# rubund/gnuais

Hardware: AMD Instinct MI355X
Metric: Msamples/s demodulated (N-channel batch, full chain) (higher is better)
Workload: dtype f32 FIR on int16 samples; u32 PLL/HDLC/CRC; 1 GPU; C3: 16384 ch x 48000 samples @48 kHz per GPU, full chain incl. HDLC/CRC-16; channels_per_gpu=16384, samples_per_channel=48000, parallelism=channels sharded over 1 GPU(s), one process per GPU, no collectives

## Files before the change

### gnuais_amd/csrc/batch.h

```cpp
#pragma once
#include <hip/hip_runtime.h>

#include <algorithm>
#include <cmath>
#include <cstdio>
#include <cstdlib>
#include <cstring>
#include <string>
#include <utility>
#include <vector>

#include "../../include/gnuais_hip.h"
#include "kernels.h"

using namespace gnuais;

namespace gnuais {
int fail(int code, const char *what, hipError_t e = hipSuccess);
}

#define HIP_TRY(expr)                                                          \
    do {                                                                       \
        hipError_t e_ = (expr);                                                \
        if (e_ != hipSuccess) return fail(GNUAIS_E_HIP, #expr, e_);            \
    } while (0)

namespace gnuais {

template <class T, bool PINNED = false>
struct Buf {
    T *p = nullptr;
    size_t bytes = 0;
    Buf() = default;
    Buf(Buf &&o) noexcept : p(std::exchange(o.p, nullptr)), bytes(std::exchange(o.bytes, 0)) {}
    Buf &operator=(Buf &&o) noexcept { std::swap(p, o.p); std::swap(bytes, o.bytes); return *this; }
    ~Buf() { (void) release(); }
    operator T *() const { return p; }
    hipError_t release()
    {
        const hipError_t e = !p ? hipSuccess : PINNED ? hipHostFree(p) : hipFree(p);
        p = nullptr;
        bytes = 0;
        return e;
    }
    hipError_t alloc(size_t n, bool zeroed = false)
    {
        hipError_t e = release();
        if (e == hipSuccess) e = PINNED ? hipHostMalloc((void **) &p, n, hipHostMallocDefault) : hipMalloc((void **) &p, n);
        if (e != hipSuccess) return p = nullptr, e;
        bytes = n;
        if (zeroed) e = PINNED ? (memset(p, 0, n), hipSuccess) : hipMemset(p, 0, n);
        if (e != hipSuccess) (void) release();
        return e;
    }
    hipError_t ensure(size_t n, bool zeroed = false) { return p ? hipSuccess : alloc(n, zeroed); }
    hipError_t grow(size_t need, size_t slack = 0) { return bytes >= need ? hipSuccess : alloc(need + slack); }
};
template <class T> using Pinned = Buf<T, true>;

struct Event {
    hipEvent_t e = nullptr;
    Event() = default;
    Event(Event &&o) noexcept : e(std::exchange(o.e, nullptr)) {}
    Event &operator=(Event &&o) noexcept { std::swap(e, o.e); return *this; }
    ~Event() { if (e) (void) hipEventDestroy(e); }
    operator hipEvent_t() const { return e; }
    hipError_t ensure(unsigned flags = hipEventDefault) { return e ? hipSuccess : hipEventCreateWithFlags(&e, flags); }
};

struct Stream {
    hipStream_t s = nullptr;
    Stream() = default;
    Stream(Stream &&o) noexcept : s(std::exchange(o.s, nullptr)) {}
    Stream &operator=(Stream &&o) noexcept { std::swap(s, o.s); return *this; }
    ~Stream() { if (s) (void) hipStreamDestroy(s); }
    operator hipStream_t() const { return s; }
    hipError_t ensure(int priority = 0) { return s ? hipSuccess : hipStreamCreateWithPriority(&s, hipStreamNonBlocking, priority); }
};

}

namespace gnuais {
struct WideStage {
    int K = 0, U = 1, D = 0, T = 0, H = 0, R = 0, NA = 0;
    int per[CHAN_MAX_K] = {}, off[CHAN_MAX_K] = {};
    Buf<uint32_t> mix, poly, hist[2];
    Buf<int32_t> groups;
    Buf<int16_t> taps;
    int cur = 0;
    unsigned long long n = 0;
};
}

enum Stage { CHAN, DISC, AFC, CHAIN, N_STAGES };

enum FormId { AUDIO, IQ, WIDE };

struct gnuais_batch {
    int device = 0;
    int N = 0, NT = 0, NE = 0, d = 0;
    uint32_t pllinc = 0;
    int max_len = 0, frame_cap = 0;
    int sgn_words = 0, bits_words = 0;
    std::vector<float> taps;
    float te[128] = {0};
    static constexpr int HB = 4;
    Buf<int16_t> hist[HB];
    int hist_cur = 0;
    static constexpr int NBUF = 8;
    int nbuf = 3;
    int sets_alloc = 0;
    Buf<uint32_t> sgn[NBUF];
    Buf<uint32_t> pll, lastbit, prev;
    int n_cu = 256;
    Buf<uint32_t> segbits[NBUF];
    Buf<uint32_t> segcnt[NBUF];
    int n_seg = 0, seg_words = 0;
    hipStream_t s_k[4] = {nullptr, nullptr, nullptr, nullptr};
    hipStream_t s_k_default[4] = {nullptr, nullptr, nullptr, nullptr};
    static constexpr int POOL = 12;
    Stream pool[POOL];
    Event e_done[5][NBUF];
    unsigned long long calls = 0, hdlc_calls = 0;
    bool pipeline = true;
    Buf<uint32_t> ctl, cand;
    Buf<uint32_t> cand_first[NBUF], cand_count[NBUF];
    int cand_K = 64;
    Buf<int32_t> counters;
    Buf<int> maxval[HB];
    int max_cur = 0, max_last = 0;
    Buf<float> d_taps;
    Buf<MfmaTaps> d_mfma;
    Buf<uint8_t> d_seq[2];
    Buf<char> d_text;
    Buf<void> nmea_scratch;
    Buf<char> d_msg;
    Buf<uint32_t> d_word;
    Buf<void> vt;
    Buf<uint32_t> vt_fslot;
    uint32_t vt_slots = 0;
    int vt_capacity = 0;
    static constexpr int NRING = 8;
    Buf<gnuais_frame> ring[NRING];
    Buf<uint32_t> ring_count[NRING];
    Buf<uint2> ring_chunks[NRING];
    int ring_runs[NRING] = {};
    int n_chunks = 0;
    bool frame_times = false;
    unsigned long long rows = 0;
    bool clock_fresh = true;
    Buf<int64_t> times;
    bool frame_signal = false, fs_iq_call = false;
    int fs_RB = 0, fs_nbuf = 0;
    unsigned long long fs_v0 = 0, fs_end = 0;
    Buf<int64_t> fs_ring;
    Buf<uint32_t> fs_carry;
    Buf<gnuais_frame_signal> signal;
    int occ_E = 0, occ_margin = 0, occ_CB = 0, occ_nbuf = 0, occ_W = 0;
    bool occ_cover_clean = false;
    unsigned long long occ_v0 = 0, occ_seq = 0, occ_drained = 0;
    long long occ_next = 0, occ_lost = 0;
    long long occ_first[64] = {};
    Buf<uint16_t> occ_codes;
    Buf<uint8_t> occ_cover, occ_carry;
    Buf<gnuais_occupancy> occ_out;
    bool repair = false;
    Buf<int32_t> repaired;
    bool long_frames = false;
    int long_cap = 0;
    Buf<uint32_t> long_ctl, long_open, long_count;
    Buf<int32_t> long_counters;
    Buf<gnuais_long_frame> long_ring;
    bool long_repair = false;
    int long_cand_cap = 0;
    int long_parity = 0;
    Buf<uint32_t> long_clean, long_cand, long_cand_count;
    int uq_window = 0, uq_hash_bits = 64, uq_cur = 0, uq_n_tail = 0;
    long long uq_late = 0;
    Buf<uint32_t> uq_tail[2];
    Buf<void> uq_scratch;
    Buf<void> uq_heard;
    int ring_cur = 0;
    bool streaming = false;
    hipStream_t s_post = nullptr, s_copy = nullptr;
    Stream s_copy_own;
    Event e_fill[NRING], e_fmt[NRING], e_txt[NRING];
    Buf<char> sd_text[NRING];
    Pinned<char> sh_text[NRING];
    Pinned<uint32_t> sh_info;
    int s_stage[NRING] = {};
    size_t sh_text_want = 0;
    Buf<uint32_t> sd_info;
    bool copy_on_k3 = false;
    int copy_wgs = 24;
    Buf<uint8_t> sd_seq[2];
    int sd_seq_cur = 0;
    unsigned long long stream_calls = 0;
    Buf<int16_t> stage_x;
    Buf<float> stage_f;
    Pinned<int16_t> pin[2];
    Buf<int16_t> dev_in[2];
    size_t pin_bytes = 0;
    Stream s_io;
    Event e_in[2];
    hipEvent_t e_in_hook = nullptr;
    unsigned long long host_calls = 0;
    FirOptions fir;
    SignBounds sign;
    int stage_mask = 0x1f;
    int k0 = 0;
    int pll_variant = 0;
    int hdlc_lpw = 0;
    int hdlc_variant = 1;
    bool timing = false;
    int timing_stride = 1;
    static constexpr int TIMING_RING = 64;
    Event evr[TIMING_RING][10];
    unsigned long long timed_calls = 0;
    int last_k = 0;
    bool timed_last = false;
    struct { hipStream_t s = nullptr; bool used = false; } last[N_STAGES];
    int last_len = 0;
    int pll_form = 0;
    int k3_same = 1;
    Buf<int16_t> iq_prev;
    Buf<int16_t> iq_audio;
    WideStage wide;
    Buf<int16_t> wide_iq;
    int afc_W = 0, afc_nb = 0, afc_est_row = -1;
    unsigned long long afc_n = 0;
    Buf<int64_t> afc_blk;
    Buf<int16_t> afc_delay, afc_est, afc_audio;
};

struct Form {
    int bytes, cols, rows;
    unsigned stages;
    int up = 1;
    size_t bytes_of(int in_rows) const { return (size_t) bytes * (size_t) cols * (size_t) in_rows; }
};

namespace gnuais {
int set_device(const gnuais_batch *b);
int drain(gnuais_batch *b, unsigned stages, hipStream_t s);
hipStream_t k3_stream(const gnuais_batch *b);
hipStream_t behind_k3(const gnuais_batch *b);
double now_ms();
int chan_zero_state(gnuais_batch *b);
int afc_zero_state(gnuais_batch *b);
int occ_zero_state(gnuais_batch *b);
int occ_tail(gnuais_batch *b, const HdlcLaunch &h, int len, hipStream_t s);
}
```

### gnuais_amd/csrc/capi_delivery.hip

```cpp
#include "batch.h"

extern "C" {

static int ensure_post_buffers(gnuais_batch *b, uint32_t have)
{
    const size_t need_text = (size_t) have * 164, need_scratch = nmea_scratch_bytes((int) have);
    HIP_TRY(b->d_text.grow(need_text));
    HIP_TRY(b->nmea_scratch.grow(need_scratch));
    return GNUAIS_OK;
}

struct Pending {
    uint32_t have;
    bool overflow, watchdog;
};

static int read_pending(gnuais_batch *b, Pending &p)
{
    if (int rc = gnuais_batch_sync(b)) return rc;
    uint32_t cnt[4] = {0, 0, 0, 0};
    HIP_TRY(hipMemcpy(cnt, b->ring_count[0], sizeof cnt, hipMemcpyDeviceToHost));
    p.have = std::min<uint32_t>(cnt[0], (uint32_t) b->frame_cap);
    p.overflow = cnt[1] || cnt[0] > (uint32_t) b->frame_cap;
    p.watchdog = cnt[3] != 0;
    return GNUAIS_OK;
}

static int late_error(const char *who, bool watchdog, bool overflow, const char *watchdog_tail = "")
{
    char msg[200];
    if (watchdog) {
        snprintf(msg, sizeof msg, "%s: the PLL stage's watchdog fired (device hung or badly oversubscribed)%s", who, watchdog_tail);
        return fail(GNUAIS_E_HIP, msg);
    }
    if (!overflow) return GNUAIS_OK;
    snprintf(msg, sizeof msg, "%s: frame ring overflowed, frames were dropped", who);
    return fail(GNUAIS_E_OVERFLOW, msg);
}

static int finish_drain(gnuais_batch *b, const Pending &p, const char *who, const char *watchdog_tail = "")
{
    HIP_TRY(hipMemset(b->ring_count[0], 0, sizeof(uint32_t) * 4));
    b->hdlc_calls = 0;
    return late_error(who, p.watchdog, p.overflow, watchdog_tail);
}

static int upload_seq(gnuais_batch *b, const uint8_t *seqnr)
{
    const size_t N = (size_t) b->N;
    for (auto &p : b->d_seq) HIP_TRY(p.ensure(N));
    HIP_TRY(hipMemcpy(b->d_seq[0], seqnr, N, hipMemcpyHostToDevice));
    HIP_TRY(hipMemcpy(b->d_seq[1], b->d_seq[0], N, hipMemcpyDeviceToDevice));
    return GNUAIS_OK;
}

static int drain_impl(gnuais_batch *b, gnuais_frame *h_frames, int max_frames, int *n_frames,
                      uint8_t *seqnr, char *out, size_t out_cap, size_t *out_len, int *n_sentences,
                      int64_t *h_times = nullptr, gnuais_frame_signal *h_signal = nullptr)
{
    if (b->streaming) return fail(GNUAIS_E_STATE, "drain: the batch is streaming (gnuais_batch_stream_nmea); "
                                                  "set_option(\"streaming\", 0) leaves that mode");
    Pending pend;
    if (int rc = read_pending(b, pend)) return rc;
    const uint32_t have = pend.have;
    if (h_frames && (uint32_t) max_frames < have) return fail(GNUAIS_E_ARG, "drain: frame buffer too small");
    if (have) {
        const size_t N = (size_t) b->N;
        if (int rc = ensure_post_buffers(b, have)) return rc;
        if (seqnr) {
            if (int rc = upload_seq(b, seqnr)) return rc;
            uint32_t info[3] = {0, 0, 0};
            HIP_TRY(nmea_format(b->ring[0], (int) have, b->N, b->d_seq[0], b->d_seq[1], b->d_text, b->d_text.bytes,
                                b->nmea_scratch, b->nmea_scratch.bytes, info, nullptr));
            if (info[2]) return fail(GNUAIS_E_HIP, "drain: a frame record names a channel outside the batch");
            if ((size_t) info[0] > out_cap) {
                *out_len = info[0];
                return fail(GNUAIS_E_ARG, "drain: text buffer too small");
            }
            if (info[0]) HIP_TRY(hipMemcpy(out, b->d_text, info[0], hipMemcpyDeviceToHost));
            HIP_TRY(hipMemcpy(seqnr, b->d_seq[1], N, hipMemcpyDeviceToHost));
            *out_len = info[0];
            if (n_sentences) *n_sentences = (int) info[1];
        }
        if (h_frames) {
            static_assert(sizeof(gnuais_frame_signal) == sizeof(int64_t), "the signal records leave through the times' gather");
            gnuais_frame *sorted = reinterpret_cast<gnuais_frame *>(b->d_text.p);
            int64_t *sorted_t = reinterpret_cast<int64_t *>(sorted + have), *sorted_s = sorted_t + have;
            HIP_TRY(frames_sort_timed(b->ring[0], h_times ? b->times.p : nullptr, (int) have, sorted, sorted_t,
                                      b->nmea_scratch, b->nmea_scratch.bytes, nullptr,
                                      h_signal ? reinterpret_cast<const int64_t *>(b->signal.p) : nullptr, sorted_s));
            HIP_TRY(hipMemcpy(h_frames, sorted, sizeof(gnuais_frame) * have, hipMemcpyDeviceToHost));
            if (h_times) HIP_TRY(hipMemcpy(h_times, sorted_t, sizeof(int64_t) * have, hipMemcpyDeviceToHost));
            if (h_signal) HIP_TRY(hipMemcpy(h_signal, sorted_s, sizeof(gnuais_frame_signal) * have, hipMemcpyDeviceToHost));
        }
        if (n_frames) *n_frames = (int) have;
    }
    return finish_drain(b, pend, "drain", "; results are incomplete");
}

int gnuais_batch_drain_messages(gnuais_batch *b, uint8_t *seqnr, const char *chanid, char *nmea, size_t nmea_cap,
                                size_t *nmea_len, int *n_sentences, char *text, size_t text_cap, size_t *text_len,
                                int *n_lines, int *n_frames)
{
    if (!b || !seqnr || !nmea_len || !text_len || (nmea_cap && !nmea) || (text_cap && !text))
        return fail(GNUAIS_E_ARG, "drain_messages: argument");
    if (b->streaming) return fail(GNUAIS_E_ARG, "drain_messages: the batch is streaming (gnuais_batch_stream_nmea)");
    *nmea_len = *text_len = 0;
    if (n_sentences) *n_sentences = 0;
    if (n_lines) *n_lines = 0;
    if (n_frames) *n_frames = 0;
    Pending pend;
    if (int rc = read_pending(b, pend)) return rc;
    const uint32_t have = pend.have;
    if (have) {
        const size_t N = (size_t) b->N, line = messages_line_bytes();
        if (nmea_cap < (size_t) have * 164 || text_cap < (size_t) have * line)
            return fail(GNUAIS_E_ARG, "drain_messages: buffers too small (164 / 512 bytes per pending frame always suffice)");
        if (int rc = ensure_post_buffers(b, have)) return rc;
        const size_t need = (size_t) have * line * 2 + (size_t) have * 8 + 256 + N + 256;
        HIP_TRY(b->d_msg.grow(need, need / 4));
        char *lines = b->d_msg, *packed = lines + (size_t) have * line;
        uint32_t *len = reinterpret_cast<uint32_t *>(packed + (size_t) have * line), *off = len + have;
        uint32_t *info2 = off + have;
        char *d_chanid = reinterpret_cast<char *>(info2 + 64);
        if (chanid) HIP_TRY(hipMemcpy(d_chanid, chanid, N, hipMemcpyHostToDevice));
        if (int rc = upload_seq(b, seqnr)) return rc;
        uint32_t raw[4] = {0, 0, 0, 0}, inf[2] = {0, 0};
        HIP_TRY(nmea_format_enqueue(b->ring[0], (int) have, (int) have, b->N, b->d_seq[0], b->d_seq[1], b->d_text,
                                    b->d_text.bytes, b->nmea_scratch, b->nmea_scratch.bytes, raw, nullptr, 0, 0,
                                    nullptr, nullptr));
        HIP_TRY(messages_format_enqueue(b->ring[0], (int) have, b->N, b->d_seq[0], chanid ? d_chanid : nullptr,
                                        b->nmea_scratch, b->nmea_scratch.bytes, lines, len, off, packed,
                                        (size_t) have * line, info2, nullptr));
        HIP_TRY(hipDeviceSynchronize());
        HIP_TRY(hipMemcpy(inf, info2, 8, hipMemcpyDeviceToHost));
        if (raw[3]) return fail(GNUAIS_E_HIP, "drain_messages: a frame record names a channel outside the batch");
        const size_t nl = (size_t) raw[0] + raw[1];
        if (nl) HIP_TRY(hipMemcpy(nmea, b->d_text, nl, hipMemcpyDeviceToHost));
        if (inf[0]) HIP_TRY(hipMemcpy(text, packed, inf[0], hipMemcpyDeviceToHost));
        HIP_TRY(hipMemcpy(seqnr, b->d_seq[1], N, hipMemcpyDeviceToHost));
        *nmea_len = nl;
        *text_len = inf[0];
        if (n_sentences) *n_sentences = (int) raw[2];
        if (n_lines) *n_lines = (int) inf[1];
        if (n_frames) *n_frames = (int) have;
    }
    return finish_drain(b, pend, "drain_messages");
}

int gnuais_batch_fold_vessels(gnuais_batch *b, gnuais_vessel *vessels, int cap, int *n_vessels)
{
    if (!b || !n_vessels || cap < 0 || (cap > 0 && !vessels)) return fail(GNUAIS_E_ARG, "fold_vessels: argument");
    if (b->streaming) return fail(GNUAIS_E_ARG, "fold_vessels: the batch is streaming (gnuais_batch_stream_nmea)");
    *n_vessels = 0;
    Pending pend;
    if (int rc = read_pending(b, pend)) return rc;
    const uint32_t have = pend.have;
    if (!have) return GNUAIS_OK;
    if (int rc = ensure_post_buffers(b, have)) return rc;
    gnuais_vessel *d_tab = reinterpret_cast<gnuais_vessel *>(b->d_text.p);
    const int d_cap = (int) std::min<size_t>(b->d_text.bytes / sizeof(gnuais_vessel), (size_t) have);
    HIP_TRY(b->d_word.ensure(16));
    HIP_TRY(vessels_fold_enqueue(b->ring[0], (int) have, b->nmea_scratch, b->nmea_scratch.bytes, d_tab, d_cap,
                                 b->d_word, nullptr));
    HIP_TRY(hipDeviceSynchronize());
    uint32_t nv = 0;
    HIP_TRY(hipMemcpy(&nv, b->d_word, 4, hipMemcpyDeviceToHost));
    *n_vessels = (int) nv;
    if ((int) nv > cap) return fail(GNUAIS_E_OVERFLOW, "fold_vessels: table too small (*n_vessels entries needed)");
    if (nv) HIP_TRY(hipMemcpy(vessels, d_tab, sizeof(gnuais_vessel) * nv, hipMemcpyDeviceToHost));
    return GNUAIS_OK;
}

int gnuais_batch_vessel_table_enable(gnuais_batch *b, int capacity)
{
    if (!b || capacity < 1 || capacity > (1 << 24)) return fail(GNUAIS_E_ARG, "vessel_table_enable: capacity 1 .. 2^24");
    if (int rc = gnuais_batch_sync(b)) return rc;
    if (b->s_post) HIP_TRY(hipStreamSynchronize(b->s_post));
    uint32_t slots = 1024;
    while (slots < 2u * (uint32_t) capacity) slots <<= 1;
    b->vt_slots = 0;
    HIP_TRY(b->vt.alloc(vessel_table_bytes(slots), true));
    HIP_TRY(b->vt_fslot.ensure(sizeof(uint32_t) * (size_t) b->frame_cap));
    b->vt_slots = slots;
    b->vt_capacity = capacity;
    return GNUAIS_OK;
}

int gnuais_batch_vessel_table_clear(gnuais_batch *b)
{
    if (!b || !b->vt) return fail(GNUAIS_E_STATE, "vessel_table_clear: no table (gnuais_batch_vessel_table_enable)");
    if (int rc = gnuais_batch_sync(b)) return rc;
    if (b->s_post) HIP_TRY(hipStreamSynchronize(b->s_post));
    HIP_TRY(hipMemset(b->vt, 0, vessel_table_bytes(b->vt_slots)));
    return GNUAIS_OK;
}

int gnuais_batch_vessel_table_update(gnuais_batch *b)
{
    if (!b || !b->vt) return fail(GNUAIS_E_STATE, "vessel_table_update: no table (gnuais_batch_vessel_table_enable)");
    if (b->streaming) return fail(GNUAIS_E_STATE, "vessel_table_update: a streaming batch updates its table by itself");
    if (int rc = gnuais_batch_sync(b)) return rc;
    HIP_TRY(vessel_table_update_enqueue(b->ring[0], b->ring_count[0], b->frame_cap, b->vt, b->vt_slots, b->vt_fslot, behind_k3(b)));
    return GNUAIS_OK;
}

int gnuais_batch_vessel_table(gnuais_batch *b, gnuais_vessel *vessels, int cap, int *n_vessels)
{
    if (!b || !n_vessels || cap < 0 || (cap > 0 && !vessels)) return fail(GNUAIS_E_ARG, "vessel_table: argument");
    *n_vessels = 0;
    if (!b->vt) return fail(GNUAIS_E_STATE, "vessel_table: no table (gnuais_batch_vessel_table_enable)");
    if (int rc = set_device(b)) return rc;
    hipStream_t s = b->streaming ? b->s_post : behind_k3(b);
    uint32_t info[4] = {0, 0, 0, 0};
    int n = 0;
    HIP_TRY(vessel_table_fetch(b->vt, b->vt_slots, vessels, cap, &n, info, s));
    *n_vessels = n;
    if (info[1] || (int) info[0] > b->vt_capacity) {
        char msg[160];
        snprintf(msg, sizeof msg, "vessel_table: more vessels than the table was enabled for (%u seen%s, capacity %d)",
                 info[0], info[1] ? ", some dropped" : "", b->vt_capacity);
        return fail(GNUAIS_E_OVERFLOW, msg);
    }
    if (n > cap) return fail(GNUAIS_E_OVERFLOW, "vessel_table: output too small (*n_vessels entries needed)");
    std::sort(vessels, vessels + n, [](const gnuais_vessel &x, const gnuais_vessel &y) { return x.mmsi < y.mmsi; });
    return GNUAIS_OK;
}

int gnuais_batch_drain_frames(gnuais_batch *b, gnuais_frame *h_out, int max, int *n_out)
{
    if (!b || !n_out || (max > 0 && !h_out)) return fail(GNUAIS_E_ARG, "drain_frames: argument");
    *n_out = 0;
    static gnuais_frame none;
    return drain_impl(b, h_out ? h_out : &none, max, n_out, nullptr, nullptr, 0, nullptr, nullptr);
}

int gnuais_batch_drain_frames_timed(gnuais_batch *b, gnuais_frame *h_out, int64_t *h_times, int max, int *n_out)
{
    if (!b || !n_out || (max > 0 && (!h_out || !h_times))) return fail(GNUAIS_E_ARG, "drain_frames_timed: argument");
    *n_out = 0;
    if (!b->frame_times) return fail(GNUAIS_E_STATE, "drain_frames_timed: the batch does not time its frames (gnuais_batch_frame_times)");
    static gnuais_frame none;
    static int64_t none_t;
    return drain_impl(b, h_out ? h_out : &none, max, n_out, nullptr, nullptr, 0, nullptr, nullptr, h_times ? h_times : &none_t);
}

int gnuais_batch_drain_frames_signal(gnuais_batch *b, gnuais_frame *h_out, int64_t *h_times, gnuais_frame_signal *h_signal,
                                     int max, int *n_out)
{
    if (!b || !n_out || (max > 0 && (!h_out || !h_times || !h_signal))) return fail(GNUAIS_E_ARG, "drain_frames_signal: argument");
    *n_out = 0;
    if (!b->frame_signal) return fail(GNUAIS_E_STATE, "drain_frames_signal: the batch does not measure its frames (gnuais_batch_frame_signal)");
    static gnuais_frame none;
    static int64_t none_t;
    static gnuais_frame_signal none_s;
    return drain_impl(b, h_out ? h_out : &none, max, n_out, nullptr, nullptr, 0, nullptr, nullptr, h_times ? h_times : &none_t,
                      h_signal ? h_signal : &none_s);
}

static int drain_unique_impl(gnuais_batch *b, gnuais_frame *h_out, int64_t *h_times, int32_t *h_copies, int max, int *n_out,
                             int32_t *h_first, gnuais_hearer *h_members, int *n_members)
{
    *n_out = 0;
    if (!b->uq_window) return fail(GNUAIS_E_STATE, "drain_frames_unique: the batch does not merge duplicates (gnuais_batch_unique)");
    if (b->streaming) return fail(GNUAIS_E_STATE, "drain_frames_unique: the batch is streaming (gnuais_batch_stream_nmea)");
    Pending pend;
    if (int rc = read_pending(b, pend)) return rc;
    const uint32_t have = pend.have;
    if ((uint32_t) max < have) return fail(GNUAIS_E_ARG, "drain_frames_unique: buffers too small (one entry per pending frame always suffices)");
    const size_t m = (size_t) b->uq_n_tail + have;
    if (m) {
        if (have)
            if (int rc = ensure_post_buffers(b, have)) return rc;
        const size_t need = unique_scratch_bytes((int) m);
        HIP_TRY(b->uq_scratch.grow(need, need / 4));
        Buf<uint32_t> &next = b->uq_tail[b->uq_cur ^ 1];
        HIP_TRY(next.grow(64 * m, 16 * m));
        auto bits_of = [](unsigned long long v) { int n = 1; while (v >> n) ++n; return n; };
        UniqueLaunch a;
        a.frames = b->ring[0];
        a.times = b->times;
        a.have = (int) have;
        a.tail = b->uq_tail[b->uq_cur];
        a.n_tail = b->uq_n_tail;
        a.tail_out = next;
        a.window = b->uq_window;
        a.rows = (long long) b->rows;
        a.hash_bits = b->uq_hash_bits;
        a.ch_bits = bits_of((unsigned long long) (b->N - 1));
        a.time_bits = bits_of(b->rows);
        a.scratch = b->uq_scratch;
        a.scratch_bytes = b->uq_scratch.bytes;
        a.out_frames = reinterpret_cast<gnuais_frame *>(b->d_text.p);
        a.out_times = reinterpret_cast<int64_t *>(a.out_frames + have);
        a.out_copies = reinterpret_cast<int32_t *>(a.out_times + have);
        if (h_first) {
            static_assert(sizeof(gnuais_hearer) == 24 && sizeof(gnuais_frame_signal) == 8, "a member is three 64-bit words");
            const size_t need_h = unique_heard_scratch_bytes((int) have);
            HIP_TRY(b->uq_heard.grow(need_h, need_h / 4));
            a.signal = b->frame_signal ? b->signal.p : nullptr;
            a.heard_scratch = b->uq_heard;
            a.heard_scratch_bytes = b->uq_heard.bytes;
            a.out_first = a.out_copies + have;
            const uintptr_t at = reinterpret_cast<uintptr_t>(a.out_first + have + 1);
            a.out_members = reinterpret_cast<gnuais_hearer *>((at + 15) & ~(uintptr_t) 15);
        }
        uint32_t info[UNIQUE_INFO_WORDS] = {0};
        for (int exact = 0; exact < 2; ++exact) {
            HIP_TRY(unique_cluster_enqueue(a, exact != 0, nullptr));
            HIP_TRY(hipMemcpy(info, unique_info(a.scratch), sizeof info, hipMemcpyDeviceToHost));
            if (!info[UNIQUE_INFO_COLLISION]) break;
        }
        const uint32_t np = info[UNIQUE_INFO_PRIMARIES];
        if (np > have || info[UNIQUE_INFO_TAIL] > m) return fail(GNUAIS_E_HIP, "drain_frames_unique: the stage's counts are out of range");
        if (np) {
            HIP_TRY(unique_deliver_enqueue(a, (int) np, nullptr));
            HIP_TRY(hipMemcpy(h_out, a.out_frames, sizeof(gnuais_frame) * np, hipMemcpyDeviceToHost));
            HIP_TRY(hipMemcpy(h_times, a.out_times, sizeof(int64_t) * np, hipMemcpyDeviceToHost));
            HIP_TRY(hipMemcpy(h_copies, a.out_copies, sizeof(int32_t) * np, hipMemcpyDeviceToHost));
            if (h_first) {
                HIP_TRY(hipMemcpy(h_first, a.out_first, sizeof(int32_t) * ((size_t) np + 1), hipMemcpyDeviceToHost));
                const int32_t nm = h_first[np];
                if (nm < 0 || (uint32_t) nm > have) return fail(GNUAIS_E_HIP, "drain_frames_heard: the stage's counts are out of range");
                HIP_TRY(hipMemcpy(h_members, a.out_members, sizeof(gnuais_hearer) * (size_t) nm, hipMemcpyDeviceToHost));
                *n_members = (int) nm;
            }
        }
        unsigned long long late = 0;
        memcpy(&late, info + UNIQUE_INFO_LATE, sizeof late);
        b->uq_cur ^= 1;
        b->uq_n_tail = (int) info[UNIQUE_INFO_TAIL];
        b->uq_late += (long long) late;
        *n_out = (int) np;
    }
    return finish_drain(b, pend, h_first ? "drain_frames_heard" : "drain_frames_unique", "; results are incomplete");
}

int gnuais_batch_drain_frames_unique(gnuais_batch *b, gnuais_frame *h_out, int64_t *h_times, int32_t *h_copies, int max,
                                     int *n_out)
{
    if (!b || !n_out || max < 0 || (max > 0 && (!h_out || !h_times || !h_copies)))
        return fail(GNUAIS_E_ARG, "drain_frames_unique: argument");
    return drain_unique_impl(b, h_out, h_times, h_copies, max, n_out, nullptr, nullptr, nullptr);
}

int gnuais_batch_drain_frames_heard(gnuais_batch *b, gnuais_frame *h_out, int64_t *h_times, int32_t *h_copies, int max,
                                    int *n_out, int32_t *h_first, gnuais_hearer *h_members, int *n_members)
{
    if (!b || !n_out || !n_members || !h_first || max < 0 || (max > 0 && (!h_out || !h_times || !h_copies || !h_members)))
        return fail(GNUAIS_E_ARG, "drain_frames_heard: argument");
    *n_members = 0;
    h_first[0] = 0;
    return drain_unique_impl(b, h_out, h_times, h_copies, max, n_out, h_first, h_members, n_members);
}

int gnuais_batch_drain_nmea(gnuais_batch *b, uint8_t *seqnr, char *out, size_t out_cap, size_t *out_len,
                            int *n_sentences, int *n_frames)
{
    if (!b || !seqnr || !out_len || (out_cap > 0 && !out)) return fail(GNUAIS_E_ARG, "drain_nmea: argument");
    *out_len = 0;
    if (n_sentences) *n_sentences = 0;
    if (n_frames) *n_frames = 0;
    return drain_impl(b, nullptr, 0, n_frames, seqnr, out, out_cap, out_len, n_sentences);
}

int gnuais_batch_drain_frames_nmea(gnuais_batch *b, gnuais_frame *h_frames, int max, int *n_frames,
                                   uint8_t *seqnr, char *out, size_t out_cap, size_t *out_len, int *n_sentences)
{
    if (!b || !h_frames || !n_frames || !seqnr || !out_len || (out_cap > 0 && !out))
        return fail(GNUAIS_E_ARG, "drain_frames_nmea: argument");
    *n_frames = 0;
    *out_len = 0;
    if (n_sentences) *n_sentences = 0;
    return drain_impl(b, h_frames, max, n_frames, seqnr, out, out_cap, out_len, n_sentences);
}

static int stream_setup(gnuais_batch *b)
{
    constexpr int NR = gnuais_batch::NRING;
    const size_t N = (size_t) b->N;
    const size_t text_cap = (size_t) b->frame_cap * 164;
    if (b->frame_times) return fail(GNUAIS_E_STATE, "stream_nmea: the batch times its frames (gnuais_batch_frame_times); "
                                                    "the streamed delivery carries no times");
    if (b->repair) return fail(GNUAIS_E_STATE, "stream_nmea: the batch repairs frames (gnuais_batch_repair); the streamed "
                                               "delivery's order table describes the CRC stage's records only");
    if (b->frame_signal) return fail(GNUAIS_E_STATE, "stream_nmea: the batch measures its frames (gnuais_batch_frame_signal); "
                                                     "the streamed delivery carries no records of them");
    if (b->uq_window) return fail(GNUAIS_E_STATE, "stream_nmea: the batch merges duplicates (gnuais_batch_unique); the "
                                                  "streamed delivery has no such stage");
    if (b->long_frames) return fail(GNUAIS_E_STATE, "stream_nmea: the batch decodes long frames (gnuais_batch_long_frames); "
                                                    "the streamed delivery carries no records of them");
    if (int rc = gnuais_batch_sync(b)) return rc;
    for (int q = 1; q < NR; ++q) {
        HIP_TRY(b->ring[q].ensure(sizeof(gnuais_frame) * (size_t) b->frame_cap));
        HIP_TRY(b->ring_count[q].ensure(sizeof(uint32_t) * 4, true));
    }
    b->n_chunks = k3_blocks(b->N) * k3_passes(b->cand_K);
    b->sh_text_want = std::max(b->sh_text_want, ((size_t) b->frame_cap * 32 + 65536) & ~(size_t) 15);
    for (int q = 0; q < NR; ++q) {
        HIP_TRY(b->ring_chunks[q].ensure(sizeof(uint2) * (size_t) b->n_chunks));
        b->ring_runs[q] = 2;
        HIP_TRY(b->sd_text[q].ensure(text_cap));
        for (Event *e : {&b->e_fill[q], &b->e_fmt[q], &b->e_txt[q]}) HIP_TRY(e->ensure(hipEventDisableTiming));
        HIP_TRY(b->sh_text[q].ensure(b->sh_text_want));
    }
    HIP_TRY(b->sd_info.ensure(sizeof(uint32_t) * 8 * NR, true));
    if (const char *v = getenv("GNUAIS_COPY_WGS")) b->copy_wgs = std::max(1, atoi(v));
    if (const char *v = getenv("GNUAIS_COPY_ON_K3")) b->copy_on_k3 = atoi(v) != 0;
    HIP_TRY(b->nmea_scratch.grow(nmea_scratch_bytes(b->frame_cap, b->n_chunks)));
    if (!b->s_copy_own) {
        int lo = 0, hi = 0;
        HIP_TRY(hipDeviceGetStreamPriorityRange(&lo, &hi));
        HIP_TRY(b->s_copy_own.ensure(hi));
        b->s_copy = b->s_copy_own;
    }
    HIP_TRY(b->sh_info.ensure(sizeof(uint32_t) * 8 * NR, true));
    for (auto &p : b->sd_seq) HIP_TRY(p.ensure(N, true));
    HIP_TRY(hipDeviceSynchronize());
    b->streaming = true;
    return GNUAIS_OK;
}

int gnuais_batch_stream_nmea(gnuais_batch *b, const char **text, size_t *len, int *n_sentences, int *n_frames)
{
    if (!b || !text || !len) return fail(GNUAIS_E_ARG, "stream_nmea: argument");
    if (int rc = set_device(b)) return rc;
    *text = nullptr;
    *len = 0;
    if (n_sentences) *n_sentences = 0;
    if (n_frames) *n_frames = -1;
    constexpr int NR = gnuais_batch::NRING;
    const size_t N = (size_t) b->N;
    if (!b->streaming)
        if (int rc = stream_setup(b)) return rc;
    hipStream_t sD = behind_k3(b);
    const int c = b->ring_cur;
    HIP_TRY(hipEventRecord(b->e_fill[c], sD));
    const int runs = b->ring_runs[c];
    const int nx = (c + 1) % NR;
    if (b->s_stage[nx]) HIP_TRY(hipStreamWaitEvent(sD, b->e_fmt[nx], 0));
    b->ring_cur = nx;
    b->ring_runs[nx] = 0;
    int rc_late = GNUAIS_OK;
    if (b->s_stage[nx]) {
        HIP_TRY(hipEventSynchronize(b->e_txt[nx]));
        const uint32_t *info = b->sh_info + 8 * nx;
        const uint32_t have = std::min<uint32_t>(info[4], (uint32_t) b->frame_cap);
        const size_t n_text = (size_t) info[0] + info[1];
        if (n_text > b->sh_text[nx].bytes) {
            const size_t want = std::max(b->sh_text_want, (n_text + n_text / 2 + 65536) & ~(size_t) 15);
            b->sh_text_want = want;
            HIP_TRY(b->sh_text[nx].grow(b->sh_text_want));
            HIP_TRY(hipMemcpyAsync(b->sh_text[nx], b->sd_text[nx], n_text, hipMemcpyDeviceToHost, b->s_copy));
            HIP_TRY(hipStreamSynchronize(b->s_copy));
        }
        *text = b->sh_text[nx];
        *len = n_text;
        if (n_sentences) *n_sentences = (int) info[2];
        if (n_frames) *n_frames = (int) have;
        b->s_stage[nx] = 0;
        if (info[3]) rc_late = fail(GNUAIS_E_HIP, "stream_nmea: a frame record names a channel outside the batch");
        else rc_late = late_error("stream_nmea", info[7] != 0, info[5] || info[4] > (uint32_t) b->frame_cap);
    }
    b->s_post = sD;
    uint32_t *totals = nullptr;
    HIP_TRY(b->sh_text[c].grow(b->sh_text_want));
    if (runs >= 1) {
        int n_host = -1;
        if (runs > 1) {
            uint32_t cnt[4];
            HIP_TRY(hipStreamSynchronize(b->s_post));
            HIP_TRY(hipMemcpy(cnt, b->ring_count[c], 16, hipMemcpyDeviceToHost));
            n_host = (int) std::min<uint32_t>(cnt[0], (uint32_t) b->frame_cap);
        }
        if (n_host != 0) {
            uint8_t *sin = b->sd_seq[b->sd_seq_cur], *sout = b->sd_seq[b->sd_seq_cur ^ 1];
            HIP_TRY(hipMemcpyAsync(sout, sin, N, hipMemcpyDeviceToDevice, b->s_post));
            HIP_TRY(nmea_format_enqueue(b->ring[c], n_host, b->frame_cap, b->N, sin, sout, b->sd_text[c],
                                        b->sd_text[c].bytes, b->nmea_scratch, b->nmea_scratch.bytes, nullptr,
                                        b->ring_chunks[c], b->n_chunks, k3_passes(b->cand_K), &totals, b->s_post));
            b->sd_seq_cur ^= 1;
        }
    }
    if (b->vt && runs >= 1)
        HIP_TRY(vessel_table_update_enqueue(b->ring[c], b->ring_count[c], b->frame_cap, b->vt, b->vt_slots, b->vt_fslot,
                                            b->s_post));
    HIP_TRY(nmea_slot_info_enqueue(totals, b->ring_count[c], b->sd_info + 8 * c, b->s_post));
    HIP_TRY(hipMemsetAsync(b->ring_count[c], 0, 16, b->s_post));
    HIP_TRY(hipEventRecord(b->e_fmt[c], b->s_post));
    hipStream_t sc = b->copy_on_k3 ? b->s_post : b->s_copy;
    if (!b->copy_on_k3) HIP_TRY(hipStreamWaitEvent(sc, b->e_fmt[c], 0));
    HIP_TRY(nmea_text_copy_enqueue(b->sd_text[c], b->sd_info + 8 * c, b->sh_text[c], b->sh_text[c].bytes,
                                   b->sh_info + 8 * c, b->copy_wgs, sc));
    HIP_TRY(hipEventRecord(b->e_txt[c], sc));
    b->s_stage[c] = 1;
    b->hdlc_calls = 0;
    b->stream_calls++;
    return rc_late;
}

int gnuais_batch_pending_frames(gnuais_batch *b, int *n_out)
{
    if (!b || !n_out) return fail(GNUAIS_E_ARG, "pending_frames: argument");
    if (b->streaming) return fail(GNUAIS_E_STATE, "pending_frames: the batch is streaming (gnuais_batch_stream_nmea)");
    Pending pend;
    if (int rc = read_pending(b, pend)) return rc;
    *n_out = (int) pend.have;
    return GNUAIS_OK;
}

int gnuais_batch_discard_frames(gnuais_batch *b, void *stream)
{
    if (!b) return fail(GNUAIS_E_ARG, "discard_frames: NULL batch");
    if (b->streaming) return fail(GNUAIS_E_STATE, "discard_frames: the batch is streaming (gnuais_batch_stream_nmea)");
    if (int rc = set_device(b)) return rc;
    hipStream_t s = b->pipeline ? k3_stream(b) : (hipStream_t) stream;
    HIP_TRY(hipMemsetAsync(b->ring_count[0], 0, sizeof(uint32_t) * 3, s));
    b->hdlc_calls = 0;
    return GNUAIS_OK;
}

int gnuais_batch_autotune_delivery(gnuais_batch *b, const int16_t *d_samples, int len, void *stream, float *ms_per_call)
{
    if (!b || !d_samples) return fail(GNUAIS_E_ARG, "autotune_delivery: NULL argument");
    if (int rc = gnuais_batch_sync(b)) return rc;
    const char *text = nullptr;
    size_t tl = 0;
    if (int rc = gnuais_batch_stream_nmea(b, &text, &tl, nullptr, nullptr)) return rc;
    if (!b->pipeline) {
        if (ms_per_call) *ms_per_call = 0.0f;
        return gnuais_batch_reset(b);
    }
    const bool timing = b->timing;
    b->timing = false;
    auto quiesce = [&]() -> int {
        if (int rc = gnuais_batch_sync(b)) return rc;
        HIP_TRY(hipDeviceSynchronize());
        return GNUAIS_OK;
    };
    auto measure = [&](double &ms, int meas) -> int {
        const int warm = gnuais_batch::NRING + 2;
        for (int i = 0; i < warm + meas; ++i) {
            if (i == warm) {
                if (int rc = quiesce()) return rc;
                ms = -now_ms();
            }
            if (int rc = gnuais_batch_run(b, d_samples, len, stream)) return rc;
            const int rc = gnuais_batch_stream_nmea(b, &text, &tl, nullptr, nullptr);
            if (rc != GNUAIS_OK && rc != GNUAIS_E_OVERFLOW) return rc;
        }
        if (int rc = quiesce()) return rc;
        ms = (ms + now_ms()) / meas;
        return GNUAIS_OK;
    };
    hipStream_t own = b->s_copy_own;
    hipStream_t top[2] = {own, own};
    double top_ms[2] = {1e30, 1e30};
    for (int cand = -1; cand < gnuais_batch::POOL; ++cand) {
        hipStream_t st = cand < 0 ? own : b->pool[cand];
        bool used = false;
        for (int q = 0; q < 4; ++q) used |= b->s_k[q] == st;
        if (used || !st) continue;
        b->s_copy = st;
        double ms = 0;
        if (int rc = measure(ms, 12)) return rc;
        if (ms < top_ms[0]) { top_ms[1] = top_ms[0]; top[1] = top[0]; top_ms[0] = ms; top[0] = st; }
        else if (ms < top_ms[1]) { top_ms[1] = ms; top[1] = st; }
    }
    hipStream_t best_s = top[0];
    double best = 1e30;
    for (int k = 0; k < 2; ++k) {
        if (k == 1 && top[1] == top[0]) break;
        b->s_copy = top[k];
        double ms = 0;
        if (int rc = measure(ms, 30)) return rc;
        if (ms < best) { best = ms; best_s = top[k]; }
    }
    b->s_copy = best_s;
    b->timing = timing;
    if (ms_per_call) *ms_per_call = (float) best;
    return gnuais_batch_reset(b);
}

}
```

### gnuais_amd/csrc/gnuais_capi.hip

```cpp
#include <chrono>

#include "batch.h"

namespace gnuais {
namespace scalar { hipError_t launch_fir_slice(const FirLaunch &a, hipStream_t stream); }
}

static thread_local std::string g_err;

int gnuais::fail(int code, const char *what, hipError_t e)
{
    char buf[512];
    if (e != hipSuccess)
        snprintf(buf, sizeof buf, "%s: %s", what, hipGetErrorString(e));
    else
        snprintf(buf, sizeof buf, "%s", what);
    g_err = buf;
    return code;
}

static const double k_tap_half[18] = {
    2.5959e-55, 2.9479e-49, 1.4741e-43, 3.2462e-38, 3.1480e-33, 1.3443e-28,
    2.5280e-24, 2.0934e-20, 7.6339e-17, 1.2259e-13, 8.6690e-11, 2.6996e-08,
    3.7020e-06, 2.2355e-04, 5.9448e-03, 6.9616e-02, 3.5899e-01, 8.1522e-01};

int gnuais::drain(gnuais_batch *b, unsigned stages, hipStream_t s)
{
    for (int q = 0; q < N_STAGES; ++q) {
        auto &l = b->last[q];
        if (!(stages >> q & 1u) || !l.used || l.s == s) continue;
        HIP_TRY(hipStreamSynchronize(l.s));
        l.s = s;
    }
    return GNUAIS_OK;
}

int gnuais::set_device(const gnuais_batch *b)
{
    HIP_TRY(hipSetDevice(b->device));
    return GNUAIS_OK;
}

double gnuais::now_ms()
{
    return std::chrono::duration<double, std::milli>(std::chrono::steady_clock::now().time_since_epoch()).count();
}

hipStream_t gnuais::k3_stream(const gnuais_batch *b)
{
    return (b->k3_same && !b->streaming) ? b->s_k[2] : b->s_k[3];
}

hipStream_t gnuais::behind_k3(const gnuais_batch *b) { return b->pipeline ? k3_stream(b) : b->last[CHAIN].s; }

template <class T>
static int read_out(gnuais_batch *b, const void *d, size_t n, std::vector<T> &v)
{
    if (int rc = gnuais_batch_sync(b)) return rc;
    v.resize(n);
    HIP_TRY(hipMemcpy(v.data(), d, n * sizeof(T), hipMemcpyDeviceToHost));
    return GNUAIS_OK;
}

extern "C" {

const char *gnuais_last_error(void) { return g_err.c_str(); }
const char *gnuais_version(void) { return "gnuais-hip 0.1 (gfx950)"; }

int gnuais_default_taps(float *out36)
{
    if (!out36) return fail(GNUAIS_E_ARG, "gnuais_default_taps: NULL");
    for (int k = 0; k < 18; ++k) {
        out36[k] = (float) k_tap_half[k];
        out36[35 - k] = (float) k_tap_half[k];
    }
    return 36;
}

static hipError_t alloc_sets(gnuais_batch *b, int n)
{
    const size_t N = (size_t) b->N;
    for (int k = b->sets_alloc; k < n && k < gnuais_batch::NBUF; ++k) {
        struct { Buf<uint32_t> &buf; size_t bytes; } want[] = {
            {b->sgn[k], sizeof(uint32_t) * sgn_words_alloc(b->sgn_words, b->N)},
            {b->segbits[k], sizeof(uint32_t) * N * (size_t) b->n_seg * PACK_STRIDE},
            {b->segcnt[k], sizeof(uint32_t) * N * (size_t) b->n_seg},
            {b->cand_first[k], sizeof(uint32_t) * N},
            {b->cand_count[k], sizeof(uint32_t) * N}};
        for (auto &w : want)
            if (hipError_t e = w.buf.ensure(w.bytes, true)) return e;
        b->sets_alloc = k + 1;
    }
    return hipSuccess;
}

void gnuais_batch_destroy(gnuais_batch *b)
{
    if (!b) return;
    (void) hipSetDevice(b->device);
    delete b;
}

int gnuais_batch_create(gnuais_batch **out, int device, int n_channels, const float *taps,
                        int n_taps, unsigned pllinc, int max_len, int frame_capacity)
{
    if (!out) return fail(GNUAIS_E_ARG, "create: out is NULL");
    *out = nullptr;
    if (n_channels <= 0 || max_len <= 0) return fail(GNUAIS_E_ARG, "create: n_channels/max_len");
    if (taps && (n_taps <= 0 || n_taps > GNUAIS_MAX_TAPS)) return fail(GNUAIS_E_ARG, "create: n_taps");
    if (pllinc > 0xffffu) return fail(GNUAIS_E_ARG, "create: pllinc must be < 0x10000");
    int ndev = 0;
    HIP_TRY(hipGetDeviceCount(&ndev));
    if (ndev <= 0) return fail(GNUAIS_E_HIP, "create: no HIP device");
    if (device < 0 || device >= ndev) return fail(GNUAIS_E_ARG, "create: device index");
    HIP_TRY(hipSetDevice(device));
    {
        int lds = 0;
        if (hipDeviceGetAttribute(&lds, hipDeviceAttributeMaxSharedMemoryPerBlock, device) == hipSuccess &&
            lds < pll_need_lds())
            return fail(GNUAIS_E_HIP, "create: the device offers too little LDS per workgroup (gfx950 / MI355X with "
                                      "160 KB is what this library is built for)");
    }
    HIP_TRY(pll_prepare_device());

    gnuais_batch *b = new gnuais_batch;
    b->device = device;
    if (hipDeviceGetAttribute(&b->n_cu, hipDeviceAttributeMultiprocessorCount, device) != hipSuccess || b->n_cu <= 0)
        b->n_cu = 256;
    b->N = n_channels;
    if (taps) {
        b->taps.assign(taps, taps + n_taps);
    } else {
        b->taps.resize(36);
        gnuais_default_taps(b->taps.data());
    }
    b->NT = (int) b->taps.size();
    b->pllinc = pllinc ? pllinc : (0x10000u / 5u);
    b->max_len = max_len;
    b->frame_cap = frame_capacity > 0 ? frame_capacity : std::max(4096, n_channels * 48);

    int k0 = 0, k1 = b->NT - 1;
    while (k0 < b->NT - 1 && b->taps[k0] == 0.0f) ++k0;
    while (k1 > k0 && b->taps[k1] == 0.0f) --k1;
    b->NE = k1 - k0 + 1;
    b->d = b->NT - k0;
    b->k0 = k0;
    if (b->NE <= FIR_MAX_NE)
        for (int j = 0; j < b->NE; ++j) b->te[j] = b->taps[k0 + j];

    b->sign = sign_bounds(b->te, b->NE);
    b->sgn_words = (max_len + 31) / 32;
    const uint64_t step = (uint64_t) b->pllinc + b->pllinc / 16;
    b->bits_words = (int) (((uint64_t) max_len * step / 65536 + 2 + 31) / 32) + 1;

    const size_t N = (size_t) b->N;
    hipError_t e = hipSuccess;
    b->n_seg = (b->sgn_words + SEG_WORDS - 1) / SEG_WORDS;
    b->seg_words = (int) (((uint64_t) SEG_WORDS * 32 * step / 65536 + 2 + 31) / 32) + 1;
    const uint64_t launch_bits = std::max((uint64_t) b->bits_words * 32, (uint64_t) b->seg_words * 32 * (uint64_t) b->n_seg);
    b->cand_K = (int) std::max<uint64_t>(64, launch_bits / 30 + 2);
    if (const char *v = getenv("GNUAIS_NBUF")) b->nbuf = std::min((int) gnuais_batch::NBUF, std::max(2, atoi(v)));
    {
        const size_t per_set = sizeof(uint32_t) * (sgn_words_alloc(b->sgn_words, b->N) + N * (size_t) b->n_seg * (PACK_STRIDE + 1) + 2 * N);
        const size_t need = gnuais_batch::HB * (sizeof(int16_t) * N * b->NT + sizeof(int) * N) + (size_t) b->nbuf * per_set +
                            sizeof(uint32_t) * N * ((size_t) b->cand_K * CAND_WORDS + HDLC_CTL_WORDS + 6) +
                            sizeof(gnuais_frame) * (size_t) b->frame_cap;
        size_t free_b = 0, total_b = 0;
        if (hipMemGetInfo(&free_b, &total_b) == hipSuccess && need > free_b) {
            char msg[256];
            snprintf(msg, sizeof msg, "create: %d channels x %d samples need %.2f GB of device memory, device %d has %.2f GB free of %.2f",
                     b->N, b->max_len, need / 1e9, device, free_b / 1e9, total_b / 1e9);
            delete b;
            return fail(GNUAIS_E_HIP, msg);
        }
    }
    auto alloc = [&](auto &buf, size_t bytes) {
        if (e == hipSuccess) e = buf.alloc(bytes, true);
    };
    for (int q = 0; q < gnuais_batch::HB; ++q) alloc(b->hist[q], sizeof(int16_t) * N * b->NT);
    if (b->seg_words > 16) {
        gnuais_batch_destroy(b);
        return fail(GNUAIS_E_ARG, "create: pllinc too large (more than one slice per ~4.6 samples)");
    }
    if (e == hipSuccess) e = alloc_sets(b, b->nbuf);
    alloc(b->pll, sizeof(uint32_t) * N);
    alloc(b->lastbit, sizeof(uint32_t) * N);
    alloc(b->prev, sizeof(uint32_t) * N);
    alloc(b->ctl, sizeof(uint32_t) * N * HDLC_CTL_WORDS);
    alloc(b->cand, sizeof(uint32_t) * N * (size_t) b->cand_K * CAND_WORDS);
    alloc(b->ring_count[0], sizeof(uint32_t) * 4);
    alloc(b->counters, sizeof(int32_t) * N * 3);
    for (int q = 0; q < gnuais_batch::HB; ++q) alloc(b->maxval[q], sizeof(int) * N);
    alloc(b->ring[0], sizeof(gnuais_frame) * (size_t) b->frame_cap);
    alloc(b->d_taps, sizeof(float) * b->NT);
    alloc(b->iq_prev, sizeof(int16_t) * 2 * N);
    if (b->sign.mfma_ok) {
        MfmaTaps host;
        fir_sign_mfma_pack(b->sign.tq, b->sign.tq_sum, &host);
        alloc(b->d_mfma, sizeof(MfmaTaps));
        if (e == hipSuccess) e = hipMemcpy(b->d_mfma, &host, sizeof(MfmaTaps), hipMemcpyHostToDevice);
    }
    if (e == hipSuccess)
        e = hipMemcpy(b->d_taps, b->taps.data(), sizeof(float) * b->NT, hipMemcpyHostToDevice);
    for (auto &set : b->evr)
        for (auto &ev : set)
            if (e == hipSuccess) e = ev.ensure();
    for (auto &pair : b->e_done)
        for (auto &ev : pair)
            if (e == hipSuccess) e = ev.ensure(hipEventDisableTiming);
    {
        int lo = 0, hi = 0;
        if (e == hipSuccess) e = hipDeviceGetStreamPriorityRange(&lo, &hi);
        const char *order = getenv("GNUAIS_STREAM_ORDER");
        if (!order || strlen(order) != 4) order = "0123";
        int made = 0;
        for (int q = 0; q < 4; ++q) {
            const int idx = (order[q] - '0') & 3;
            if (e == hipSuccess && !b->s_k[idx]) {
                e = b->pool[made].ensure(hi);
                b->s_k[idx] = b->pool[made++];
            }
        }
        for (auto &st : b->s_k)
            if (e == hipSuccess && !st) {
                e = b->pool[made].ensure(hi);
                st = b->pool[made++];
            }
        for (int q = 0; q < 4; ++q) b->s_k_default[q] = b->s_k[q];
        for (; made < gnuais_batch::POOL; ++made)
            if (e == hipSuccess) e = b->pool[made].ensure(made < 8 ? hi : 0);
    }
    if (const char *v = getenv("GNUAIS_K3_SAME")) b->k3_same = atoi(v) != 0;
    if (const char *v = getenv("GNUAIS_PLL_VARIANT")) {
        const int pv = atoi(v);
        if (pv == 0 || pv == 7 || pv == 8) b->pll_variant = pv;
    }
    if (const char *v = getenv("GNUAIS_PIPELINE")) b->pipeline = atoi(v) != 0;
    if (const char *v = getenv("GNUAIS_HDLC_VARIANT")) b->hdlc_variant = atoi(v) != 0;
    if (const char *v = getenv("GNUAIS_HDLC_LPW")) b->hdlc_lpw = std::min(64, std::max(1, atoi(v)));
    if (e != hipSuccess) {
        gnuais_batch_destroy(b);
        return fail(GNUAIS_E_HIP, "create: device allocation", e);
    }
    if (const char *v = getenv("GNUAIS_FIR_VARIANT")) {
        const int fv = atoi(v);
        if (fv == 0 || fv == 3) b->fir.fir_variant = fv;
    }
    if (const char *v = getenv("GNUAIS_FIR_FLAG2")) b->fir.fir_flag2 = atoi(v) != 0;
    if (const char *v = getenv("GNUAIS_FIR_T")) b->fir.fir_T = std::max(64, atoi(v) / 32 * 32);
    *out = b;
    int rc = gnuais_batch_reset(b);
    if (rc != GNUAIS_OK) {
        gnuais_batch_destroy(b);
        *out = nullptr;
    }
    return rc;
}


static int rings_reset(gnuais_batch *b)
{
    for (int q = 0; q < gnuais_batch::NRING; ++q) {
        if (b->ring_count[q]) HIP_TRY(hipMemset(b->ring_count[q], 0, sizeof(uint32_t) * 4));
        b->s_stage[q] = 0;
        b->ring_runs[q] = 0;
    }
    b->ring_cur = 0;
    b->stream_calls = 0;
    return GNUAIS_OK;
}

static int long_zero_state(gnuais_batch *b, bool everything)
{
    if (!b->long_ctl) return GNUAIS_OK;
    HIP_TRY(launch_hdlc_long_reset(b->long_ctl, everything ? b->long_counters.p : nullptr, b->N, nullptr));
    if (everything) HIP_TRY(hipMemset(b->long_count, 0, sizeof(uint32_t) * 2));
    if (everything && b->long_cand_count) {
        HIP_TRY(hipMemset(b->long_cand_count, 0, sizeof(uint32_t) * 2));
        b->long_parity = 0;
    }
    return GNUAIS_OK;
}

static int latch_rows(gnuais_batch *b, unsigned long long rows)
{
    b->rows = rows;
    b->fs_v0 = b->fs_end = rows;
    return occ_zero_state(b);
}

int gnuais_batch_reset(gnuais_batch *b)
{
    if (!b) return fail(GNUAIS_E_ARG, "reset: NULL batch");
    if (int rc = set_device(b)) return rc;
    const size_t N = (size_t) b->N;
    HIP_TRY(hipDeviceSynchronize());
    for (int q = 0; q < gnuais_batch::HB; ++q)
        HIP_TRY(hipMemset(b->hist[q], 0, sizeof(int16_t) * N * b->NT));
    b->hist_cur = 0;
    HIP_TRY(hipMemset(b->pll, 0, sizeof(uint32_t) * N));
    HIP_TRY(hipMemset(b->lastbit, 0, sizeof(uint32_t) * N));
    HIP_TRY(hipMemset(b->prev, 0, sizeof(uint32_t) * N));
    for (int k = 0; k < b->sets_alloc; ++k)
        HIP_TRY(hipMemset(b->segcnt[k], 0, sizeof(uint32_t) * N * (size_t) b->n_seg));
    b->calls = 0;
    if (int rc = latch_rows(b, 0)) return rc;
    b->last[CHAIN].used = false;
    b->hdlc_calls = 0;
    HIP_TRY(hipMemset(b->counters, 0, sizeof(int32_t) * N * 3));
    if (b->repaired) HIP_TRY(hipMemset(b->repaired, 0, sizeof(int32_t) * N));
    b->uq_n_tail = 0;
    b->uq_late = 0;
    for (int q = 0; q < gnuais_batch::HB; ++q) HIP_TRY(hipMemset(b->maxval[q], 0, sizeof(int) * N));
    b->max_cur = 0;
    b->max_last = 0;
    if (int rc = rings_reset(b)) return rc;
    for (auto &p : b->sd_seq)
        if (p) HIP_TRY(hipMemset(p, 0, N));
    HIP_TRY(launch_hdlc_reset(b->ctl, b->N, nullptr));
    if (int rc = long_zero_state(b, true)) return rc;
    HIP_TRY(hipMemset(b->iq_prev, 0, sizeof(int16_t) * 2 * N));
    b->last[DISC].used = false;
    if (int rc = chan_zero_state(b)) return rc;
    if (int rc = afc_zero_state(b)) return rc;
    HIP_TRY(hipDeviceSynchronize());
    b->last_len = 0;
    b->pll_form = 0;
    b->clock_fresh = true;
    return GNUAIS_OK;
}

int gnuais_batch_set_clock(gnuais_batch *b, long long rows, const uint64_t *h_bits)
{
    if (!b) return fail(GNUAIS_E_ARG, "set_clock: NULL batch");
    if (rows < 0) return fail(GNUAIS_E_ARG, "set_clock: rows < 0");
    if (!b->clock_fresh) return fail(GNUAIS_E_STATE, "set_clock: a run or decode call has been made since create / reset");
    if (b->wide.K || b->afc_W)
        return fail(GNUAIS_E_STATE, "set_clock: not with a wide stage or the AFC configured (their sample counts start at 0)");
    if (int rc = set_device(b)) return rc;
    const size_t N = (size_t) b->N;
    std::vector<uint32_t> lo(N), hi(N);
    for (size_t c = 0; c < N; ++c) {
        const uint64_t v = h_bits ? h_bits[c] : 0;
        lo[c] = (uint32_t) v;
        hi[c] = (uint32_t) (v >> 32);
    }
    HIP_TRY(hipDeviceSynchronize());
    HIP_TRY(hipMemcpy(b->ctl + 2 * N, lo.data(), sizeof(uint32_t) * N, hipMemcpyHostToDevice));
    HIP_TRY(hipMemcpy(b->ctl + 5 * N, hi.data(), sizeof(uint32_t) * N, hipMemcpyHostToDevice));
    return latch_rows(b, (unsigned long long) rows);
}

int gnuais_batch_set_option(gnuais_batch *b, const char *name, int value)
{
    if (!b || !name) return fail(GNUAIS_E_ARG, "set_option: NULL");
    if (!strcmp(name, "stage_mask")) {
        b->stage_mask = value & 0x1f;
        return GNUAIS_OK;
    }
    if (!strcmp(name, "fir_T")) {
        if (value < 64 || value % 32) return fail(GNUAIS_E_ARG, "fir_T must be a multiple of 32, >= 64");
        b->fir.fir_T = value;
    } else if (!strcmp(name, "nbuf")) {
        if (value < 2 || value > gnuais_batch::NBUF) return fail(GNUAIS_E_ARG, "nbuf must be 2..8");
        if (b->frame_signal && value > b->fs_nbuf)
            return fail(GNUAIS_E_STATE, "nbuf: the block ring of gnuais_batch_frame_signal is sized for the depth it was switched on "
                                        "at; switch it off first");
        if (b->occ_E && value > b->occ_nbuf)
            return fail(GNUAIS_E_STATE, "nbuf: the rings of gnuais_batch_occupancy are sized for the depth it was switched on at; "
                                        "switch it off first");
        if (int rc = gnuais_batch_sync(b)) return rc;
        HIP_TRY(hipDeviceSynchronize());
        HIP_TRY(alloc_sets(b, value));
        b->nbuf = value;
    } else if (!strcmp(name, "streaming")) {
        if (value != 0 && b->frame_times)
            return fail(GNUAIS_E_STATE, "streaming: the batch times its frames (gnuais_batch_frame_times); the streamed delivery carries no times");
        if (value != 0 && b->repair)
            return fail(GNUAIS_E_STATE, "streaming: the batch repairs frames (gnuais_batch_repair); the streamed delivery's order table describes the CRC stage's records only");
        if (value != 0 && b->frame_signal)
            return fail(GNUAIS_E_STATE, "streaming: the batch measures its frames (gnuais_batch_frame_signal); the streamed delivery carries no records of them");
        if (value != 0 && b->uq_window)
            return fail(GNUAIS_E_STATE, "streaming: the batch merges duplicates (gnuais_batch_unique); the streamed delivery has no such stage");
        if (value != 0 && b->long_repair)
            return fail(GNUAIS_E_STATE, "streaming: the batch repairs long frames (gnuais_batch_long_repair); the streamed delivery carries no records of them");
        if (value != 0 && b->long_frames)
            return fail(GNUAIS_E_STATE, "streaming: the batch decodes long frames (gnuais_batch_long_frames); the streamed delivery carries no records of them");
        if (value != 0) return fail(GNUAIS_E_ARG, "streaming can only be switched off here (stream_nmea switches it on)");
        if (b->streaming) {
            if (int rc = gnuais_batch_sync(b)) return rc;
            HIP_TRY(hipDeviceSynchronize());
            if (int rc = rings_reset(b)) return rc;
            b->hdlc_calls = 0;
            b->streaming = false;
        }
    } else if (!strcmp(name, "fir_flag2")) {
        if (value != 0 && value != 1) return fail(GNUAIS_E_ARG, "fir_flag2: 0 or 1");
        b->fir.fir_flag2 = value;
    } else if (!strcmp(name, "fir_pk_taps")) {
        if (value != 0 && value != 48) return fail(GNUAIS_E_ARG, "fir_pk_taps: 0 or 48");
        b->fir.fir_pk_taps = value;
    } else if (!strcmp(name, "fir_mfma")) {
        if (value != 0 && value != 1) return fail(GNUAIS_E_ARG, "fir_mfma: 0 or 1");
        b->fir.fir_mfma = value;
    } else if (!strcmp(name, "fir_variant")) {
        if (value != 0 && value != 3) return fail(GNUAIS_E_ARG, "fir_variant must be 0 (the exact sum for every sample) or 3 (the sign-exact slicer)");
        b->fir.fir_variant = value;
    } else if (!strcmp(name, "timing_stride")) {
        if (value < 1) return fail(GNUAIS_E_ARG, "timing_stride must be >= 1");
        b->timing_stride = value;
    } else if (!strcmp(name, "pipeline")) {
        b->pipeline = value != 0;
    } else if (!strcmp(name, "pll_variant")) {
        if (value != 0 && value != 7 && value != 8)
            return fail(GNUAIS_E_ARG, "pll_variant must be 0 (by channel count), 7 (time-parallel, pll_tp.hip) or 8 (pll_h3.hip)");
        b->pll_variant = value;
    } else if (!strcmp(name, "hdlc_variant")) {
        b->hdlc_variant = value != 0;
    } else if (!strcmp(name, "unique_hash_bits")) {
        if (value < 1 || value > 64) return fail(GNUAIS_E_ARG, "unique_hash_bits must be 1..64");
        b->uq_hash_bits = value;
    } else if (!strcmp(name, "hdlc_lpw")) {
        if (value < 1 || value > 64) return fail(GNUAIS_E_ARG, "hdlc_lpw must be 1..64");
        b->hdlc_lpw = value;
    } else {
        return fail(GNUAIS_E_ARG, "set_option: unknown option");
    }
    return GNUAIS_OK;
}

static void fill_fir(const gnuais_batch *b, FirLaunch &f, const int16_t *x, int len, float *dump,
                     int k)
{
    memset(&f, 0, sizeof f);
    f.x = x;
    f.hist = b->hist[b->hist_cur];
    f.sgn = b->sgn[k];
    f.dump = dump;
    f.maxval = b->maxval[b->max_cur];
    f.hist_out = b->hist[(b->hist_cur + 1) % gnuais_batch::HB];
    f.maxval_next = b->maxval[(b->max_cur + 2) % gnuais_batch::HB];
    f.d_taps = b->d_taps;
    memcpy(f.te, b->te, sizeof f.te);
    f.N = b->N;
    f.L = len;
    f.NT = b->NT;
    f.NE = b->NE;
    f.d = b->d;
    f.te_mem = b->d_taps + b->k0;
    f.map = 1;
}

static void fill_hdlc(const gnuais_batch *b, HdlcLaunch &h, int k)
{
    h.segbits = b->segbits[k]; h.segcnt = b->segcnt[k]; h.ctl = b->ctl; h.cand = b->cand;
    h.cand_first = b->cand_first[k]; h.cand_count = b->cand_count[k];
    h.counters = b->counters;
    h.frames = b->ring[b->ring_cur];
    h.frame_count = b->ring_count[b->ring_cur];
    h.frame_cap = (uint32_t) b->frame_cap; h.N = b->N; h.n_seg = b->n_seg;
    h.seg_words = b->seg_words; h.K = b->cand_K; h.K_call = b->cand_K;
    int small_lpw = 1;
    while (small_lpw < 16 && (b->N + small_lpw - 1) / small_lpw > 512) small_lpw *= 2;
    if (b->N > PLL_TP_MAX_CHANNELS) small_lpw = 16;
    const int ev_lpw = 2 * ((b->N + 63) / 64) > (b->n_cu > 0 ? b->n_cu : 256) ? 64 : small_lpw;
    h.lanes_per_wave = b->hdlc_lpw ? b->hdlc_lpw : (b->hdlc_variant ? ev_lpw : 64);
    h.chunks = (b->streaming && b->ring_runs[b->ring_cur] == 0) ? b->ring_chunks[b->ring_cur] : nullptr;
}

static FrameTimeLaunch fill_frame_times(const gnuais_batch *b, const HdlcLaunch &h, int len)
{
    FrameTimeLaunch t;
    t.frames = h.frames; t.frame_count = h.frame_count; t.frame_cap = h.frame_cap;
    t.ctl = h.ctl; t.segcnt = h.segcnt; t.times = b->times;
    t.N = h.N; t.n_seg = h.n_seg; t.seg_words = h.seg_words;
    t.len = len; t.n0 = (int64_t) b->rows;
    return t;
}

static FrameSignalLaunch fill_frame_signal(const gnuais_batch *b, const HdlcLaunch &h, int len)
{
    FrameSignalLaunch a;
    a.frames = h.frames; a.frame_count = h.frame_count; a.frame_cap = h.frame_cap;
    a.times = b->times; a.ring = b->fs_ring; a.signal = b->signal.p;
    a.RB = b->fs_RB; a.N = h.N;
    a.len = len; a.n0 = (int64_t) b->rows;
    a.pllinc = b->pllinc; a.n_taps = b->NT; a.afc_window = b->afc_W;
    a.v0 = (int64_t) (b->fs_iq_call ? b->fs_v0 : b->rows + (unsigned long long) std::max(len, 0));
    return a;
}

static RepairLaunch fill_repair(const gnuais_batch *b, const HdlcLaunch &h)
{
    RepairLaunch r;
    r.cand = h.cand; r.cand_first = h.cand_first; r.cand_count = h.cand_count;
    r.repaired = b->repaired;
    r.frames = h.frames; r.frame_count = h.frame_count; r.frame_cap = h.frame_cap;
    r.N = h.N; r.K = h.K;
    return r;
}

static LongLaunch fill_long(const gnuais_batch *b, const HdlcLaunch &h, int len)
{
    LongLaunch a;
    a.segbits = h.segbits; a.segcnt = h.segcnt; a.ctl = h.ctl;
    a.lctl = b->long_ctl; a.open = b->long_open; a.counters = b->long_counters;
    a.frames = b->long_ring.p; a.frame_count = b->long_count; a.frame_cap = (uint32_t) b->long_cap;
    a.N = h.N; a.n_seg = h.n_seg; a.seg_words = h.seg_words;
    a.len = len; a.n0 = (int64_t) b->rows;
    if (b->long_repair) {
        a.clean = b->long_clean; a.cand = b->long_cand; a.cand_count = b->long_cand_count;
        a.cand_cap = (uint32_t) b->long_cand_cap; a.parity = b->long_parity;
    }
    return a;
}

static int run_long(gnuais_batch *b, const HdlcLaunch &h, int len, hipStream_t s)
{
    HIP_TRY(launch_hdlc_long(fill_long(b, h, len), s));
    if (b->long_repair) {
        LongRepairLaunch r;
        r.cand = b->long_cand; r.cand_count = b->long_cand_count.p + b->long_parity; r.cand_cap = (uint32_t) b->long_cand_cap;
        r.repaired = b->long_counters.p + 2 * (size_t) b->N;
        r.frames = b->long_ring.p; r.frame_count = b->long_count; r.frame_cap = (uint32_t) b->long_cap;
        r.N = b->N;
        r.blocks = 16 * std::max(b->n_cu, 1);
        HIP_TRY(launch_hdlc_long_repair(r, s));
        b->long_parity ^= 1;
    }
    return GNUAIS_OK;
}

static int run_fir(gnuais_batch *b, const int16_t *x, int len, float *dump, hipStream_t s, int k)
{
    const FirPlan p = plan_fir(b->sign, b->fir, FirShape{b->N, b->NT, b->NE, b->d}, len, dump != nullptr);
    FirLaunch f;
    fill_fir(b, f, x, len, dump, k);
    static_cast<FirThresholds &>(f) = p.th;
    if (b->sign.ok)
        for (int j = 0; j < f.NC; ++j) f.ctaps[j] = b->te[(b->NE - f.NC) / 2 + j];
    switch (p.kernel) {
    case FirKernel::GENERIC:
        HIP_TRY(hipMemsetAsync(f.maxval_next, 0, sizeof(int) * (size_t) b->N, s));
        HIP_TRY(launch_fir_generic(f, s));
        HIP_TRY(launch_fir_history(x, f.hist, f.hist_out, b->N, len, b->NT, s));
        break;
    case FirKernel::SCALAR32:
        HIP_TRY(scalar::launch_fir_slice(f, s));
        break;
    case FirKernel::SIGN:
        HIP_TRY(launch_fir_sign(f, s));
        break;
    case FirKernel::SIGN_PACKED:
        HIP_TRY(launch_fir_sign_pk(f, s));
        break;
    case FirKernel::SIGN_PACKED_MFMA: {
        FirLaunch m = f;
        f.T = p.head;
        f.max_segments = 1;
        m.NC = FIR_MFMA_NC;
        m.mfma = b->d_mfma;
        m.eps_seen = p.mfma_seen_u;
        m.eps_ahead = p.mfma_abs_u;
        HIP_TRY(launch_fir_sign_pk(f, s));
        HIP_TRY(launch_fir_sign_mfma(m, p.head, s));
        break;
    }
    }
    b->hist_cur = (b->hist_cur + 1) % gnuais_batch::HB;
    b->max_last = b->max_cur;
    b->max_cur = (b->max_cur + 1) % gnuais_batch::HB;
    return GNUAIS_OK;
}

static void fill_pll(const gnuais_batch *b, PllLaunch &p, int k, int len)
{
    p.sgn = b->sgn[k]; p.pll = b->pll; p.prev = b->prev;
    p.watchdog = b->ring_count[b->ring_cur] + 3; p.lastbit = b->lastbit;
    p.segbits = b->segbits[k]; p.segcnt = b->segcnt[k];
    p.N = b->N; p.L = len; p.n_seg = b->n_seg; p.seg_words = b->seg_words; p.pllinc = b->pllinc; p.variant = b->pll_variant;
    p.n_cu = b->n_cu;
}


static int run_tail(gnuais_batch *b, int k, int len, bool tm, const Event *ev,
                    hipStream_t s0, hipEvent_t after)
{
    const bool pl = b->pipeline;
    hipStream_t sC = pl ? b->s_k[2] : s0, sD = pl ? k3_stream(b) : s0;
    HdlcLaunch h;
    fill_hdlc(b, h, k);
    if (pl && after) HIP_TRY(hipStreamWaitEvent(sC, after, 0));
    if (pl && b->calls >= 1 && sD != sC)
        HIP_TRY(hipStreamWaitEvent(sC, b->e_done[4][(k + b->nbuf - 1) % b->nbuf], 0));
    if (tm) HIP_TRY(hipEventRecord(ev[5], sC));
    if (b->stage_mask & 8) HIP_TRY(b->hdlc_variant ? launch_hdlc_events(h, sC) : launch_hdlc_deframe(h, sC));
    if (tm) HIP_TRY(hipEventRecord(ev[7], sC));
    if (pl) HIP_TRY(hipEventRecord(b->e_done[3][k], sC));
    if (pl && sD != sC) HIP_TRY(hipStreamWaitEvent(sD, b->e_done[3][k], 0));
    if (tm) HIP_TRY(hipEventRecord(ev[9], sD));
    if (b->stage_mask & 16) HIP_TRY(launch_hdlc_crc(h, sD));
    if (b->repair && (b->stage_mask & 16)) HIP_TRY(launch_hdlc_repair(fill_repair(b, h), sD));
    if (b->frame_times && (b->stage_mask & 16)) HIP_TRY(launch_frame_times(fill_frame_times(b, h, len), sD));
    if (b->frame_signal && (b->stage_mask & 16)) HIP_TRY(launch_frame_signal(fill_frame_signal(b, h, len), sD));
    if (b->occ_E && b->fs_iq_call && (b->stage_mask & 16))
        if (int rc = occ_tail(b, h, len, sD)) return rc;
    if (b->long_frames && (b->stage_mask & 8))
        if (int rc = run_long(b, h, len, sD)) return rc;
    if (b->streaming) b->ring_runs[b->ring_cur]++;
    b->hdlc_calls++;
    if (tm) HIP_TRY(hipEventRecord(ev[4], sD));
    if (pl) HIP_TRY(hipEventRecord(b->e_done[4][k], sD));
    return GNUAIS_OK;
}

int gnuais_batch_run(gnuais_batch *b, const int16_t *d_samples, int len, void *stream)
{
    if (!b || !d_samples) return fail(GNUAIS_E_ARG, "run: NULL argument");
    if (len <= 0 || len > b->max_len) return fail(GNUAIS_E_ARG, "run: len out of range (max_len)");
    if (int rc = set_device(b)) return rc;
    b->clock_fresh = false;
    hipStream_t s0 = (hipStream_t) stream;
    const bool pl = b->pipeline;
    const int k = (int) (b->calls % (unsigned) b->nbuf);
    const bool reuse = pl && b->calls >= (unsigned) b->nbuf;
    const bool tm = b->timing && (b->calls % (unsigned) b->timing_stride) == 0;
    const Event *ev = b->evr[b->timed_calls % gnuais_batch::TIMING_RING];

    {
        hipStream_t sA = pl ? b->s_k[0] : s0;
        if (reuse) HIP_TRY(hipEventSynchronize(b->e_done[4][k]));
        if (int rc = drain(b, 1u << CHAIN, s0)) return rc;
        hipStream_t sF = s0;
        if (tm) HIP_TRY(hipEventRecord(ev[0], sF));
        if (b->stage_mask & 1)
            if (int rc = run_fir(b, d_samples, len, nullptr, sF, k)) return rc;
        if (tm) HIP_TRY(hipEventRecord(ev[1], sF));
        if (b->e_in_hook) {
            HIP_TRY(hipEventRecord(b->e_in_hook, sF));
            b->e_in_hook = nullptr;
        }
        if (pl) HIP_TRY(hipEventRecord(b->e_done[0][k], sF));
        PllLaunch p;
        fill_pll(b, p, k, len);
        if (pl) HIP_TRY(hipStreamWaitEvent(sA, b->e_done[0][k], 0));
        if (tm) HIP_TRY(hipEventRecord(ev[2], sA));
        if (b->stage_mask & 2) {
            b->pll_form = pll_form_of(p);
            HIP_TRY(launch_pll(p, sA));
        }
        if (tm) HIP_TRY(hipEventRecord(ev[6], sA));
        if (pl) HIP_TRY(hipEventRecord(b->e_done[1][k], sA));
        if (int rc = run_tail(b, k, len, tm, ev, s0, pl ? b->e_done[1][k] : nullptr)) return rc;
    }

    b->timed_last = tm;
    if (tm) b->timed_calls++;
    b->last[CHAIN] = {s0, true};
    b->last_len = len;
    b->last_k = k;
    b->calls++;
    b->rows += (unsigned long long) len;
    return GNUAIS_OK;
}

int gnuais_batch_autotune(gnuais_batch *b, const int16_t *d_samples, int len, void *stream, float *ms_per_call)
{
    if (!b || !d_samples) return fail(GNUAIS_E_ARG, "autotune: NULL argument");
    if (!b->pipeline) {
        if (ms_per_call) *ms_per_call = 0.0f;
        return GNUAIS_OK;
    }
    if (int rc = gnuais_batch_sync(b)) return rc;
    const bool timing = b->timing;
    b->timing = false;
    struct K3Own { gnuais_batch *b; int was; ~K3Own() { b->k3_same = was; } } k3_own{b, b->k3_same};
    b->k3_same = 0;
    auto measure = [&](double &ms, int meas = 10) -> int {
        const int warm = 4;
        for (int i = 0; i < warm + meas; ++i) {
            if (i == warm) {
                if (int rc = gnuais_batch_sync(b)) return rc;
                ms = -now_ms();
            }
            if (int rc = gnuais_batch_run(b, d_samples, len, stream)) return rc;
            if (int rc = gnuais_batch_discard_frames(b, stream)) return rc;
        }
        if (int rc = gnuais_batch_sync(b)) return rc;
        ms = (ms + now_ms()) / meas;
        return GNUAIS_OK;
    };
    const int order[4] = {0, 3, 2, 1};
    double best_all = 0;
    auto search = [&](int chosen[4]) -> int {
        for (int q = 0; q < 4; ++q) chosen[q] = -1;
        for (int r = 0; r < 4; ++r) {
            const int role = order[r];
            double best = 1e30;
            int best_s = -1;
            for (int cand = 0; cand < gnuais_batch::POOL; ++cand) {
                bool used = false;
                for (int q = 0; q < r; ++q) used |= chosen[order[q]] == cand;
                if (used) continue;
                int trial[4];
                for (int q = 0; q < 4; ++q) trial[q] = chosen[q];
                trial[role] = cand;
                for (int q = r + 1; q < 4; ++q) {
                    for (int f = 0; f < gnuais_batch::POOL; ++f) {
                        bool taken = false;
                        for (int t = 0; t < 4; ++t) taken |= trial[t] == f;
                        if (!taken) { trial[order[q]] = f; break; }
                    }
                }
                for (int q = 0; q < 4; ++q) b->s_k[q] = b->pool[trial[q]];
                double ms = 0;
                if (int rc = measure(ms)) return rc;
                if (ms < best) { best = ms; best_s = cand; }
            }
            chosen[role] = best_s;
        }
        return GNUAIS_OK;
    };
    hipStream_t cand_set[3][4];
    int n_sets = 0;
    for (int q = 0; q < 4; ++q) cand_set[0][q] = b->s_k_default[q];
    n_sets = 1;
    for (int rep = 0; rep < 2; ++rep) {
        int chosen[4];
        if (int rc = search(chosen)) return rc;
        for (int q = 0; q < 4; ++q) cand_set[n_sets][q] = b->pool[chosen[q]];
        ++n_sets;
    }
    int best_set = 0;
    best_all = 1e30;
    double ms_set[3] = {0, 0, 0};
    for (int k = 0; k < n_sets; ++k) {
        for (int q = 0; q < 4; ++q) b->s_k[q] = cand_set[k][q];
        if (int rc = measure(ms_set[k], 40)) return rc;
    }
    best_all = ms_set[0];
    for (int k = 1; k < n_sets; ++k)
        if (ms_set[k] < 0.97 * ms_set[0] && ms_set[k] < best_all) { best_all = ms_set[k]; best_set = k; }
    for (int q = 0; q < 4; ++q) b->s_k[q] = cand_set[best_set][q];
    b->timing = timing;
    if (ms_per_call) *ms_per_call = (float) best_all;
    return gnuais_batch_reset(b);
}

int gnuais_batch_sync(gnuais_batch *b)
{
    if (!b) return fail(GNUAIS_E_ARG, "sync: NULL batch");
    if (int rc = set_device(b)) return rc;
    HIP_TRY(hipStreamSynchronize(b->last[CHAIN].s));
    for (auto &st : b->s_k) HIP_TRY(hipStreamSynchronize(st));
    return GNUAIS_OK;
}


int gnuais_batch_filter(gnuais_batch *b, const int16_t *d_samples, int len, float *d_out,
                        void *stream)
{
    if (!b || !d_samples || !d_out) return fail(GNUAIS_E_ARG, "filter: NULL argument");
    if (len <= 0 || len > b->max_len) return fail(GNUAIS_E_ARG, "filter: len out of range");
    if (int rc = set_device(b)) return rc;
    hipStream_t s = (hipStream_t) stream;
    if (int rc = gnuais_batch_sync(b)) return rc;
    if (int rc = run_fir(b, d_samples, len, d_out, s, (int) (b->calls % (unsigned) b->nbuf))) return rc;
    b->last[CHAIN].s = s;
    b->timed_last = false;
    return GNUAIS_OK;
}

int gnuais_batch_filter_host(gnuais_batch *b, const int16_t *h_samples, int len, float *h_out)
{
    if (!b || !h_samples || !h_out) return fail(GNUAIS_E_ARG, "filter_host: NULL argument");
    if (len <= 0 || len > b->max_len) return fail(GNUAIS_E_ARG, "filter_host: len out of range");
    if (int rc = set_device(b)) return rc;
    const size_t n = (size_t) len * (size_t) b->N;
    HIP_TRY(b->stage_x.grow(n * sizeof(int16_t)));
    HIP_TRY(b->stage_f.grow(n * sizeof(float)));
    HIP_TRY(hipMemcpy(b->stage_x, h_samples, n * sizeof(int16_t), hipMemcpyHostToDevice));
    if (int rc = gnuais_batch_filter(b, b->stage_x, len, b->stage_f, nullptr)) return rc;
    if (int rc = gnuais_batch_sync(b)) return rc;
    HIP_TRY(hipMemcpy(h_out, b->stage_f, n * sizeof(float), hipMemcpyDeviceToHost));
    return GNUAIS_OK;
}

int gnuais_batch_decode_bits(gnuais_batch *b, const uint8_t *h_bits, int stride,
                             const int32_t *h_count)
{
    if (!b || !h_bits || !h_count || stride <= 0) return fail(GNUAIS_E_ARG, "decode_bits: argument");
    if (int rc = gnuais_batch_sync(b)) return rc;
    b->clock_fresh = false;
    const int N = b->N, segcap = b->seg_words * 32, chunk = segcap * b->n_seg;
    int maxc = 0;
    for (int c = 0; c < N; ++c) {
        if (h_count[c] < 0 || h_count[c] > stride) return fail(GNUAIS_E_ARG, "decode_bits: count");
        maxc = std::max(maxc, h_count[c]);
    }
    const size_t rowlen = (size_t) b->n_seg * PACK_STRIDE;
    std::vector<uint32_t> words(rowlen * N), cnt((size_t) b->n_seg * N);
    for (int pos = 0; pos < maxc; pos += chunk) {
        std::fill(words.begin(), words.end(), 0u);
        std::fill(cnt.begin(), cnt.end(), 0u);
        for (int c = 0; c < N; ++c) {
            const int n = std::max(0, std::min(chunk, h_count[c] - pos));
            const uint8_t *src = h_bits + (size_t) c * stride + pos;
            for (int k = 0; k < n; ++k) {
                const int seg = k / segcap, kk = k % segcap;
                if (src[k] & 1)
                    words[(size_t) c * rowlen + (size_t) seg * PACK_STRIDE + (kk >> 5)] |= 1u << (kk & 31);
            }
            for (int seg = 0; seg * segcap < n; ++seg)
                cnt[(size_t) c * b->n_seg + seg] = (uint32_t) std::min(segcap, n - seg * segcap);
        }
        HIP_TRY(hipMemcpy(b->segbits[0], words.data(), words.size() * 4, hipMemcpyHostToDevice));
        HIP_TRY(hipMemcpy(b->segcnt[0], cnt.data(), cnt.size() * 4, hipMemcpyHostToDevice));
        HdlcLaunch h;
        fill_hdlc(b, h, 0);
        HIP_TRY(b->hdlc_variant ? launch_hdlc_events(h, nullptr) : launch_hdlc_deframe(h, nullptr));
        HIP_TRY(launch_hdlc_crc(h, nullptr));
        if (b->repair) HIP_TRY(launch_hdlc_repair(fill_repair(b, h), nullptr));
        if (b->frame_times) HIP_TRY(launch_frame_times(fill_frame_times(b, h, 0), nullptr));
        if (b->frame_signal) HIP_TRY(launch_frame_signal(fill_frame_signal(b, h, 0), nullptr));
        if (b->long_frames)
            if (int rc = run_long(b, h, 0, nullptr)) return rc;
        if (b->streaming) b->ring_runs[b->ring_cur]++;
        b->hdlc_calls++;
        HIP_TRY(hipDeviceSynchronize());
    }
    b->last[CHAIN].s = nullptr;
    return GNUAIS_OK;
}

int gnuais_batch_last_bits(gnuais_batch *b, uint8_t *h_bits, int stride, int32_t *h_count)
{
    if (!b || !h_bits || !h_count || stride <= 0) return fail(GNUAIS_E_ARG, "last_bits: argument");
    if (int rc = gnuais_batch_sync(b)) return rc;
    const int N = b->N;
    const size_t rowlen = (size_t) b->n_seg * PACK_STRIDE;
    std::vector<uint32_t> words(rowlen * N), cnt((size_t) b->n_seg * N);
    HIP_TRY(hipMemcpy(words.data(), b->segbits[b->last_k], words.size() * 4, hipMemcpyDeviceToHost));
    HIP_TRY(hipMemcpy(cnt.data(), b->segcnt[b->last_k], cnt.size() * 4, hipMemcpyDeviceToHost));
    const int nseg_used = ((b->last_len + 31) / 32 + SEG_WORDS - 1) / SEG_WORDS;
    for (int c = 0; c < N; ++c) {
        int n = 0;
        uint8_t *dst = h_bits + (size_t) c * stride;
        for (int seg = 0; seg < nseg_used; ++seg) {
            const int m = (int) std::min<uint32_t>(cnt[(size_t) c * b->n_seg + seg],
                                                   (uint32_t) b->seg_words * 32);
            if (n + m > stride) return fail(GNUAIS_E_ARG, "last_bits: stride too small");
            const uint32_t *w = &words[(size_t) c * rowlen + (size_t) seg * PACK_STRIDE];
            for (int k = 0; k < m; ++k) dst[n + k] = (w[k >> 5] >> (k & 31)) & 1u;
            n += m;
        }
        h_count[c] = n;
    }
    return GNUAIS_OK;
}


int gnuais_batch_counters(gnuais_batch *b, gnuais_counters *h_out)
{
    if (!b || !h_out) return fail(GNUAIS_E_ARG, "counters: argument");
    const int N = b->N;
    std::vector<int32_t> v;
    if (int rc = read_out(b, b->counters, (size_t) N * 3, v)) return rc;
    for (int c = 0; c < N; ++c) {
        h_out[c].receivedframes = v[c];
        h_out[c].lostframes = v[(size_t) N + c];
        h_out[c].lostframes2 = v[(size_t) 2 * N + c];
    }
    return GNUAIS_OK;
}

int gnuais_batch_total_received(gnuais_batch *b, long long *total)
{
    if (!b || !total) return fail(GNUAIS_E_ARG, "total_received: argument");
    std::vector<int32_t> v;
    if (int rc = read_out(b, b->counters, (size_t) b->N, v)) return rc;
    long long t = 0;
    for (int32_t x : v) t += x;
    *total = t;
    return GNUAIS_OK;
}

int gnuais_batch_maxval(gnuais_batch *b, int16_t *h_out)
{
    if (!b || !h_out) return fail(GNUAIS_E_ARG, "maxval: argument");
    std::vector<int> v;
    if (int rc = read_out(b, b->maxval[b->max_last], (size_t) b->N, v)) return rc;
    for (int c = 0; c < b->N; ++c) h_out[c] = (int16_t) v[c];
    return GNUAIS_OK;
}

int gnuais_batch_pll_state(gnuais_batch *b, gnuais_pll_state *h_out)
{
    if (!b || !h_out) return fail(GNUAIS_E_ARG, "pll_state: argument");
    std::vector<uint32_t> v, lb, pv;
    if (int rc = read_out(b, b->pll, (size_t) b->N, v)) return rc;
    if (int rc = read_out(b, b->lastbit, (size_t) b->N, lb)) return rc;
    if (int rc = read_out(b, b->prev, (size_t) b->N, pv)) return rc;
    for (int c = 0; c < b->N; ++c) {
        h_out[c].pll = v[c] & 0xffffu;
        h_out[c].prev = pv[c] & 1;
        h_out[c].lastbit = lb[c] & 1;
    }
    return GNUAIS_OK;
}

int gnuais_batch_fsm_state(gnuais_batch *b, gnuais_fsm_state *h_out)
{
    if (!b || !h_out) return fail(GNUAIS_E_ARG, "fsm_state: argument");
    std::vector<uint32_t> v;
    if (int rc = read_out(b, b->ctl, (size_t) b->N, v)) return rc;
    for (int c = 0; c < b->N; ++c) {
        const uint32_t w = v[c];
        h_out[c].state = w & 7;
        h_out[c].nstartsign = (w >> 3) & 15;
        h_out[c].antallpreamble = (w >> 7) & 15;
        h_out[c].antallenner = (w >> 11) & 7;
        h_out[c].bitstuff = (w >> 14) & 1;
        h_out[c].last = (w >> 15) & 1;
        h_out[c].bufferpos = (w >> 16) & 511;
    }
    return GNUAIS_OK;
}

int gnuais_batch_protodec_reset(gnuais_batch *b)
{
    if (!b) return fail(GNUAIS_E_ARG, "protodec_reset: NULL batch");
    if (int rc = gnuais_batch_sync(b)) return rc;
    HIP_TRY(launch_hdlc_fsm_reset(b->ctl, b->N, nullptr));
    if (int rc = long_zero_state(b, false)) return rc;
    HIP_TRY(hipStreamSynchronize(nullptr));
    return GNUAIS_OK;
}

int gnuais_batch_frame_bits(gnuais_batch *b, int channel, uint8_t *h_bits, int cap, int *n_bits)
{
    if (!b || !h_bits || !n_bits || channel < 0 || channel >= b->N || cap < 0)
        return fail(GNUAIS_E_ARG, "frame_bits: argument");
    if (int rc = gnuais_batch_sync(b)) return rc;
    uint32_t w[HDLC_CTL_WORDS];
    for (int q = 0; q < HDLC_CTL_WORDS; ++q)
        HIP_TRY(hipMemcpy(&w[q], b->ctl + (size_t) q * (size_t) b->N + channel, 4, hipMemcpyDeviceToHost));
    *n_bits = -1;
    const uint32_t state = w[0] & 7, nstart = w[3];
    if (nstart == 0) return GNUAIS_OK;
    uint32_t rec[CAND_WORDS];
    HIP_TRY(hipMemcpy(rec, b->cand + ((size_t) channel * b->cand_K + (nstart - 1) % (uint32_t) b->cand_K) * CAND_WORDS,
                      sizeof rec, hipMemcpyDeviceToHost));
    int rawlen;
    const bool open = state == 4 || state == 5;
    if (open) {
        rawlen = (int) w[4];
        if ((rawlen >> 5) < CAND_WORDS - CAND_HDR) rec[CAND_HDR + (rawlen >> 5)] = w[1];
    } else if (rec[0] >> 17) {
        rawlen = (int) ((rec[0] >> 17) & 0x3ffu);
    } else {
        return GNUAIS_OK;
    }
    if (rawlen < 0 || rawlen > 32 * (CAND_WORDS - CAND_HDR)) return fail(GNUAIS_E_STATE, "frame_bits: record length");
    int n = 0, ones = 0;
    for (int i = 0; i < rawlen; ++i) {
        const uint8_t x = (rec[CAND_HDR + (i >> 5)] >> (i & 31)) & 1u;
        if (ones == 5) { ones = 0; continue; }
        if (n < cap) h_bits[n] = x;
        ++n;
        ones = x ? ones + 1 : 0;
    }
    *n_bits = n;
    return GNUAIS_OK;
}

int gnuais_batch_history(gnuais_batch *b, int16_t *h_out)
{
    if (!b || !h_out) return fail(GNUAIS_E_ARG, "history: argument");
    const int N = b->N, NT = b->NT;
    std::vector<int16_t> v;
    if (int rc = read_out(b, b->hist[b->hist_cur], (size_t) N * NT, v)) return rc;
    for (int c = 0; c < N; ++c)
        for (int k = 0; k < NT; ++k) h_out[(size_t) c * NT + k] = v[(size_t) k * N + c];
    return GNUAIS_OK;
}

int gnuais_batch_last_signs(gnuais_batch *b, uint8_t *h_out, int stride)
{
    if (!b || !h_out || stride < b->last_len) return fail(GNUAIS_E_ARG, "last_signs: argument");
    if (int rc = gnuais_batch_sync(b)) return rc;
    const int N = b->N, W = (b->last_len + 31) / 32;
    std::vector<uint32_t> w(sgn_words_alloc(W, N));
    if (W) HIP_TRY(hipMemcpy(w.data(), b->sgn[b->last_k], w.size() * 4, hipMemcpyDeviceToHost));
    for (int c = 0; c < N; ++c)
        for (int n = 0; n < b->last_len; ++n)
            h_out[(size_t) c * stride + n] = (w[sgn_index(n >> 5, N, c)] >> (31 - (n & 31))) & 1u;
    return GNUAIS_OK;
}

static int long_ring_capacity(const gnuais_batch *b)
{
    const uint64_t launch_bits = std::max((uint64_t) b->bits_words * 32, (uint64_t) b->seg_words * 32 * (uint64_t) b->n_seg);
    return (int) std::max<uint64_t>(256, (uint64_t) b->N * (launch_bits / 470 + 2));
}

int gnuais_batch_info(const gnuais_batch *b, const char *name, double *value)
{
    if (!b || !name || !value) return fail(GNUAIS_E_ARG, "info: argument");
    const SignChoice c = sign_choice(b->sign, b->fir, b->N);
    if (!strcmp(name, "sign_exact")) *value = c.exact;
    else if (!strcmp(name, "sign_eps")) *value = c.eps;
    else if (!strcmp(name, "sign_flag_scale")) *value = c.th.fscale;
    else if (!strcmp(name, "sign_eps_seen")) *value = c.th.eps_seen;
    else if (!strcmp(name, "sign_eps_ahead")) *value = c.th.eps_ahead;
    else if (!strcmp(name, "sign_matrix_pipe")) *value = c.matrix_pipe;
    else if (!strcmp(name, "sign_central_taps")) *value = c.th.NC;
    else if (!strcmp(name, "first_effective_tap")) *value = b->k0;
    else if (!strcmp(name, "n_effective_taps")) *value = b->NE;
    else if (!strcmp(name, "compute_units")) *value = b->n_cu;
    else if (!strcmp(name, "device")) *value = b->device;
    else if (!strcmp(name, "afc_window")) *value = b->afc_W;
    else if (!strcmp(name, "segments")) *value = b->n_seg;
    else if (!strcmp(name, "pack_bits")) *value = b->seg_words * 32;
    else if (!strcmp(name, "frame_times")) *value = b->frame_times;
    else if (!strcmp(name, "frame_signal")) *value = b->frame_signal;
    else if (!strcmp(name, "occupancy")) *value = b->occ_E;
    else if (!strcmp(name, "rows")) *value = (double) b->rows;
    else if (!strcmp(name, "pll_form")) *value = b->pll_form;
    else if (!strcmp(name, "repair")) *value = b->repair;
    else if (!strcmp(name, "long_frames")) *value = b->long_frames;
    else if (!strcmp(name, "long_frame_cap")) *value = b->long_cap ? b->long_cap : long_ring_capacity(b);
    else if (!strcmp(name, "long_repair")) *value = b->long_repair;
    else if (!strcmp(name, "long_cand_cap")) *value = b->long_cand_cap ? b->long_cand_cap : long_ring_capacity(b);
    else if (!strcmp(name, "unique")) *value = b->uq_window;
    else if (!strcmp(name, "unique_late")) *value = (double) b->uq_late;
    else if (!strncmp(name, "stream_of_stage_", 16) && name[16] >= '0' && name[16] <= '3' && !name[17]) {
        *value = -1;
        for (int q = 0; q < gnuais_batch::POOL; ++q)
            if (b->pool[q] == b->s_k[name[16] - '0']) *value = q;
    }
    else if (!strcmp(name, "stream_depth")) *value = gnuais_batch::NRING - 1;
    else return fail(GNUAIS_E_ARG, "info: unknown name");
    return GNUAIS_OK;
}

int gnuais_batch_frame_times(gnuais_batch *b, int on)
{
    if (!b) return fail(GNUAIS_E_ARG, "frame_times: NULL batch");
    if (b->streaming) return fail(GNUAIS_E_STATE, "frame_times: the batch is streaming (gnuais_batch_stream_nmea); "
                                                  "set_option(\"streaming\", 0) leaves that mode");
    if (!on && b->uq_window)
        return fail(GNUAIS_E_STATE, "frame_times: the batch merges duplicates by their times (gnuais_batch_unique); "
                                    "gnuais_batch_unique(b, 0) first");
    if (!on && b->frame_signal)
        return fail(GNUAIS_E_STATE, "frame_times: the batch finds its frames' spans by their times (gnuais_batch_frame_signal); "
                                    "gnuais_batch_frame_signal(b, 0) first");
    if (int rc = gnuais_batch_sync(b)) return rc;
    if (on && !b->frame_times) {
        HIP_TRY(b->times.ensure(sizeof(int64_t) * (size_t) b->frame_cap));
        HIP_TRY(hipMemset(b->times, 0xff, sizeof(int64_t) * (size_t) b->frame_cap));
    }
    b->frame_times = on != 0;
    return GNUAIS_OK;
}

int gnuais_batch_long_frames(gnuais_batch *b, int on)
{
    if (!b) return fail(GNUAIS_E_ARG, "long_frames: NULL batch");
    if (b->streaming) return fail(GNUAIS_E_STATE, "long_frames: the batch is streaming (gnuais_batch_stream_nmea); "
                                                  "set_option(\"streaming\", 0) leaves that mode");
    if (int rc = gnuais_batch_sync(b)) return rc;
    HIP_TRY(hipDeviceSynchronize());
    if (on && !b->long_ctl) {
        const size_t N = (size_t) b->N;
        b->long_cap = long_ring_capacity(b);
        HIP_TRY(b->long_open.ensure(sizeof(uint32_t) * N * LONG_REC_WORDS, true));
        HIP_TRY(b->long_counters.ensure(sizeof(int32_t) * N * 3, true));
        HIP_TRY(b->long_count.ensure(sizeof(uint32_t) * 2, true));
        HIP_TRY(b->long_ring.ensure(sizeof(gnuais_long_frame) * (size_t) b->long_cap));
        HIP_TRY(b->long_ctl.ensure(sizeof(uint32_t) * N * LONG_CTL_WORDS, true));
    }
    if (int rc = long_zero_state(b, true)) return rc;
    HIP_TRY(hipStreamSynchronize(nullptr));
    b->long_frames = on != 0;
    if (!on) b->long_repair = false;
    return GNUAIS_OK;
}

int gnuais_batch_long_repair(gnuais_batch *b, int on)
{
    if (!b) return fail(GNUAIS_E_ARG, "long_repair: NULL batch");
    if (b->streaming) return fail(GNUAIS_E_STATE, "long_repair: the batch is streaming (gnuais_batch_stream_nmea); "
                                                  "set_option(\"streaming\", 0) leaves that mode");
    if (!b->long_frames)
        return fail(GNUAIS_E_STATE, "long_repair: the batch does not decode long frames (gnuais_batch_long_frames): "
                                    "the repair works on what that decoder counts as failed");
    if (int rc = gnuais_batch_sync(b)) return rc;
    HIP_TRY(hipDeviceSynchronize());
    if (on && !b->long_cand) {
        const size_t N = (size_t) b->N;
        b->long_cand_cap = b->long_cap;
        HIP_TRY(b->long_clean.ensure(sizeof(uint32_t) * N * LONG_REC_WORDS, true));
        HIP_TRY(b->long_cand_count.ensure(sizeof(uint32_t) * 2, true));
        HIP_TRY(b->long_cand.ensure(sizeof(uint32_t) * (size_t) b->long_cand_cap * LONG_CAND_WORDS));
    }
    if (on) {
        HIP_TRY(hipMemset(b->long_cand_count, 0, sizeof(uint32_t) * 2));
        b->long_parity = 0;
    }
    b->long_repair = on != 0;
    return GNUAIS_OK;
}

int gnuais_batch_long_repaired(gnuais_batch *b, int32_t *h_out)
{
    if (!b || !h_out) return fail(GNUAIS_E_ARG, "long_repaired: argument");
    if (!b->long_ctl) return fail(GNUAIS_E_STATE, "long_repaired: the batch has never decoded long frames (gnuais_batch_long_frames)");
    std::vector<int32_t> v;
    if (int rc = read_out(b, b->long_counters, (size_t) b->N * 3, v)) return rc;
    memcpy(h_out, v.data() + 2 * (size_t) b->N, sizeof(int32_t) * (size_t) b->N);
    return GNUAIS_OK;
}

static_assert(sizeof(gnuais_long_frame) == 152 && sizeof(gnuais_long_frame) == 4 * LONG_FRAME_WORDS, "gnuais_long_frame layout");

static int long_pending(gnuais_batch *b, const char *who, uint32_t &have, bool &overflow)
{
    if (!b->long_ctl) {
        char msg[160];
        snprintf(msg, sizeof msg, "%s: the batch has never decoded long frames (gnuais_batch_long_frames)", who);
        return fail(GNUAIS_E_STATE, msg);
    }
    if (int rc = gnuais_batch_sync(b)) return rc;
    uint32_t cnt[2] = {0, 0};
    HIP_TRY(hipMemcpy(cnt, b->long_count, sizeof cnt, hipMemcpyDeviceToHost));
    have = std::min<uint32_t>(cnt[0], (uint32_t) b->long_cap);
    overflow = cnt[1] || cnt[0] > (uint32_t) b->long_cap;
    return GNUAIS_OK;
}

int gnuais_batch_pending_long_frames(gnuais_batch *b, int *n_out)
{
    if (!b || !n_out) return fail(GNUAIS_E_ARG, "pending_long_frames: argument");
    uint32_t have = 0;
    bool overflow = false;
    if (int rc = long_pending(b, "pending_long_frames", have, overflow)) return rc;
    *n_out = (int) have;
    return GNUAIS_OK;
}

int gnuais_batch_drain_long_frames(gnuais_batch *b, gnuais_long_frame *h_out, int max, int *n_out)
{
    if (!b || !n_out || max < 0 || (max && !h_out)) return fail(GNUAIS_E_ARG, "drain_long_frames: argument");
    *n_out = 0;
    uint32_t have = 0;
    bool overflow = false;
    if (int rc = long_pending(b, "drain_long_frames", have, overflow)) return rc;
    if ((uint32_t) max < have) return fail(GNUAIS_E_ARG, "drain_long_frames: frame buffer too small");
    if (have) {
        std::vector<gnuais_long_frame> v(have);
        HIP_TRY(hipMemcpy(v.data(), b->long_ring, sizeof(gnuais_long_frame) * have, hipMemcpyDeviceToHost));
        const auto stamp = [](const gnuais_long_frame &f) { return (uint64_t) f.end_bit | ((uint64_t) ((f.flags >> 1) & 31) << 32); };
        std::stable_sort(v.begin(), v.end(), [&](const gnuais_long_frame &x, const gnuais_long_frame &y) {
            return x.channel != y.channel ? x.channel < y.channel : stamp(x) < stamp(y);
        });
        memcpy(h_out, v.data(), sizeof(gnuais_long_frame) * have);
    }
    *n_out = (int) have;
    HIP_TRY(hipMemset(b->long_count, 0, sizeof(uint32_t) * 2));
    if (overflow) return fail(GNUAIS_E_OVERFLOW, "drain_long_frames: long-frame ring overflowed, frames were dropped");
    return GNUAIS_OK;
}

int gnuais_batch_long_counters(gnuais_batch *b, int32_t *h_delivered, int32_t *h_failed)
{
    if (!b || !h_delivered || !h_failed) return fail(GNUAIS_E_ARG, "long_counters: argument");
    if (!b->long_ctl) return fail(GNUAIS_E_STATE, "long_counters: the batch has never decoded long frames (gnuais_batch_long_frames)");
    std::vector<int32_t> v;
    if (int rc = read_out(b, b->long_counters, (size_t) b->N * 2, v)) return rc;
    memcpy(h_delivered, v.data(), sizeof(int32_t) * (size_t) b->N);
    memcpy(h_failed, v.data() + b->N, sizeof(int32_t) * (size_t) b->N);
    return GNUAIS_OK;
}

int gnuais_batch_long_fsm_state(gnuais_batch *b, gnuais_fsm_state *h_out)
{
    if (!b || !h_out) return fail(GNUAIS_E_ARG, "long_fsm_state: argument");
    if (!b->long_ctl) return fail(GNUAIS_E_STATE, "long_fsm_state: the batch has never decoded long frames (gnuais_batch_long_frames)");
    std::vector<uint32_t> v;
    if (int rc = read_out(b, b->long_ctl, (size_t) b->N, v)) return rc;
    for (int c = 0; c < b->N; ++c) {
        const uint32_t w = v[c];
        h_out[c].state = w & 7;
        h_out[c].nstartsign = (w >> 3) & 15;
        h_out[c].antallpreamble = (w >> 7) & 15;
        h_out[c].antallenner = (w >> 11) & 7;
        h_out[c].bitstuff = (w >> 14) & 1;
        h_out[c].last = (w >> 15) & 1;
        h_out[c].bufferpos = (w >> 16) & 2047;
    }
    return GNUAIS_OK;
}

int gnuais_batch_repair(gnuais_batch *b, int on)
{
    if (!b) return fail(GNUAIS_E_ARG, "repair: NULL batch");
    if (b->streaming) return fail(GNUAIS_E_STATE, "repair: the batch is streaming (gnuais_batch_stream_nmea); "
                                                  "set_option(\"streaming\", 0) leaves that mode");
    if (int rc = gnuais_batch_sync(b)) return rc;
    if (on) HIP_TRY(b->repaired.ensure(sizeof(int32_t) * (size_t) b->N, true));
    b->repair = on != 0;
    return GNUAIS_OK;
}

int gnuais_batch_unique(gnuais_batch *b, int window_rows)
{
    if (!b || window_rows < 0) return fail(GNUAIS_E_ARG, "unique: NULL batch or a negative window");
    if (b->streaming) return fail(GNUAIS_E_STATE, "unique: the batch is streaming (gnuais_batch_stream_nmea); "
                                                  "set_option(\"streaming\", 0) leaves that mode");
    if (window_rows && !b->frame_times)
        return fail(GNUAIS_E_STATE, "unique: the batch does not time its frames (gnuais_batch_frame_times): copies are "
                                    "merged by their receive times");
    if (int rc = gnuais_batch_sync(b)) return rc;
    b->uq_window = window_rows;
    b->uq_n_tail = 0;
    b->uq_late = 0;
    return GNUAIS_OK;
}

int gnuais_batch_unique_late(gnuais_batch *b, long long *late)
{
    if (!b || !late) return fail(GNUAIS_E_ARG, "unique_late: argument");
    *late = b->uq_late;
    return GNUAIS_OK;
}

int gnuais_batch_repaired(gnuais_batch *b, int32_t *h_out)
{
    if (!b || !h_out) return fail(GNUAIS_E_ARG, "repaired: argument");
    if (!b->repaired) {
        if (int rc = gnuais_batch_sync(b)) return rc;
        std::fill(h_out, h_out + b->N, 0);
        return GNUAIS_OK;
    }
    std::vector<int32_t> v;
    if (int rc = read_out(b, b->repaired, (size_t) b->N, v)) return rc;
    std::copy(v.begin(), v.end(), h_out);
    return GNUAIS_OK;
}

int gnuais_batch_time_map(const gnuais_batch *b, int kind, long long *mul, long long *off)
{
    if (!b || !mul || !off) return fail(GNUAIS_E_ARG, "time_map: argument");
    const long long d_f = (b->NT + 1) / 2, half_w = b->afc_W / 2;
    switch (kind) {
    case GNUAIS_INPUT_AUDIO:
        *mul = 1;
        *off = -d_f;
        return GNUAIS_OK;
    case GNUAIS_INPUT_IQ:
        *mul = 1;
        *off = -d_f - half_w;
        return GNUAIS_OK;
    case GNUAIS_INPUT_WIDEBAND: {
        if (!b->wide.K) return fail(GNUAIS_E_STATE, "time_map: no channeliser configured (gnuais_batch_channeliser)");
        if (b->wide.U > 1)
            return fail(GNUAIS_E_STATE, "time_map: the wide stage resamples by a ratio up / down with up > 1: use "
                                        "gnuais_batch_time_map_ratio");
        const long long D = b->wide.D, T = b->wide.T;
        *mul = D;
        *off = (-d_f - half_w) * D + D - 1 - (T - 1) / 2;
        return GNUAIS_OK;
    }
    default:
        return fail(GNUAIS_E_ARG, "time_map: kind must be GNUAIS_INPUT_AUDIO, _IQ or _WIDEBAND");
    }
}

int gnuais_batch_time_map_ratio(const gnuais_batch *b, int kind, long long *num, long long *den, long long *off)
{
    if (!b || !num || !den || !off) return fail(GNUAIS_E_ARG, "time_map_ratio: argument");
    if (kind != GNUAIS_INPUT_WIDEBAND || !b->wide.K || b->wide.U == 1) {
        *den = 1;
        return gnuais_batch_time_map(b, kind, num, off);
    }
    const long long d_f = (b->NT + 1) / 2, half_w = b->afc_W / 2, D = b->wide.D, T = b->wide.T;
    *num = D;
    *den = b->wide.U;
    *off = (-d_f - half_w) * D + D - 1 - (T - 1) / 2;
    return GNUAIS_OK;
}

int gnuais_batch_n_channels(const gnuais_batch *b) { return b ? b->N : 0; }
int gnuais_batch_n_taps(const gnuais_batch *b) { return b ? b->NT : 0; }

int gnuais_batch_set_timing(gnuais_batch *b, int on)
{
    if (!b) return fail(GNUAIS_E_ARG, "set_timing: NULL batch");
    b->timing = on != 0;
    if (on) b->timed_calls = 0;
    return GNUAIS_OK;
}

static int timing_of(gnuais_batch *b, unsigned long long call, float *ms)
{
    const Event *ev = b->evr[call % gnuais_batch::TIMING_RING];
    HIP_TRY(hipEventElapsedTime(&ms[0], ev[0], ev[1]));
    HIP_TRY(hipEventElapsedTime(&ms[1], ev[2], ev[6]));
    HIP_TRY(hipEventElapsedTime(&ms[2], ev[5], ev[7]));
    HIP_TRY(hipEventElapsedTime(&ms[3], ev[9], ev[4]));
    HIP_TRY(hipEventElapsedTime(&ms[4], ev[0], ev[4]));
    return GNUAIS_OK;
}

int gnuais_batch_last_timing(gnuais_batch *b, float *ms5)
{
    if (!b || !ms5) return fail(GNUAIS_E_ARG, "last_timing: argument");
    if (!b->timed_calls) return fail(GNUAIS_E_STATE, "last_timing: no timed run");
    if (int rc = gnuais_batch_sync(b)) return rc;
    return timing_of(b, b->timed_calls - 1, ms5);
}

int gnuais_batch_mean_timing(gnuais_batch *b, float *ms5, int *n_calls)
{
    if (!b || !ms5 || !n_calls) return fail(GNUAIS_E_ARG, "mean_timing: argument");
    if (!b->timed_calls) return fail(GNUAIS_E_STATE, "mean_timing: no timed run");
    if (int rc = gnuais_batch_sync(b)) return rc;
    const unsigned long long n = std::min<unsigned long long>(b->timed_calls, gnuais_batch::TIMING_RING);
    double acc[5] = {0, 0, 0, 0, 0};
    for (unsigned long long i = 0; i < n; ++i) {
        float t[5];
        if (int rc = timing_of(b, b->timed_calls - 1 - i, t)) return rc;
        for (int q = 0; q < 5; ++q) acc[q] += t[q];
    }
    for (int q = 0; q < 5; ++q) ms5[q] = (float) (acc[q] / (double) n);
    *n_calls = (int) n;
    return GNUAIS_OK;
}

int gnuais_crc16_batch(int device, const uint8_t *h_data, int stride, const int32_t *h_len,
                       int n_msgs, uint16_t *h_crc)
{
    if (!h_data || !h_len || !h_crc || stride <= 0 || n_msgs <= 0)
        return fail(GNUAIS_E_ARG, "crc16_batch: argument");
    HIP_TRY(hipSetDevice(device));
    Buf<uint8_t> d_data;
    Buf<int32_t> d_len;
    Buf<uint16_t> d_crc;
    hipError_t e = d_data.alloc((size_t) stride * n_msgs);
    if (e == hipSuccess) e = d_len.alloc(sizeof(int32_t) * n_msgs);
    if (e == hipSuccess) e = d_crc.alloc(sizeof(uint16_t) * n_msgs);
    if (e == hipSuccess) e = hipMemcpy(d_data, h_data, (size_t) stride * n_msgs, hipMemcpyHostToDevice);
    if (e == hipSuccess) e = hipMemcpy(d_len, h_len, sizeof(int32_t) * n_msgs, hipMemcpyHostToDevice);
    if (e == hipSuccess) e = launch_crc16(d_data, stride, d_len, n_msgs, d_crc, nullptr);
    if (e == hipSuccess) e = hipMemcpy(h_crc, d_crc, sizeof(uint16_t) * n_msgs, hipMemcpyDeviceToHost);
    if (e != hipSuccess) return fail(GNUAIS_E_HIP, "crc16_batch", e);
    return GNUAIS_OK;
}

int gnuais_crc16_bits(int device, const uint8_t *h_bits, int n_bytes, uint16_t *h_crc, uint8_t *h_msb, int n_out)
{
    if (!h_bits || !h_crc || n_bytes <= 0 || n_bytes > 64 || n_out < 0 || n_out > 8 * n_bytes || (n_out > 0 && !h_msb))
        return fail(GNUAIS_E_ARG, "crc16_bits: argument (1..64 bytes, n_out <= 8 * n_bytes)");
    HIP_TRY(hipSetDevice(device));
    Buf<uint8_t> d;
    hipError_t e = d.alloc(512 + 512 + 16);
    if (e == hipSuccess) e = hipMemcpy(d, h_bits, (size_t) n_bytes * 8, hipMemcpyHostToDevice);
    if (e == hipSuccess)
        e = launch_crc16_bits(d, n_bytes, reinterpret_cast<uint16_t *>(d + 1024), n_out ? d + 512 : nullptr, n_out, nullptr);
    if (e == hipSuccess) e = hipMemcpy(h_crc, d + 1024, sizeof(uint16_t), hipMemcpyDeviceToHost);
    if (e == hipSuccess && n_out) e = hipMemcpy(h_msb, d + 512, (size_t) n_out, hipMemcpyDeviceToHost);
    if (e != hipSuccess) return fail(GNUAIS_E_HIP, "crc16_bits", e);
    return GNUAIS_OK;
}

int gnuais_tile_channels(const int16_t *d_base, int n_base, int len, int16_t *d_out,
                         int n_channels, void *stream)
{
    if (!d_base || !d_out || n_base <= 0 || len <= 0 || n_channels <= 0)
        return fail(GNUAIS_E_ARG, "tile_channels: argument");
    HIP_TRY(launch_tile_channels(d_base, n_base, len, d_out, n_channels, (hipStream_t) stream));
    return GNUAIS_OK;
}

}
```

### gnuais_amd/csrc/hdlc_crc.hip

```cpp
#include <hip/hip_runtime.h>
#include <stdint.h>

#include "kernels.h"

namespace gnuais {

enum { ST_SKURR = 1, ST_PREAMBLE = 2, ST_STARTSIGN = 3, ST_DATA = 4, ST_STOPSIGN = 5 };

constexpr uint32_t CAND_VALID = 0x10000u;
constexpr int PACK_MAX = PACK_STRIDE;

__global__ void hdlc_reset_kernel(uint32_t *__restrict__ ctl, int N)
{
    const int c = blockIdx.x * blockDim.x + threadIdx.x;
    if (c >= N) return;
    ctl[c] = ST_SKURR;
    ctl[(size_t) N + c] = 0;
    ctl[(size_t) 2 * N + c] = 0;
    ctl[(size_t) 3 * N + c] = 0;
    ctl[(size_t) 4 * N + c] = 0;
    ctl[(size_t) 5 * N + c] = 0;
}

__global__ void hdlc_fsm_reset_kernel(uint32_t *__restrict__ ctl, int N)
{
    const int c = blockIdx.x * blockDim.x + threadIdx.x;
    if (c >= N) return;
    ctl[c] = ST_SKURR;
    ctl[(size_t) N + c] = 0;
    ctl[(size_t) 4 * N + c] = 0;
}

__device__ __forceinline__ uint32_t lowmask(int k)
{
    return k >= 32 ? ~0u : ((1u << k) - 1u);
}
__device__ __forceinline__ int ctz32(uint32_t v)
{
    return v ? __ffs((int) v) - 1 : 32;
}
__device__ __forceinline__ int clz32(uint32_t v)
{
    return v ? __clz((int) v) : 32;
}

__global__ __launch_bounds__(64) __attribute__((amdgpu_waves_per_eu(7, 8))) void hdlc_deframe_kernel(
    const uint32_t *__restrict__ segbits, const uint32_t *__restrict__ segcnt,
    uint32_t *__restrict__ ctl, uint32_t *__restrict__ cand, uint32_t *__restrict__ cand_first,
    uint32_t *__restrict__ cand_count, int32_t *__restrict__ counters,
    uint32_t *__restrict__ flags, int N, int n_seg, int seg_words, int K)
{
    __builtin_amdgcn_s_setprio(3);
    const int cg = blockIdx.x * blockDim.x + threadIdx.x;
    const bool live = cg < N;
    const size_t c = (size_t) (live ? cg : N - 1), n_ = (size_t) N;

    const uint32_t c0 = ctl[c];
    int state = c0 & 7, nstartsign = (c0 >> 3) & 15, antallpreamble = (c0 >> 7) & 15;
    int antallenner = (c0 >> 11) & 7, bitstuff = (c0 >> 14) & 1;
    uint32_t last = (c0 >> 15) & 1;
    int bufferpos = (c0 >> 16) & 511;
    uint32_t cur = ctl[n_ + c];
    const uint32_t seen0 = ctl[2 * n_ + c], seenhi0 = ctl[5 * n_ + c];
    uint32_t nstart = ctl[3 * n_ + c];
    int rawpos = (int) ctl[4 * n_ + c];
    int lost2 = 0;

    const bool open0 = (state == ST_DATA || state == ST_STOPSIGN);
    const uint32_t first = nstart - (open0 ? 1u : 0u);
    uint32_t *rec = cand + ((size_t) c * K + (open0 ? (nstart - 1) % (uint32_t) K : 0u)) * CAND_WORDS;
    bool rec_ok = open0;

    uint32_t seenbase = seen0;

#define HDLC_RESET()                                                                    \
    do { state = ST_SKURR; nstartsign = 0; antallpreamble = 0; antallenner = 0;        \
         last = 0; bitstuff = 0; bufferpos = 0; } while (0)

    extern __shared__ uint32_t lds_pack[];
    const int tpb = (int) blockDim.x, tx = (int) threadIdx.x;
    const uint32_t *__restrict__ rows = segbits + c * (size_t) n_seg * (size_t) PACK_STRIDE;
    uint32_t pf[PACK_MAX];
    int pf_cnt = live ? (int) segcnt[c * (size_t) n_seg] : 0;
#pragma unroll
    for (int q = 0; q < PACK_MAX / 4; ++q) {
        const uint4 v = reinterpret_cast<const uint4 *>(rows)[q];
        pf[4 * q] = v.x; pf[4 * q + 1] = v.y; pf[4 * q + 2] = v.z; pf[4 * q + 3] = v.w;
    }

    for (int seg = 0; seg < n_seg; ++seg) {
        int tile_end = pf_cnt;
        if (tile_end > seg_words * 32) tile_end = seg_words * 32;
#pragma unroll
        for (int q = 0; q < PACK_MAX; ++q) lds_pack[q * tpb + tx] = pf[q];
        lds_pack[PACK_MAX * tpb + tx] = 0;
        if (seg + 1 < n_seg) {
            const uint32_t *__restrict__ nrow = rows + (size_t) (seg + 1) * (size_t) PACK_STRIDE;
            pf_cnt = live ? (int) segcnt[c * (size_t) n_seg + seg + 1] : 0;
#pragma unroll
            for (int q = 0; q < PACK_MAX / 4; ++q) {
                const uint4 v = reinterpret_cast<const uint4 *>(nrow)[q];
                pf[4 * q] = v.x; pf[4 * q + 1] = v.y; pf[4 * q + 2] = v.z; pf[4 * q + 3] = v.w;
            }
        }
        int pos = 0;
#define FETCH_WINDOW()                                                                          \
        const int lw = pos >> 5, sh = pos & 31;                                                 \
        const uint32_t lo = lds_pack[lw * tpb + tx], hi = lds_pack[(lw + 1) * tpb + tx];        \
        const uint32_t W = sh ? ((lo >> sh) | (hi << (32 - sh))) : lo;   \
        const int nv = (tile_end - pos < 32) ? tile_end - pos : 32

        while (__any(pos < tile_end)) {
            while (__any(pos < tile_end && state == ST_SKURR)) {
                if (pos < tile_end && state == ST_SKURR) {
                    FETCH_WINDOW();
                    const uint32_t vm = lowmask(nv);
                    const uint32_t A = W ^ ((W << 1) | last);
                    const uint32_t B2 = A & (A << 1), B4 = B2 & (B2 << 2), B8 = B4 & (B4 << 4);
                    const uint32_t B15 = B8 & (B8 << 7);
                    const int t = ctz32(~A);
                    const int need = 14 - antallpreamble;
                    const uint32_t C = lowmask(t) & ~lowmask(need > 0 ? need : 0);
                    const uint32_t TR = (B15 | C) & ~W & vm;
                    if (TR) {
                        pos += ctz32(TR) + 1;
                        state = ST_PREAMBLE;
                        antallpreamble = 0;
                        last = 0;
                    } else {
                        pos += nv;
                        last = (W >> (nv - 1)) & 1u;
                        const int ap = (t >= nv) ? antallpreamble + nv : clz32(~(A << (32 - nv)));
                        antallpreamble = ap > 15 ? 15 : ap;
                    }
                }
            }
            while (__any(pos < tile_end && state != ST_SKURR && state != ST_DATA)) {
                if (pos < tile_end && state != ST_SKURR && state != ST_DATA) {
                    FETCH_WINDOW();
                    int k = 0;
                    if (state == ST_STOPSIGN) {
                        const uint32_t x = W & 1u;
                        const int nb = bufferpos - 6 - 16;
                        if (x == 0 && nb > 0) {
                            if (rec_ok) {
                                rec[CAND_HDR + (rawpos >> 5)] = cur;
                                const uint32_t eb = seenbase + (uint32_t) pos;
                                const uint32_t ebhi = (seenhi0 + (eb < seen0 ? 1u : 0u)) & 31u;
                                rec[1] = eb;
                                rec[0] = (uint32_t) nb | CAND_VALID | ((uint32_t) rawpos << 17) | (ebhi << 27);
                            }
                        } else {
                            ++lost2;
                            if (rec_ok) {
                                rec[CAND_HDR + (rawpos >> 5)] = cur;
                                rec[0] = (uint32_t) rawpos << 17;
                            }
                        }
                        HDLC_RESET();
                        last = x;
                        k = 1;
                    } else if (state != ST_PREAMBLE && state != ST_STARTSIGN) {
                        HDLC_RESET();
                        last = W & 1u;
                        k = 1;
                    } else {
                        if (state == ST_PREAMBLE && nstartsign == 0) {
                            const uint32_t A = W ^ ((W << 1) | last);
                            int t = ctz32(~A);
                            if (t > nv) t = nv;
                            if (t > 0) {
                                antallpreamble = antallpreamble + t > 15 ? 15 : antallpreamble + t;
                                last = (W >> (t - 1)) & 1u;
                                k = t;
                            }
                            if (k < nv) {
                                const uint32_t x0 = (W >> k) & 1u;
                                nstartsign = x0 ? 3 : 1;
                                last = x0;
                                ++k;
                            }
                        }
                        if (k < nv && nstartsign != 0) {
                            const int R = 7 - nstartsign;
                            const int avail = nv - k;
                            int L = ctz32(~(W >> k));
                            if (L > avail) L = avail;
                            if (L >= R + 1) {
                                HDLC_RESET(); nstartsign = 1; last = 1; k += R + 1;
                            } else if (L < avail) {
                                if (L == R) {
                                    state = ST_DATA; nstartsign = 1; antallenner = 0; antallpreamble = 0;
                                    bufferpos = 0; cur = 0; rawpos = 0; bitstuff = 0; last = 0;
                                    rec_ok = (nstart - first) < (uint32_t) K;
                                    rec = cand + ((size_t) c * K + nstart % (uint32_t) K) * CAND_WORDS;
                                    if (rec_ok) rec[0] = 0; else flags[1] = 1;
                                    ++nstart;
                                } else if (L == R - 1) {
                                    HDLC_RESET(); nstartsign = 1; last = 0;
                                } else {
                                    HDLC_RESET(); last = 0;
                                }
                                k += L + 1;
                            } else {
                                nstartsign += L;
                                if (nstartsign >= 6) { state = ST_STARTSIGN; antallpreamble = 0; }
                                last = 1;
                                k += L;
                            }
                        }
                    }
                    pos += k;
                }
            }
            while (__any(pos < tile_end && state == ST_DATA)) {
                if (pos < tile_end && state == ST_DATA) {
                    FETCH_WINDOW();
                    if (bitstuff) {
                        const uint32_t x = W & 1u;
                        if (x) {
                            state = ST_STOPSIGN;
                        } else {
                            if ((rawpos & 31) == 31) {
                                if (rec_ok) rec[CAND_HDR + (rawpos >> 5)] = cur;
                                cur = 0;
                            }
                            ++rawpos;
                        }
                        bitstuff = 0;
                        last = x;
                        pos += 1;
                    } else {
                        const int m = last ? antallenner + 1 : 0;
                        const int room = 449 - bufferpos;
                        int nw = nv;
                        if (nw > 32 - m) nw = 32 - m;
                        if (nw > room) nw = room;
                        const int nvE = nw + m;
                        const uint32_t vmE = lowmask(nvE);
                        const uint32_t E = ((W << m) | lowmask(m)) & vmE;
                        const uint32_t X1 = E & (E >> 1), X2 = X1 & (X1 >> 2);
                        const uint32_t R5 = X2 & (E >> 4);
                        const uint32_t S5 = R5 & ~(E << 1);
                        const uint32_t P5 = S5 << 4;
                        const uint32_t nx = E >> 1, kn = vmE >> 1;
                        const uint32_t END5 = P5 & nx & kn;
                        const uint32_t STF5 = P5 & ~nx & kn;
                        const uint32_t PND5 = P5 & ~kn;
                        int nraw, stored;
                        if (END5) {
                            const int pe = ctz32(END5);
                            nraw = pe + 1 - m;
                            stored = nraw - __popc(STF5 & lowmask(pe));
                        } else {
                            nraw = nw;
                            stored = nw - __popc(STF5);
                        }
                        {
                            const uint32_t sb = W & lowmask(nraw);
                            const int bsh = rawpos & 31;
                            const uint64_t t64 = (uint64_t) sb << bsh;
                            cur |= (uint32_t) t64;
                            if (bsh + nraw >= 32) {
                                if (rec_ok) rec[CAND_HDR + (rawpos >> 5)] = cur;
                                cur = (uint32_t) (t64 >> 32);
                            }
                            rawpos += nraw;
                        }
                        bufferpos += stored;
                        if (END5) {
                            pos += nraw + 1;
                            state = ST_STOPSIGN;
                            antallenner = 0;
                            last = 1;
                        } else {
                            pos += nraw;
                            const uint32_t xl = (W >> (nraw - 1)) & 1u;
                            if (bufferpos >= 449) {
                                if (rec_ok) rec[0] = 0;
                                HDLC_RESET();
                                last = xl;
                            } else if (PND5) {
                                bitstuff = 1;
                                antallenner = 0;
                                last = 1;
                            } else {
                                const int r = clz32(~(E << (32 - nvE)));
                                last = xl;
                                antallenner = r > 0 ? r - 1 : 0;
                            }
                        }
                    }
                }
            }
        }
#undef FETCH_WINDOW
        seenbase += (uint32_t) tile_end;
    }
#undef HDLC_RESET

    if (live) {
        ctl[c] = (uint32_t) state | ((uint32_t) nstartsign << 3) | ((uint32_t) antallpreamble << 7) |
                 ((uint32_t) antallenner << 11) | ((uint32_t) bitstuff << 14) | (last << 15) |
                 ((uint32_t) bufferpos << 16);
        ctl[n_ + c] = cur;
        ctl[2 * n_ + c] = seenbase;
        ctl[5 * n_ + c] = seenhi0 + (seenbase < seen0 ? 1u : 0u);
        ctl[3 * n_ + c] = nstart;
        ctl[4 * n_ + c] = (uint32_t) rawpos;
        const bool open1 = (state == ST_DATA || state == ST_STOPSIGN);
        const uint32_t limit = nstart - (open1 ? 1u : 0u);
        cand_first[c] = first;
        uint32_t cnt = limit - first;
        cand_count[c] = cnt > (uint32_t) K ? (uint32_t) K : cnt;
        if (lost2) counters[2 * n_ + c] += lost2;
    }
}

__global__ __launch_bounds__(256) void hdlc_crc_kernel(
    const uint32_t *__restrict__ cand, const uint32_t *__restrict__ cand_first,
    const uint32_t *__restrict__ cand_count, int32_t *__restrict__ counters,
    uint32_t *__restrict__ frames, uint32_t *__restrict__ flags, uint32_t frame_cap, int N, int K,
    uint2 *__restrict__ chunks, int n_pass)
{
    __shared__ uint32_t tab[256];
    __shared__ uint32_t pre[K3_CH + 1];
    extern __shared__ uint32_t k3_dyn[];
    uint32_t (*const stage)[HDLC_BUF_WORDS + 1] = reinterpret_cast<uint32_t (*)[HDLC_BUF_WORDS + 1]>(k3_dyn);
    uint32_t (*const rawlds)[CAND_WORDS - CAND_HDR + 1] =
        reinterpret_cast<uint32_t (*)[CAND_WORDS - CAND_HDR + 1]>(k3_dyn + 256 * (HDLC_BUF_WORDS + 1));
    __shared__ uint32_t wave_cnt[4];
    __shared__ uint32_t pass_base;
    const int tid = threadIdx.x;
    const int c_own = blockIdx.x * K3_CH + tid;

    {
        uint32_t t = (uint32_t) tid;
#pragma unroll
        for (int k = 0; k < 8; ++k) t = (t >> 1) ^ ((t & 1u) ? 0x8408u : 0u);
        tab[tid] = t;
    }
    if (tid < K3_CH) pre[tid + 1] = (c_own < N) ? cand_count[c_own] : 0u;
    __syncthreads();
    if (tid == 0) {
        uint32_t run = 0;
        pre[0] = 0;
        for (int q = 1; q <= K3_CH; ++q) { run += pre[q]; pre[q] = run; }
    }
    __syncthreads();
    const uint32_t total = pre[K3_CH];
    const size_t n_ = (size_t) N;

    int pass = 0;
    for (uint32_t i0 = 0; i0 < total; i0 += 256, ++pass) {
        const uint32_t i = i0 + (uint32_t) tid;
        bool good = false;
        uint32_t out[16];
#pragma unroll
        for (int q = 0; q < 16; ++q) out[q] = 0;
        if (i < total) {
            int lo = 0, hi = K3_CH - 1;
            while (lo < hi) {
                const int mid = (lo + hi + 1) >> 1;
                if (pre[mid] <= i) lo = mid; else hi = mid - 1;
            }
            const int c = blockIdx.x * K3_CH + lo;
            const uint32_t j = i - pre[lo];
            const uint32_t slot = (cand_first[c] + j) % (uint32_t) K;
            const uint32_t *rec = cand + ((size_t) c * K + slot) * CAND_WORDS;
            const uint32_t hdr = rec[0];
            if (hdr & CAND_VALID) {
                const int n = (int) (hdr & 0xffffu);
                const int rawlen = (int) ((hdr >> 17) & 0x3ffu);
                const int nbytes = n >> 3, buflen = nbytes + 2;
                {
                    uint32_t raw[CAND_WORDS - CAND_HDR];
#pragma unroll
                    for (int q = 0; q < CAND_WORDS - CAND_HDR; ++q) raw[q] = rec[CAND_HDR + q];
#pragma unroll
                    for (int q = 0; q < CAND_WORDS - CAND_HDR; ++q) rawlds[tid][q] = raw[q];
                    unsigned long long acc = 0;
                    uint32_t prevw = 0;
                    int fill = 0, ow = 0;
                    const int nwords = (rawlen + 31) >> 5;
#pragma unroll 1
                    for (int q = 0; q < nwords; ++q) {
                        uint32_t rw = rawlds[tid][q];
                        const int nvq = rawlen - 32 * q < 32 ? rawlen - 32 * q : 32;
                        const unsigned long long cc = ((unsigned long long) rw << 32) | prevw;
                        const uint32_t five = (uint32_t) (cc >> 31) & (uint32_t) (cc >> 30) & (uint32_t) (cc >> 29) &
                                              (uint32_t) (cc >> 28) & (uint32_t) (cc >> 27);
                        uint32_t stf = five & ~rw & (nvq >= 32 ? ~0u : (1u << nvq) - 1u);
                        prevw = rw;
                        int nout = nvq;
                        while (stf) {
                            const int pz = 31 - __clz((int) stf);
                            stf &= ~(1u << pz);
                            rw = (rw & ((1u << pz) - 1u)) | ((pz >= 31 ? 0u : rw >> (pz + 1)) << pz);
                            --nout;
                        }
                        if (nout < 32) rw &= (1u << nout) - 1u;
                        acc |= (unsigned long long) rw << fill;
                        fill += nout;
                        if (fill >= 32) {
                            if (ow <= HDLC_BUF_WORDS) stage[tid][ow] = (uint32_t) acc;
                            ++ow;
                            acc >>= 32;
                            fill -= 32;
                        }
                    }
                    if (ow <= HDLC_BUF_WORDS) stage[tid][ow] = (uint32_t) acc;
                    for (int q = ow + 1; q <= HDLC_BUF_WORDS; ++q) stage[tid][q] = 0;
                }
                uint32_t w[HDLC_BUF_WORDS];
#pragma unroll
                for (int q = 0; q < HDLC_BUF_WORDS; ++q) w[q] = stage[tid][q];
                uint32_t crc = 0xffffu;
#pragma unroll
                for (int q = 0; q < HDLC_BUF_WORDS; ++q) {
#pragma unroll
                    for (int bq = 0; bq < 4; ++bq) {
                        if (q * 4 + bq < buflen) {
                            const uint32_t byte = (w[q] >> (8 * bq)) & 0xffu;
                            crc = (crc >> 8) ^ tab[(crc ^ byte) & 0xffu];
                        }
                    }
                }
                if (crc == 0xf0b8u) {
                    good = true;
                    atomicAdd(&counters[c], 1);
                    out[0] = (uint32_t) c;
                    out[1] = rec[1];
#pragma unroll
                    for (int q = 0; q < 14; ++q) {
                        uint32_t v = 0;
                        if (q * 4 < nbytes) {
                            v = w[q];
                            const int keep = nbytes - q * 4;
                            if (keep < 4) v &= (1u << (8 * keep)) - 1u;
                        }
                        if (q == 13) v = (v & 0xffu) | ((1u | ((hdr >> 27) << 1)) << 8) | ((uint32_t) n << 16);
                        out[2 + q] = v;
                    }
                } else {
                    atomicAdd(&counters[n_ + c], 1);
                }
            }
        }
        const unsigned long long m = __ballot(good);
        const int wave = tid >> 6, lane = tid & 63;
        const uint32_t below = (uint32_t) __popcll(m & ((1ull << lane) - 1ull));
        if (lane == 0) wave_cnt[wave] = (uint32_t) __popcll(m);
        __syncthreads();
        uint32_t woff = 0, npass = 0;
#pragma unroll
        for (int q = 0; q < 4; ++q) {
            if (q < wave) woff += wave_cnt[q];
            npass += wave_cnt[q];
        }
        if (tid == 0) {
            const uint32_t base = npass ? atomicAdd(&flags[0], npass) : 0u;
            pass_base = base;
            if (chunks && pass < n_pass)
                chunks[(size_t) blockIdx.x * n_pass + pass] =
                    make_uint2(base, base >= frame_cap ? 0u : (npass < frame_cap - base ? npass : frame_cap - base));
        }
        __syncthreads();
        if (good) {
            const uint32_t idx = pass_base + woff + below;
            if (idx < frame_cap) {
                uint4 *dst = reinterpret_cast<uint4 *>(frames + (size_t) idx * 16);
                dst[0] = make_uint4(out[0], out[1], out[2], out[3]);
                dst[1] = make_uint4(out[4], out[5], out[6], out[7]);
                dst[2] = make_uint4(out[8], out[9], out[10], out[11]);
                dst[3] = make_uint4(out[12], out[13], out[14], out[15]);
            } else {
                flags[1] = 1;
            }
        }
        __syncthreads();
    }
    if (chunks)
        for (int q = pass + tid; q < n_pass; q += 256) chunks[(size_t) blockIdx.x * n_pass + q] = make_uint2(0u, 0u);
}

hipError_t launch_hdlc_deframe(const HdlcLaunch &a, hipStream_t stream)
{
    const int lpw = a.lanes_per_wave > 0 ? a.lanes_per_wave : 64;
    if (a.seg_words > PACK_MAX) return hipErrorInvalidValue;
    hipLaunchKernelGGL(hdlc_deframe_kernel, dim3((a.N + lpw - 1) / lpw), dim3(lpw),
                       (PACK_MAX + 1) * lpw * sizeof(uint32_t), stream,
                       a.segbits, a.segcnt, a.ctl, a.cand, a.cand_first, a.cand_count, a.counters,
                       a.frame_count, a.N, a.n_seg, a.seg_words, a.K);
    return hipGetLastError();
}

hipError_t launch_hdlc_crc(const HdlcLaunch &a, hipStream_t stream)
{
    constexpr size_t K3_DYN_LDS = 256 * ((HDLC_BUF_WORDS + 1) + (CAND_WORDS - CAND_HDR + 1)) * sizeof(uint32_t);
    hipLaunchKernelGGL(hdlc_crc_kernel, dim3((unsigned) ((a.N + K3_CH - 1) / K3_CH)), dim3(256), K3_DYN_LDS,
                       stream, a.cand, a.cand_first, a.cand_count, a.counters,
                       (uint32_t *) a.frames, a.frame_count, a.frame_cap, a.N, a.K, a.chunks, k3_passes(a.K_call > 0 ? a.K_call : a.K));
    return hipGetLastError();
}

hipError_t launch_hdlc_fsm_reset(uint32_t *ctl, int N, hipStream_t stream)
{
    hipLaunchKernelGGL(hdlc_fsm_reset_kernel, dim3((N + 255) / 256), dim3(256), 0, stream, ctl, N);
    return hipGetLastError();
}

hipError_t launch_hdlc_reset(uint32_t *ctl, int N, hipStream_t stream)
{
    hipLaunchKernelGGL(hdlc_reset_kernel, dim3((N + 255) / 256), dim3(256), 0, stream, ctl, N);
    return hipGetLastError();
}

}
```

### gnuais_amd/csrc/hdlc_events.hip

```cpp
#include <hip/hip_runtime.h>
#include <stdint.h>

#include "kernels.h"

namespace gnuais {

namespace {

enum { ST_SKURR = 1, ST_PREAMBLE = 2, ST_STARTSIGN = 3, ST_DATA = 4, ST_STOPSIGN = 5 };
constexpr uint32_t CAND_VALID = 0x10000u;
constexpr int EW = PACK_STRIDE;
constexpr int NONE = 1 << 20;

__device__ __forceinline__ uint32_t lowmask(int k) { return k >= 32 ? ~0u : k <= 0 ? 0u : ((1u << k) - 1u); }
__device__ __forceinline__ int ctz32(uint32_t v) { return v ? __ffs((int) v) - 1 : 32; }
__device__ __forceinline__ int clz32(uint32_t v) { return v ? __clz((int) v) : 32; }
__device__ __forceinline__ int wave_max_i(int v, int lanes, int lane)
{
#pragma unroll
    for (int o = 32; o; o >>= 1) {
        const int u = __shfl_xor(v, o);
        v = ((lane ^ o) < lanes && u > v) ? u : v;
    }
    return v;
}

}

constexpr int EV_ROWS = (EW + 2) + 4 * EW + (EW + 1);

template <int TPB>
__global__ __launch_bounds__(64) void hdlc_events_kernel(
    const uint32_t *__restrict__ segbits, const uint32_t *__restrict__ segcnt,
    uint32_t *__restrict__ ctl, uint32_t *__restrict__ cand, uint32_t *__restrict__ cand_first,
    uint32_t *__restrict__ cand_count, int32_t *__restrict__ counters,
    uint32_t *__restrict__ flags, int N, int n_seg, int seg_words, int K)
{
    __builtin_amdgcn_s_setprio(3);
    extern __shared__ uint32_t lds[];
    const int tpb = TPB > 0 ? TPB : (int) blockDim.x, tx = (int) threadIdx.x;
    const int cg = blockIdx.x * blockDim.x + threadIdx.x;
    const bool live = cg < N;
    const size_t c = (size_t) (live ? cg : N - 1), n_ = (size_t) N;
    uint32_t *const Xa = lds + tx, *const NAa = Xa + (EW + 2) * tpb, *const CBa = NAa + EW * tpb,
                   *const E6a = CBa + EW * tpb, *const SFa = E6a + EW * tpb, *const PSa = SFa + EW * tpb;
#define XW(q) Xa[((q) + 1) * tpb]

    const uint32_t c0 = ctl[c];
    int state = c0 & 7, nstartsign = (c0 >> 3) & 15, antallpreamble = (c0 >> 7) & 15;
    int antallenner = (c0 >> 11) & 7, bitstuff = (c0 >> 14) & 1;
    uint32_t last = (c0 >> 15) & 1;
    int bufferpos = (c0 >> 16) & 511;
    uint32_t cur = ctl[n_ + c];
    const uint32_t seen0 = ctl[2 * n_ + c], seenhi0 = ctl[5 * n_ + c];
    uint32_t nstart = ctl[3 * n_ + c];
    int rawpos = (int) ctl[4 * n_ + c];
    int lost2 = 0;

    const bool open0 = (state == ST_DATA || state == ST_STOPSIGN);
    const uint32_t first = nstart - (open0 ? 1u : 0u);
    uint32_t *rec = cand + ((size_t) c * K + (open0 ? (nstart - 1) % (uint32_t) K : 0u)) * CAND_WORDS;
    bool rec_ok = open0;
    uint32_t seenbase = seen0;

#define HDLC_RESET()                                                                    \
    do { state = ST_SKURR; nstartsign = 0; antallpreamble = 0; antallenner = 0;        \
         last = 0; bitstuff = 0; bufferpos = 0; } while (0)
#define ENTER_DATA()                                                                    \
    do { state = ST_DATA; nstartsign = 1; antallenner = 0; antallpreamble = 0;         \
         bufferpos = 0; cur = 0; rawpos = 0; bitstuff = 0; last = 0;                    \
         rec_ok = (nstart - first) < (uint32_t) K;                                      \
         rec = cand + ((size_t) c * K + nstart % (uint32_t) K) * CAND_WORDS;            \
         if (rec_ok) rec[0] = 0; else flags[1] = 1;                                     \
         ++nstart; } while (0)
#define RAW_APPEND(v_, n_bits_)                                                         \
    do { const uint32_t sb_ = (v_); const int nb_ = (n_bits_), bsh_ = rawpos & 31;      \
         const uint64_t t64_ = (uint64_t) sb_ << bsh_;                                  \
         cur |= (uint32_t) t64_;                                                        \
         if (bsh_ + nb_ >= 32) {                                                        \
             if (rec_ok) rec[CAND_HDR + (rawpos >> 5)] = cur;                           \
             cur = (uint32_t) (t64_ >> 32);                                             \
         }                                                                              \
         rawpos += nb_; } while (0)
#define STOP_BIT(x_, at_)                                                               \
    do { const int nb_ = bufferpos - 6 - 16;                                            \
         if ((x_) == 0 && nb_ > 0) {                                                    \
             if (rec_ok) {                                                              \
                 const uint32_t eb_ = seenbase + (uint32_t) (at_);                      \
                 const uint32_t ebhi_ = (seenhi0 + (eb_ < seen0 ? 1u : 0u)) & 31u;      \
                 rec[CAND_HDR + (rawpos >> 5)] = cur;                                   \
                 rec[1] = eb_;                                                          \
                 rec[0] = (uint32_t) nb_ | CAND_VALID | ((uint32_t) rawpos << 17) | (ebhi_ << 27); \
             }                                                                          \
         } else {                                                                       \
             ++lost2;                                                                   \
             if (rec_ok) {       \
                 rec[CAND_HDR + (rawpos >> 5)] = cur;                                   \
                 rec[0] = (uint32_t) rawpos << 17;                                      \
             }                                                                          \
         }                                                                              \
         HDLC_RESET();                                                                  \
         last = (x_); } while (0)

    auto slow_bit = [&](uint32_t x, int at) {
        int ns_v = nstartsign, bp_v = bufferpos;
        {
        int nstartsign = ns_v, bufferpos = bp_v;
        switch (state) {
        case ST_DATA:
            if (bitstuff) {
                if (x == 1) {
                    state = ST_STOPSIGN;
                } else {
                    RAW_APPEND(0u, 1);
                }
                bitstuff = 0;
            } else {
                if (x == last && x == 1) {
                    if (++antallenner == 4) { bitstuff = 1; antallenner = 0; }
                } else {
                    antallenner = 0;
                }
                RAW_APPEND(x, 1);
                if (++bufferpos >= 449) {
                    if (rec_ok) rec[0] = 0;
                    HDLC_RESET();
                }
            }
            break;
        case ST_SKURR:
            antallpreamble = (x != last) ? (antallpreamble < 15 ? antallpreamble + 1 : 15) : 0;
            if (antallpreamble > 14 && x == 0) { state = ST_PREAMBLE; antallpreamble = 0; }
            break;
        case ST_PREAMBLE:
            if (x != last && nstartsign == 0) {
                antallpreamble = antallpreamble < 15 ? antallpreamble + 1 : 15;
            } else if (x == 1) {
                if (nstartsign == 0) nstartsign = 3;
                else if (nstartsign == 5) { nstartsign = 6; antallpreamble = 0; state = ST_STARTSIGN; }
                else ++nstartsign;
            } else {
                if (nstartsign == 0) nstartsign = 1; else HDLC_RESET();
            }
            break;
        case ST_STARTSIGN:
            if (nstartsign >= 7) {
                if (x == 0) { ENTER_DATA(); nstartsign = 0; } else HDLC_RESET();
            } else if (x == 0) {
                HDLC_RESET();
            }
            ++nstartsign;
            if (nstartsign > 15) nstartsign = 15;
            break;
        case ST_STOPSIGN:
            STOP_BIT(x, at);
            break;
        default:
            HDLC_RESET();
            break;
        }
        ns_v = nstartsign; bp_v = bufferpos;
        }
        nstartsign = ns_v; bufferpos = bp_v;
        last = x;
    };

    const uint32_t *__restrict__ rows = segbits + c * (size_t) n_seg * (size_t) PACK_STRIDE;
    uint32_t pf[EW];
    int pf_cnt = 0;
    bool pf_ready = false;
    auto fetch = [&](int seg) {
        const uint32_t *__restrict__ row = rows + (size_t) seg * (size_t) PACK_STRIDE;
        {
            pf_cnt = live ? (int) segcnt[c * (size_t) n_seg + seg] : 0;
#pragma unroll
            for (int q = 0; q < EW / 4; ++q) {
                const uint4 v = reinterpret_cast<const uint4 *>(row)[q];
                pf[4 * q] = v.x; pf[4 * q + 1] = v.y; pf[4 * q + 2] = v.z; pf[4 * q + 3] = v.w;
            }
        }
        pf_ready = true;
    };

    for (int seg = 0; seg < n_seg; ++seg) {
        if (!pf_ready) fetch(seg);
        int tile_end = pf_cnt;
        if (tile_end > seg_words * 32) tile_end = seg_words * 32;

        const int m_in = (state == ST_DATA) ? (bitstuff ? 5 : (last ? antallenner + 1 : 0)) : 0;
        uint32_t prevw = (state == ST_DATA) ? (m_in ? ~0u << (32 - m_in) : 0u) : (last << 31);
        uint32_t ps = 0, nzNA = 0, nzCB = 0, nzE6 = 0;
        XW(-1) = prevw;
#pragma unroll
        for (int q = 0; q < EW; ++q) XW(q) = pf[q];
        pf_ready = false;
        if (seg + 1 < n_seg) fetch(seg + 1);
        const int nwq = __builtin_amdgcn_readfirstlane((int) wave_max_i((tile_end + 31) >> 5, tpb, tx));
        auto shl_in = [](uint32_t v, uint32_t below, int n) -> uint32_t {
            return __builtin_amdgcn_alignbit(v, below, 32 - n);
        };
        uint32_t pA = 0, pa2 = 0, pa4 = 0, pa8 = 0;
        uint32_t pu2 = prevw & (prevw << 1);
        uint32_t pt = (pu2 & (pu2 << 2)) & (prevw << 4);
#pragma unroll
        for (int q = 0; q < EW; ++q) {
            if (q >= nwq) {
                XW(q) = 0; NAa[q * tpb] = 0; CBa[q * tpb] = 0; E6a[q * tpb] = 0; SFa[q * tpb] = 0; PSa[q * tpb] = ps;
                continue;
            }
            const uint32_t vm = lowmask(tile_end - 32 * q);
            const uint32_t xw = XW(q) & vm;
            const uint32_t A = (xw ^ shl_in(xw, prevw, 1)) & vm;
            const uint32_t a2 = A & shl_in(A, pA, 1), a4 = a2 & shl_in(a2, pa2, 2), a8 = a4 & shl_in(a4, pa4, 4);
            const uint32_t a15 = a8 & shl_in(a8, pa8, 7);
            const uint32_t u2 = xw & shl_in(xw, prevw, 1), u4 = u2 & shl_in(u2, pu2, 2);
            const uint32_t t5 = u4 & shl_in(xw, prevw, 4);
            const uint32_t na = ~A & vm, cb = a15 & ~xw & vm;
            const uint32_t e6 = u4 & shl_in(u2, pu2, 4) & vm;
            const uint32_t sf = shl_in(t5, pt, 1) & ~xw & vm;
            XW(q) = xw;
            NAa[q * tpb] = na;
            CBa[q * tpb] = cb;
            E6a[q * tpb] = e6;
            SFa[q * tpb] = sf;
            PSa[q * tpb] = ps;
            ps += (uint32_t) __popc(sf);
            nzNA |= (na < 1u ? na : 1u) << q;
            nzCB |= (cb < 1u ? cb : 1u) << q;
            nzE6 |= (e6 < 1u ? e6 : 1u) << q;
            pA = A; pa2 = a2; pa4 = a4; pa8 = a8; pu2 = u2; pt = t5;
            prevw = xw;
        }
        XW(EW) = 0;
        PSa[EW * tpb] = ps;

        auto first_set = [&](const uint32_t *arr, uint32_t nz, int p) -> int {
            if (p >= tile_end) return NONE;
            const int q = p >> 5;
            const uint32_t m = arr[q * tpb] & (~0u << (p & 31));
            if (m) return 32 * q + ctz32(m);
            const uint32_t rest = q >= 31 ? 0u : nz & (~0u << (q + 1));
            if (!rest) return NONE;
            const int q2 = ctz32(rest);
            return 32 * q2 + ctz32(arr[q2 * tpb]);
        };
        auto bit_at = [&](int p) -> uint32_t { return (XW(p >> 5) >> (p & 31)) & 1u; };
        auto window = [&](int p) -> uint32_t {
            const int q = p >> 5, sh = p & 31;
            const uint32_t lo = XW(q), hi = XW(q + 1 <= EW ? q + 1 : EW);
            return sh ? ((lo >> sh) | (hi << (32 - sh))) : lo;
        };
        auto stuffed = [&](int a, int b) -> int {
            if (b <= a) return 0;
            const int qa = a >> 5, qb = b >> 5;
            int n = (int) PSa[qb * tpb] - (int) PSa[qa * tpb];
            n -= __popc(SFa[qa * tpb] & lowmask(a & 31));
            if (qb < EW) n += __popc(SFa[qb * tpb] & lowmask(b & 31));
            return n;
        };

        int pos = 0;
        int rs = -1;
        bool hunt0 = true;
        bool slow = false;

        auto hunt = [&]() {
            int trig = NONE;
            if (rs < 0 && hunt0) {
                const int t0 = first_set(NAa, nzNA, 0);
                int k0 = 14 - antallpreamble;
                if (k0 < 0) k0 = 0;
                const int lim = t0 < tile_end ? t0 : tile_end;
                if (k0 < lim && bit_at(k0)) ++k0;
                if (k0 < lim) trig = k0;
                const int cb = first_set(CBa, nzCB, 0);
                if (cb < trig) trig = cb;
            } else {
                const int from = rs + 15 > pos ? rs + 15 : pos;
                trig = first_set(CBa, nzCB, from);
            }
            if (trig < tile_end) {
                state = ST_PREAMBLE;
                antallpreamble = 0;
                last = 0;
                pos = trig + 1;
            } else {
                int lastna = -1;
                for (uint32_t nz = nzNA; nz;) {
                    const int q = 31 - clz32(nz);
                    const uint32_t m = NAa[q * tpb];
                    lastna = 32 * q + 31 - clz32(m);
                    break;
                }
                int ap;
                if (rs < 0 && hunt0) ap = lastna < 0 ? antallpreamble + tile_end : tile_end - 1 - lastna;
                else {
                    const int since = tile_end - 1 - rs, run = tile_end - 1 - lastna;
                    ap = since < run ? since : run;
                }
                antallpreamble = ap > 15 ? 15 : ap;
                last = bit_at(tile_end - 1);
                pos = tile_end;
            }
        };

        while (__any(pos < tile_end)) {
            if (pos < tile_end) {
                if (state == ST_SKURR && !slow) hunt();
                if (state == ST_PREAMBLE && nstartsign == 0 && pos < tile_end && !slow) {
                    const int j = first_set(NAa, nzNA, pos);
                    if (j >= tile_end) {
                        const int ap = antallpreamble + (tile_end - pos);
                        antallpreamble = ap > 15 ? 15 : ap;
                        last = bit_at(tile_end - 1);
                        pos = tile_end;
                    } else {
                        const int ap = antallpreamble + (j - pos);
                        antallpreamble = ap > 15 ? 15 : ap;
                        const uint32_t xj = bit_at(j);
                        nstartsign = xj ? 3 : 1;
                        last = xj;
                        pos = j + 1;
                    }
                }
                if (((state == ST_PREAMBLE && nstartsign != 0) || state == ST_STARTSIGN) && pos < tile_end && !slow) {
                    const uint32_t W = window(pos);
                    const int avail = tile_end - pos < 32 ? tile_end - pos : 32;
                    const int R = 7 - nstartsign;
                    int Lr = ctz32(~W);
                    if (Lr > avail) Lr = avail;
                    if (R < 0) {
                        slow = true;
                    } else if (Lr >= R + 1) {
                        HDLC_RESET(); nstartsign = 1; last = 1;
                        rs = pos + R; hunt0 = false;
                        pos += R + 1;
                    } else if (Lr < avail) {
                        if (Lr == R) {
                            ENTER_DATA();
                            pos += Lr + 1;
                        } else if (Lr == R - 1) {
                            HDLC_RESET(); nstartsign = 1; last = 0;
                            rs = pos + Lr; hunt0 = false;
                            pos += Lr + 1;
                        } else {
                            HDLC_RESET(); last = 0;
                            rs = pos + Lr; hunt0 = false;
                            pos += Lr + 1;
                        }
                    } else {
                        nstartsign += Lr;
                        if (nstartsign >= 6) { state = ST_STARTSIGN; antallpreamble = 0; }
                        last = 1;
                        pos += Lr;
                    }
                }
                if (state == ST_DATA && pos < tile_end && !slow) {
                    const int e6 = first_set(E6a, nzE6, pos);
                    const int e = e6 < tile_end ? e6 : tile_end;
                    const int stored = (e - pos) - stuffed(pos, e);
                    if (bufferpos + stored >= 449) {
                        int need = 449 - bufferpos, p = pos, t = pos;
                        for (;;) {
                            const int q = p >> 5;
                            const int we = (32 * (q + 1) < e) ? 32 * (q + 1) : e;
                            uint32_t m = ~SFa[q * tpb] & (~0u << (p & 31)) & lowmask(we - 32 * q);
                            const int n = __popc(m);
                            if (n >= need) {
                                for (int k = 1; k < need; ++k) m &= m - 1;
                                t = 32 * q + ctz32(m);
                                break;
                            }
                            need -= n;
                            p = we;
                        }
                        if (rec_ok) rec[0] = 0;
                        const uint32_t xt = bit_at(t);
                        HDLC_RESET();
                        last = xt;
                        rs = t; hunt0 = false;
                        pos = t + 1;
                    } else {
                        for (int p = pos; p < e;) {
                            const int sh = p & 31;
                            const int take = (32 - sh < e - p) ? 32 - sh : e - p;
                            RAW_APPEND((XW(p >> 5) >> sh) & lowmask(take), take);
                            p += take;
                        }
                        bufferpos += stored;
                        if (e6 < tile_end) {
                            state = ST_STOPSIGN;
                            antallenner = 0;
                            bitstuff = 0;
                            last = 1;
                            pos = e6 + 1;
                        } else {
                            int r;
                            if (tile_end >= 8) {
                                r = clz32(~(window(tile_end - 8) << 24));
                            } else {
                                r = clz32(~((XW(0) << (32 - tile_end)) | (XW(-1) >> tile_end)));
                            }
                            last = bit_at(tile_end - 1);
                            if (r >= 5) { bitstuff = 1; antallenner = 0; }
                            else { bitstuff = 0; antallenner = r > 0 ? r - 1 : 0; }
                            pos = tile_end;
                        }
                    }
                }
                if (state == ST_STOPSIGN && pos < tile_end && !slow) {
                    const uint32_t x = bit_at(pos);
                    STOP_BIT(x, pos);
                    rs = pos; hunt0 = false;
                    pos += 1;
                }
                if (pos < tile_end && (slow || state < ST_SKURR || state > ST_STOPSIGN)) {
                    const int st0 = state;
                    const uint32_t x = bit_at(pos);
                    slow_bit(x, pos);
                    if (state == ST_SKURR && st0 != ST_SKURR) { rs = pos; hunt0 = false; }
                    if (state != st0) slow = false;
                    pos += 1;
                }
                if (state == ST_SKURR && !slow && pos < tile_end) hunt();
            }
        }
        seenbase += (uint32_t) tile_end;
    }
#undef XW
#undef HDLC_RESET
#undef ENTER_DATA
#undef RAW_APPEND
#undef STOP_BIT

    if (live) {
        ctl[c] = (uint32_t) state | ((uint32_t) nstartsign << 3) | ((uint32_t) antallpreamble << 7) |
                 ((uint32_t) antallenner << 11) | ((uint32_t) bitstuff << 14) | (last << 15) |
                 ((uint32_t) bufferpos << 16);
        ctl[n_ + c] = cur;
        ctl[2 * n_ + c] = seenbase;
        ctl[5 * n_ + c] = seenhi0 + (seenbase < seen0 ? 1u : 0u);
        ctl[3 * n_ + c] = nstart;
        ctl[4 * n_ + c] = (uint32_t) rawpos;
        const bool open1 = (state == ST_DATA || state == ST_STOPSIGN);
        const uint32_t limit = nstart - (open1 ? 1u : 0u);
        cand_first[c] = first;
        uint32_t cnt = limit - first;
        cand_count[c] = cnt > (uint32_t) K ? (uint32_t) K : cnt;
        if (lost2) counters[2 * n_ + c] += lost2;
    }
}

hipError_t launch_hdlc_events(const HdlcLaunch &a, hipStream_t stream)
{
    if (a.seg_words > PACK_STRIDE) return hipErrorInvalidValue;
    const int lpw = a.lanes_per_wave >= 1 && a.lanes_per_wave <= 64 ? a.lanes_per_wave : 64;
    const dim3 grid((a.N + lpw - 1) / lpw), block(lpw);
    const size_t lds = EV_ROWS * lpw * sizeof(uint32_t);
#define EV_LAUNCH(T)                                                                                                  \
    hipLaunchKernelGGL(hdlc_events_kernel<T>, grid, block, lds, stream, a.segbits, a.segcnt, a.ctl, a.cand, a.cand_first, \
                       a.cand_count, a.counters, a.frame_count, a.N, a.n_seg, a.seg_words, a.K)
    switch (lpw) {
    case 8: EV_LAUNCH(8); break;
    case 16: EV_LAUNCH(16); break;
    case 32: EV_LAUNCH(32); break;
    case 64: EV_LAUNCH(64); break;
    default: EV_LAUNCH(0); break;
    }
#undef EV_LAUNCH
    return hipGetLastError();
}

}
```

### gnuais_amd/csrc/kernels.h

```cpp
#pragma once
#include <hip/hip_runtime.h>
#include <stdint.h>

#include "fir_plan.h"

namespace gnuais {

struct FirLaunch : FirThresholds {
    const int16_t *x;
    const int16_t *hist;
    uint32_t *sgn;
    float *dump;
    int *maxval;
    int16_t *hist_out;
    int *maxval_next;
    const float *d_taps;
    float te[64];
    int N, L;
    int NT, NE, d;
    float ctaps[48];
    const float *te_mem;
    int map;
    int max_segments = 0;
    const struct MfmaTaps *mfma = nullptr;
};
int launch_fir_sign_quantum(int NC);
hipError_t launch_fir_sign(const FirLaunch &a, hipStream_t stream);
int launch_fir_sign_pk_quantum(int NC);
struct alignas(16) MfmaTaps { int a[3][3][64][4]; int k0; };
void fir_sign_mfma_pack(const int *tq48, long tq_sum, MfmaTaps *out);
hipError_t launch_fir_sign_mfma(const FirLaunch &a, int first, hipStream_t stream);
hipError_t launch_fir_sign_pk(const FirLaunch &a, hipStream_t stream);
hipError_t launch_fir_generic(const FirLaunch &a, hipStream_t stream);
hipError_t launch_fir_history(const int16_t *x, const int16_t *hist_in, int16_t *hist_out,
                              int N, int L, int NT, hipStream_t stream);

constexpr int PLL_LDS_BYTES = 81 * 1024;
constexpr int SEG_WORDS = 64;
constexpr int SEG_LEN = SEG_WORDS * 32;
constexpr int PACK_STRIDE = 16;
__host__ __device__ inline size_t sgn_index(int w, int N, int c)
{
    return ((size_t) (w >> 2) * (size_t) N + (size_t) c) * 4 + (size_t) (w & 3);
}
__host__ __device__ inline size_t sgn_words_alloc(int W, int N)
{
    return (size_t) ((W + 3) / 4 + 1) * 4 * (size_t) N;
}
struct PllLaunch {
    const uint32_t *sgn;
    uint32_t *pll;
    uint32_t *prev;
    uint32_t *lastbit;
    uint32_t *watchdog;
    uint32_t *segbits;
    uint32_t *segcnt;
    int N, L, n_seg, seg_words;
    uint32_t pllinc;
    int n_cu;
    int variant = 0;
};
int pll_form_of(const PllLaunch &a);
int pll_need_lds();
hipError_t pll_prepare_device();
hipError_t launch_pll(const PllLaunch &a, hipStream_t stream);
bool pll_tp_applicable(const PllLaunch &a);
hipError_t launch_pll_tp(const PllLaunch &a, hipStream_t stream);
constexpr int PLL_TP_MAX_CHANNELS = 1536;

constexpr int HDLC_CTL_WORDS = 6;
constexpr int HDLC_BUF_WORDS = 15;
constexpr int CAND_HDR = 2;
constexpr int CAND_WORDS = 20;
struct HdlcLaunch {
    const uint32_t *segbits;
    const uint32_t *segcnt;
    uint32_t *ctl;
    uint32_t *cand;
    uint32_t *cand_first;
    uint32_t *cand_count;
    int32_t *counters;
    void *frames;
    uint32_t *frame_count;
    uint32_t frame_cap;
    int N, n_seg, seg_words, K;
    int K_call = 0;
    int lanes_per_wave;
    uint2 *chunks = nullptr;
};
constexpr int K3_CH = 32;
inline int k3_blocks(int N) { return (N + K3_CH - 1) / K3_CH; }
inline int k3_passes(int K) { return (K3_CH * K + 255) / 256; }
hipError_t launch_hdlc_deframe(const HdlcLaunch &a, hipStream_t stream);
hipError_t launch_hdlc_events(const HdlcLaunch &a, hipStream_t stream);
hipError_t launch_hdlc_crc(const HdlcLaunch &a, hipStream_t stream);
hipError_t launch_hdlc_reset(uint32_t *ctl, int N, hipStream_t stream);
hipError_t launch_hdlc_fsm_reset(uint32_t *ctl, int N, hipStream_t stream);

struct FrameTimeLaunch {
    const void *frames;
    const uint32_t *frame_count;
    uint32_t frame_cap;
    const uint32_t *ctl;
    const uint32_t *segcnt;
    int64_t *times;
    int N, n_seg, seg_words;
    int len;
    int64_t n0;
};
hipError_t launch_frame_times(const FrameTimeLaunch &a, hipStream_t stream);
hipError_t launch_frame_times_gather(const int64_t *times, const uint32_t *order, int n, int64_t *out, hipStream_t stream);

hipError_t launch_iq_power(const int16_t *iq, uint32_t *carry, int64_t *ring, int RB, int N, int len,
                           unsigned long long n0, bool first, hipStream_t stream);
struct FrameSignalLaunch {
    const void *frames;
    const uint32_t *frame_count;
    uint32_t frame_cap;
    const int64_t *times;
    const int64_t *ring;
    void *signal;
    int RB, N;
    int len;
    int64_t n0;
    uint32_t pllinc;
    int n_taps, afc_window;
    int64_t v0;
};
hipError_t launch_frame_signal(const FrameSignalLaunch &a, hipStream_t stream);

hipError_t launch_occ_code(const int64_t *sums, int RB, uint16_t *codes, int CB, int N, long long j0, int count,
                           hipStream_t stream);
struct OccCoverLaunch {
    const void *frames;
    const uint32_t *frame_count;
    uint32_t frame_cap;
    const int64_t *times;
    uint8_t *cover;
    int CB, N;
    int len;
    int64_t n0;
    uint32_t pllinc;
    int n_taps, afc_window;
    int64_t v0, b0;
};
hipError_t launch_occ_cover(const OccCoverLaunch &a, hipStream_t stream);
struct OccEpochLaunch {
    uint16_t *codes;
    uint8_t *cover;
    uint8_t *carry;
    void *out;
    int CB, N, E, margin;
    int64_t first;
    bool first_epoch;
};
hipError_t launch_occ_epoch(const OccEpochLaunch &a, hipStream_t stream);

hipError_t launch_tile_channels(const int16_t *base, int n_base, int len, int16_t *out,
                                int n_channels, hipStream_t stream);
hipError_t launch_crc16(const uint8_t *data, int stride, const int32_t *len, int n,
                        uint16_t *crc, hipStream_t stream);
hipError_t launch_crc16_bits(const uint8_t *bits, int n_bytes, uint16_t *crc, uint8_t *msb, int n_out,
                             hipStream_t stream);

constexpr int IQ_DISC_ROWS = 64;
hipError_t launch_iq_discriminator(const int16_t *iq, int16_t *out, int16_t *carry, int N, int len, hipStream_t stream);

constexpr int AFC_BLOCK = 64;
constexpr int AFC_MIN_WINDOW = 128, AFC_MAX_WINDOW = 16384;
hipError_t launch_iq_discriminator_afc(const int16_t *iq, int16_t *out, int16_t *carry, int N, int len, int64_t *blk,
                                       int nb, unsigned long long n0, hipStream_t stream);
hipError_t launch_afc_estimate(const int64_t *blk, int nb, int N, int16_t *est, long long j_lo, int n_est, int W,
                               hipStream_t stream);
hipError_t launch_afc_apply(const int16_t *audio, int16_t *delay, const int16_t *est, long long j_lo, int16_t *out, int N,
                            int len, int W, unsigned long long n0, hipStream_t stream);

constexpr int CHAN_MAX_K = 32;
struct WideLaunch {
    const void *in;
    uint32_t *out;
    const uint32_t *hist;
    const uint32_t *mix;
    const uint32_t *poly;
    const int16_t *taps;
    int M, K, D, T, len;
    int NA;
    int n_groups, seg_rows;
    int per[CHAN_MAX_K], off[CHAN_MAX_K];
    int ph0[CHAN_MAX_K];
    const int32_t *groups;
    int U, H;
};
hipError_t launch_wide(const WideLaunch &a, int fmt, uint32_t *hist_out, hipStream_t stream);
template <int F, bool RATIONAL> hipError_t wide_fast_launch(const WideLaunch &a, dim3 grid, hipStream_t stream);
template <int F> void wide_direct_launch(const WideLaunch &a, dim3 grid, hipStream_t stream);
template <int F> void wide_carry_launch(const WideLaunch &a, uint32_t *hist_out, hipStream_t stream);

size_t nmea_scratch_bytes(int n_frames, int n_chunks = 0);
hipError_t frames_sort(const struct gnuais_frame *frames, int n, struct gnuais_frame *out, void *scratch,
                       size_t scratch_bytes, hipStream_t s);
hipError_t frames_sort_timed(const struct gnuais_frame *frames, const int64_t *times, int n, struct gnuais_frame *out,
                             int64_t *times_out, void *scratch, size_t scratch_bytes, hipStream_t s,
                             const int64_t *words = nullptr, int64_t *words_out = nullptr);
hipError_t nmea_format_enqueue(const struct gnuais_frame *frames, int n, int n_max, int n_channels,
                               const uint8_t *seq_in, uint8_t *seq_out, char *out, size_t out_cap, void *scratch,
                               size_t scratch_bytes, uint32_t *h_info4, const uint2 *chunks, int n_chunks,
                               int chunk_passes, uint32_t **totals_dev, hipStream_t s);
hipError_t nmea_slot_info_enqueue(const uint32_t *totals, const uint32_t *ring_count, uint32_t *info8_dev, hipStream_t s);
hipError_t nmea_text_copy_enqueue(const char *src, const uint32_t *info8_dev, char *dst_pinned, size_t dst_cap,
                                  uint32_t *info8_pinned, int workgroups, hipStream_t s);
size_t messages_line_bytes();
hipError_t messages_format_enqueue(const struct gnuais_frame *frames, int n, int n_channels, const uint8_t *seq_in,
                                   const char *chanid_dev, void *scratch, size_t scratch_bytes, char *lines,
                                   uint32_t *len, uint32_t *off, char *out, size_t out_cap, uint32_t *info2,
                                   hipStream_t s);
hipError_t vessels_fold_enqueue(const struct gnuais_frame *frames, int n, void *scratch, size_t scratch_bytes,
                                struct gnuais_vessel *out, int cap, uint32_t *count_dev, hipStream_t s);
size_t vessel_table_bytes(uint32_t slots);
hipError_t vessel_table_update_enqueue(const struct gnuais_frame *frames, const uint32_t *count, int n_max, void *table,
                                       uint32_t slots, uint32_t *fslot, hipStream_t s);
hipError_t vessel_table_fetch(const void *table, uint32_t slots, struct gnuais_vessel *h_out, int max, int *n_out,
                              uint32_t h_info[4], hipStream_t s);
hipError_t nmea_format(const struct gnuais_frame *frames, int n, int n_channels, const uint8_t *seq_in,
                       uint8_t *seq_out, char *out, size_t out_cap, void *scratch, size_t scratch_bytes,
                       uint32_t *h_info, hipStream_t s);

struct RepairLaunch {
    const uint32_t *cand;
    const uint32_t *cand_first;
    const uint32_t *cand_count;
    int32_t *repaired;
    void *frames;
    uint32_t *frame_count;
    uint32_t frame_cap;
    int N, K;
};
hipError_t launch_hdlc_repair(const RepairLaunch &a, hipStream_t stream);

constexpr int LONG_CTL_WORDS = 3;
constexpr int LONG_REC_WORDS = 40;
constexpr int LONG_FRAME_WORDS = 38;
constexpr int LONG_LIMIT_BITS = 1031;
constexpr int LONG_SHORT_BITS = 426;
struct LongLaunch {
    const uint32_t *segbits;
    const uint32_t *segcnt;
    const uint32_t *ctl;
    uint32_t *lctl;
    uint32_t *open;
    int32_t *counters;
    void *frames;
    uint32_t *frame_count;
    uint32_t frame_cap;
    int N, n_seg, seg_words;
    int len;
    int64_t n0;
    uint32_t *clean = nullptr;
    uint32_t *cand = nullptr;
    uint32_t *cand_count = nullptr;
    uint32_t cand_cap = 0;
    int parity = 0;
};
hipError_t launch_hdlc_long(const LongLaunch &a, hipStream_t stream);
hipError_t launch_hdlc_long_reset(uint32_t *lctl, int32_t *counters, int N, hipStream_t stream);

constexpr int LONG_CAND_HDR = 6;
constexpr int LONG_CAND_WORDS = LONG_CAND_HDR + LONG_REC_WORDS;
struct LongRepairLaunch {
    const uint32_t *cand;
    const uint32_t *cand_count;
    uint32_t cand_cap;
    int32_t *repaired;
    void *frames;
    uint32_t *frame_count;
    uint32_t frame_cap;
    int N;
    int blocks;
};
hipError_t launch_hdlc_long_repair(const LongRepairLaunch &a, hipStream_t stream);

constexpr int UNIQUE_INFO_COLLISION = 0;
constexpr int UNIQUE_INFO_CLUSTERS = 1;
constexpr int UNIQUE_INFO_PRIMARIES = 2;
constexpr int UNIQUE_INFO_TAIL = 3;
constexpr int UNIQUE_INFO_LATE = 4;
constexpr int UNIQUE_INFO_WORDS = 8;
struct UniqueLaunch {
    const void *frames;
    const int64_t *times;
    int have;
    const void *tail;
    int n_tail;
    void *tail_out;
    long long window, rows;
    int hash_bits;
    int ch_bits, time_bits;
    void *scratch;
    size_t scratch_bytes;
    struct gnuais_frame *out_frames;
    int64_t *out_times;
    int32_t *out_copies;
    const void *signal = nullptr;
    void *heard_scratch = nullptr;
    size_t heard_scratch_bytes = 0;
    int32_t *out_first = nullptr;
    struct gnuais_hearer *out_members = nullptr;
};
size_t unique_scratch_bytes(int n_entries);
size_t unique_heard_scratch_bytes(int have);
uint32_t *unique_info(void *scratch);
hipError_t unique_cluster_enqueue(const UniqueLaunch &a, bool exact, hipStream_t s);
hipError_t unique_deliver_enqueue(const UniqueLaunch &a, int n_primaries, hipStream_t s);

}
```

Baseline: 1.695 million Msamples/s.

## Fold frame-ring discard into deframer launch and slice CRC with prefetched candidates

Frame-ring discard becomes a deferred flag. Its memset is folded into the deframer kernel's first thread, with a parity-tagged overflow mark, and an env-controlled cycle mode can skip the deframer-to-CRC event handoff when both stages share a stream. The CRC kernel now uses a slice-by-4 table, a wave-shuffle scan of candidate counts, 16-byte vector loads of whole candidate records with one-pass-ahead prefetch, and builds the output record only for accepted frames. The aim is to remove a memset launch and an event record per call and to cut CRC kernel latency. In exchange the discard state machine gets more complex, with ordering risk if a discard is pending while other APIs run.

```diff
diff --git a/gnuais_amd/csrc/batch.h b/gnuais_amd/csrc/batch.h
--- a/gnuais_amd/csrc/batch.h
+++ b/gnuais_amd/csrc/batch.h
@@ -146,6 +146,10 @@
     Buf<uint2> ring_chunks[NRING];
     int ring_runs[NRING] = {};
     int n_chunks = 0;
+    bool discard_pending = false;
+    hipStream_t discard_stream = nullptr;
+    unsigned discard_launches = 0;
+    int cycle_parts = 3;
     bool frame_times = false;
     unsigned long long rows = 0;
     bool clock_fresh = true;
@@ -245,6 +249,7 @@
 int drain(gnuais_batch *b, unsigned stages, hipStream_t s);
 hipStream_t k3_stream(const gnuais_batch *b);
 hipStream_t behind_k3(const gnuais_batch *b);
+int discard_flush(gnuais_batch *b);
 double now_ms();
 int chan_zero_state(gnuais_batch *b);
 int afc_zero_state(gnuais_batch *b);
diff --git a/gnuais_amd/csrc/capi_delivery.hip b/gnuais_amd/csrc/capi_delivery.hip
--- a/gnuais_amd/csrc/capi_delivery.hip
+++ b/gnuais_amd/csrc/capi_delivery.hip
@@ -1,4 +1,13 @@
 #include "batch.h"
+
+int gnuais::discard_flush(gnuais_batch *b)
+{
+    if (!b->discard_pending) return GNUAIS_OK;
+    b->discard_pending = false;
+    hipStream_t s = b->pipeline ? k3_stream(b) : b->discard_stream;
+    HIP_TRY(hipMemsetAsync(b->ring_count[0], 0, sizeof(uint32_t) * 3, s));
+    return GNUAIS_OK;
+}
 
 extern "C" {
 
@@ -17,6 +26,7 @@
 
 static int read_pending(gnuais_batch *b, Pending &p)
 {
+    if (int rc = discard_flush(b)) return rc;
     if (int rc = gnuais_batch_sync(b)) return rc;
     uint32_t cnt[4] = {0, 0, 0, 0};
     HIP_TRY(hipMemcpy(cnt, b->ring_count[0], sizeof cnt, hipMemcpyDeviceToHost));
@@ -200,6 +210,7 @@
 {
     if (!b || !b->vt) return fail(GNUAIS_E_STATE, "vessel_table_update: no table (gnuais_batch_vessel_table_enable)");
     if (b->streaming) return fail(GNUAIS_E_STATE, "vessel_table_update: a streaming batch updates its table by itself");
+    if (int rc = discard_flush(b)) return rc;
     if (int rc = gnuais_batch_sync(b)) return rc;
     HIP_TRY(vessel_table_update_enqueue(b->ring[0], b->ring_count[0], b->frame_cap, b->vt, b->vt_slots, b->vt_fslot, behind_k3(b)));
     return GNUAIS_OK;
@@ -390,6 +401,7 @@
                                                   "streamed delivery has no such stage");
     if (b->long_frames) return fail(GNUAIS_E_STATE, "stream_nmea: the batch decodes long frames (gnuais_batch_long_frames); "
                                                     "the streamed delivery carries no records of them");
+    if (int rc = discard_flush(b)) return rc;
     if (int rc = gnuais_batch_sync(b)) return rc;
     for (int q = 1; q < NR; ++q) {
         HIP_TRY(b->ring[q].ensure(sizeof(gnuais_frame) * (size_t) b->frame_cap));
@@ -514,8 +526,10 @@
     if (!b) return fail(GNUAIS_E_ARG, "discard_frames: NULL batch");
     if (b->streaming) return fail(GNUAIS_E_STATE, "discard_frames: the batch is streaming (gnuais_batch_stream_nmea)");
     if (int rc = set_device(b)) return rc;
-    hipStream_t s = b->pipeline ? k3_stream(b) : (hipStream_t) stream;
-    HIP_TRY(hipMemsetAsync(b->ring_count[0], 0, sizeof(uint32_t) * 3, s));
+    b->discard_stream = (hipStream_t) stream;
+    b->discard_pending = true;
+    if (!(b->cycle_parts & 1))
+        if (int rc = discard_flush(b)) return rc;
     b->hdlc_calls = 0;
     return GNUAIS_OK;
 }
diff --git a/gnuais_amd/csrc/crc_sliced.h b/gnuais_amd/csrc/crc_sliced.h
--- /dev/null
+++ b/gnuais_amd/csrc/crc_sliced.h
@@ -0,0 +1,49 @@
+#pragma once
+#include <stdint.h>
+
+#if defined(__HIPCC__) || defined(__CUDACC__)
+#define CRC_HD __host__ __device__ inline
+#else
+#define CRC_HD inline
+#endif
+
+namespace gnuais {
+namespace crc {
+
+constexpr uint32_t POLY = 0x8408u;
+constexpr int SLICES = 4;
+
+CRC_HD uint32_t advance8(uint32_t b)
+{
+    for (int s = 0; s < 8; ++s) b = (b >> 1) ^ ((b & 1u) ? POLY : 0u);
+    return b;
+}
+
+CRC_HD uint16_t sliced_entry(int k, uint32_t b)
+{
+    for (int s = 0; s <= k; ++s) b = advance8(b);
+    return (uint16_t) b;
+}
+
+CRC_HD uint32_t step1(uint32_t crc, uint32_t byte, const uint16_t *tab)
+{
+    return (crc >> 8) ^ tab[(crc ^ byte) & 0xffu];
+}
+
+CRC_HD uint32_t step4(uint32_t crc, uint32_t word, const uint16_t *tab)
+{
+    const uint32_t v = crc ^ word;
+    return (uint32_t) tab[3 * 256 + (v & 0xffu)] ^ (uint32_t) tab[2 * 256 + ((v >> 8) & 0xffu)] ^
+           (uint32_t) tab[256 + ((v >> 16) & 0xffu)] ^ (uint32_t) tab[v >> 24];
+}
+
+CRC_HD uint32_t run_words(uint32_t crc, const uint32_t *w, int n, const uint16_t *tab)
+{
+    int q = 0;
+    for (; 4 * q + 4 <= n; ++q) crc = step4(crc, w[q], tab);
+    for (int k = 4 * q; k < n; ++k) crc = step1(crc, (w[k >> 2] >> (8 * (k & 3))) & 0xffu, tab);
+    return crc;
+}
+
+}
+}
diff --git a/gnuais_amd/csrc/gnuais_capi.hip b/gnuais_amd/csrc/gnuais_capi.hip
--- a/gnuais_amd/csrc/gnuais_capi.hip
+++ b/gnuais_amd/csrc/gnuais_capi.hip
@@ -231,6 +231,7 @@
             if (e == hipSuccess) e = b->pool[made].ensure(made < 8 ? hi : 0);
     }
     if (const char *v = getenv("GNUAIS_K3_SAME")) b->k3_same = atoi(v) != 0;
+    if (const char *v = getenv("GNUAIS_CYCLE")) b->cycle_parts = atoi(v) & 3;
     if (const char *v = getenv("GNUAIS_PLL_VARIANT")) {
         const int pv = atoi(v);
         if (pv == 0 || pv == 7 || pv == 8) b->pll_variant = pv;
@@ -267,6 +268,7 @@
     }
     b->ring_cur = 0;
     b->stream_calls = 0;
+    b->discard_pending = false;
     return GNUAIS_OK;
 }
 
@@ -294,6 +296,7 @@
     if (!b) return fail(GNUAIS_E_ARG, "reset: NULL batch");
     if (int rc = set_device(b)) return rc;
     const size_t N = (size_t) b->N;
+    if (int rc = discard_flush(b)) return rc;
     HIP_TRY(hipDeviceSynchronize());
     for (int q = 0; q < gnuais_batch::HB; ++q)
         HIP_TRY(hipMemset(b->hist[q], 0, sizeof(int16_t) * N * b->NT));
@@ -410,6 +413,7 @@
         if (value < 1) return fail(GNUAIS_E_ARG, "timing_stride must be >= 1");
         b->timing_stride = value;
     } else if (!strcmp(name, "pipeline")) {
+        if (int rc = discard_flush(b)) return rc;
         b->pipeline = value != 0;
     } else if (!strcmp(name, "pll_variant")) {
         if (value != 0 && value != 7 && value != 8)
@@ -466,6 +470,18 @@
     const int ev_lpw = 2 * ((b->N + 63) / 64) > (b->n_cu > 0 ? b->n_cu : 256) ? 64 : small_lpw;
     h.lanes_per_wave = b->hdlc_lpw ? b->hdlc_lpw : (b->hdlc_variant ? ev_lpw : 64);
     h.chunks = (b->streaming && b->ring_runs[b->ring_cur] == 0) ? b->ring_chunks[b->ring_cur] : nullptr;
+    h.discard = b->discard_pending && !b->streaming && b->ring_cur == 0;
+    h.ovf_mark = 2u << ((b->discard_launches + (h.discard ? 1u : 0u)) & 1u);
+}
+
+static int run_deframer(gnuais_batch *b, const HdlcLaunch &h, hipStream_t s)
+{
+    HIP_TRY(b->hdlc_variant ? launch_hdlc_events(h, s) : launch_hdlc_deframe(h, s));
+    if (h.discard) {
+        b->discard_pending = false;
+        b->discard_launches++;
+    }
+    return GNUAIS_OK;
 }
 
 static FrameTimeLaunch fill_frame_times(const gnuais_batch *b, const HdlcLaunch &h, int len)
@@ -594,10 +610,13 @@
     if (pl && b->calls >= 1 && sD != sC)
         HIP_TRY(hipStreamWaitEvent(sC, b->e_done[4][(k + b->nbuf - 1) % b->nbuf], 0));
     if (tm) HIP_TRY(hipEventRecord(ev[5], sC));
-    if (b->stage_mask & 8) HIP_TRY(b->hdlc_variant ? launch_hdlc_events(h, sC) : launch_hdlc_deframe(h, sC));
+    if (b->stage_mask & 8)
+        if (int rc = run_deframer(b, h, sC)) return rc;
     if (tm) HIP_TRY(hipEventRecord(ev[7], sC));
-    if (pl) HIP_TRY(hipEventRecord(b->e_done[3][k], sC));
+    const bool hand_off = pl && (sD != sC || !(b->cycle_parts & 2));
+    if (hand_off) HIP_TRY(hipEventRecord(b->e_done[3][k], sC));
     if (pl && sD != sC) HIP_TRY(hipStreamWaitEvent(sD, b->e_done[3][k], 0));
+    if (int rc = discard_flush(b)) return rc;
     if (tm) HIP_TRY(hipEventRecord(ev[9], sD));
     if (b->stage_mask & 16) HIP_TRY(launch_hdlc_crc(h, sD));
     if (b->repair && (b->stage_mask & 16)) HIP_TRY(launch_hdlc_repair(fill_repair(b, h), sD));
@@ -818,7 +837,7 @@
         HIP_TRY(hipMemcpy(b->segcnt[0], cnt.data(), cnt.size() * 4, hipMemcpyHostToDevice));
         HdlcLaunch h;
         fill_hdlc(b, h, 0);
-        HIP_TRY(b->hdlc_variant ? launch_hdlc_events(h, nullptr) : launch_hdlc_deframe(h, nullptr));
+        if (int rc = run_deframer(b, h, nullptr)) return rc;
         HIP_TRY(launch_hdlc_crc(h, nullptr));
         if (b->repair) HIP_TRY(launch_hdlc_repair(fill_repair(b, h), nullptr));
         if (b->frame_times) HIP_TRY(launch_frame_times(fill_frame_times(b, h, 0), nullptr));
diff --git a/gnuais_amd/csrc/hdlc_crc.hip b/gnuais_amd/csrc/hdlc_crc.hip
--- a/gnuais_amd/csrc/hdlc_crc.hip
+++ b/gnuais_amd/csrc/hdlc_crc.hip
@@ -1,6 +1,7 @@
 #include <hip/hip_runtime.h>
 #include <stdint.h>
 
+#include "crc_sliced.h"
 #include "kernels.h"
 
 namespace gnuais {
@@ -48,10 +49,11 @@
     const uint32_t *__restrict__ segbits, const uint32_t *__restrict__ segcnt,
     uint32_t *__restrict__ ctl, uint32_t *__restrict__ cand, uint32_t *__restrict__ cand_first,
     uint32_t *__restrict__ cand_count, int32_t *__restrict__ counters,
-    uint32_t *__restrict__ flags, int N, int n_seg, int seg_words, int K)
+    uint32_t *__restrict__ flags, int N, int n_seg, int seg_words, int K, uint32_t ovf_mark)
 {
     __builtin_amdgcn_s_setprio(3);
     const int cg = blockIdx.x * blockDim.x + threadIdx.x;
+    if ((ovf_mark & 1u) && cg == 0) hdlc_discard_ring(flags, ovf_mark & ~1u);
     const bool live = cg < N;
     const size_t c = (size_t) (live ? cg : N - 1), n_ = (size_t) N;
 
@@ -194,7 +196,7 @@
                                     bufferpos = 0; cur = 0; rawpos = 0; bitstuff = 0; last = 0;
                                     rec_ok = (nstart - first) < (uint32_t) K;
                                     rec = cand + ((size_t) c * K + nstart % (uint32_t) K) * CAND_WORDS;
-                                    if (rec_ok) rec[0] = 0; else flags[1] = 1;
+                                    if (rec_ok) rec[0] = 0; else flags[1] = ovf_mark & ~1u;
                                     ++nstart;
                                 } else if (L == R - 1) {
                                     HDLC_RESET(); nstartsign = 1; last = 0;
@@ -317,134 +319,148 @@
     }
 }
 
+struct K3Rec {
+    uint4 v[CAND_WORDS / 4];
+    int c;
+};
+static_assert(CAND_WORDS % 4 == 0 && CAND_HDR == 2, "a candidate record is a whole number of 16-byte loads");
+
+__device__ __forceinline__ void k3_fetch(K3Rec &r, uint32_t i, uint32_t total, const uint32_t *pre, const uint32_t *first,
+                                         const uint32_t *__restrict__ cand, int K, int ch0)
+{
+    r.c = -1;
+    r.v[0].x = 0;
+    if (i >= total) return;
+    int lo = 0, hi = K3_CH - 1;
+    while (lo < hi) {
+        const int mid = (lo + hi + 1) >> 1;
+        if (pre[mid] <= i) lo = mid; else hi = mid - 1;
+    }
+    r.c = ch0 + lo;
+    const uint32_t slot = (first[lo] + (i - pre[lo])) % (uint32_t) K;
+    const uint4 *rec = reinterpret_cast<const uint4 *>(cand + ((size_t) r.c * K + slot) * CAND_WORDS);
+#pragma unroll
+    for (int q = 0; q < CAND_WORDS / 4; ++q) r.v[q] = rec[q];
+}
+
 __global__ __launch_bounds__(256) void hdlc_crc_kernel(
     const uint32_t *__restrict__ cand, const uint32_t *__restrict__ cand_first,
     const uint32_t *__restrict__ cand_count, int32_t *__restrict__ counters,
     uint32_t *__restrict__ frames, uint32_t *__restrict__ flags, uint32_t frame_cap, int N, int K,
     uint2 *__restrict__ chunks, int n_pass)
 {
-    __shared__ uint32_t tab[256];
+    __shared__ uint16_t tab[crc::SLICES * 256];
     __shared__ uint32_t pre[K3_CH + 1];
+    __shared__ uint32_t first[K3_CH];
     extern __shared__ uint32_t k3_dyn[];
-    uint32_t (*const stage)[HDLC_BUF_WORDS + 1] = reinterpret_cast<uint32_t (*)[HDLC_BUF_WORDS + 1]>(k3_dyn);
-    uint32_t (*const rawlds)[CAND_WORDS - CAND_HDR + 1] =
-        reinterpret_cast<uint32_t (*)[CAND_WORDS - CAND_HDR + 1]>(k3_dyn + 256 * (HDLC_BUF_WORDS + 1));
+    constexpr int RAW_WORDS = CAND_WORDS - CAND_HDR;
+    const int tid = threadIdx.x;
+    uint32_t *const stage = k3_dyn + tid;
+    uint32_t *const rawlds = k3_dyn + 256 * (HDLC_BUF_WORDS + 1) + tid;
     __shared__ uint32_t wave_cnt[4];
     __shared__ uint32_t pass_base;
-    const int tid = threadIdx.x;
-    const int c_own = blockIdx.x * K3_CH + tid;
+    const int ch0 = blockIdx.x * K3_CH;
 
     {
         uint32_t t = (uint32_t) tid;
 #pragma unroll
-        for (int k = 0; k < 8; ++k) t = (t >> 1) ^ ((t & 1u) ? 0x8408u : 0u);
-        tab[tid] = t;
-    }
-    if (tid < K3_CH) pre[tid + 1] = (c_own < N) ? cand_count[c_own] : 0u;
-    __syncthreads();
-    if (tid == 0) {
-        uint32_t run = 0;
-        pre[0] = 0;
-        for (int q = 1; q <= K3_CH; ++q) { run += pre[q]; pre[q] = run; }
+        for (int k = 0; k < crc::SLICES; ++k) {
+            t = crc::advance8(t);
+            tab[k * 256 + tid] = (uint16_t) t;
+        }
+    }
+    static_assert(K3_CH <= 64, "the scan is one wave's");
+    if (tid < 64) {
+        const int c_own = ch0 + tid;
+        const bool own = tid < K3_CH && c_own < N;
+        uint32_t v = own ? cand_count[c_own] : 0u;
+        const uint32_t f = own ? cand_first[c_own] : 0u;
+#pragma unroll
+        for (int d = 1; d < K3_CH; d <<= 1) {
+            const uint32_t up = __shfl_up(v, d);
+            if (tid >= d) v += up;
+        }
+        if (tid < K3_CH) { pre[tid + 1] = v; first[tid] = f; }
+        if (tid == 0) pre[0] = 0;
     }
     __syncthreads();
     const uint32_t total = pre[K3_CH];
     const size_t n_ = (size_t) N;
 
+    K3Rec nx;
+    k3_fetch(nx, (uint32_t) tid, total, pre, first, cand, K, ch0);
     int pass = 0;
     for (uint32_t i0 = 0; i0 < total; i0 += 256, ++pass) {
-        const uint32_t i = i0 + (uint32_t) tid;
+        const K3Rec r = nx;
+        if (i0 + 256 < total) k3_fetch(nx, i0 + 256 + (uint32_t) tid, total, pre, first, cand, K, ch0);
         bool good = false;
-        uint32_t out[16];
-#pragma unroll
-        for (int q = 0; q < 16; ++q) out[q] = 0;
-        if (i < total) {
-            int lo = 0, hi = K3_CH - 1;
-            while (lo < hi) {
-                const int mid = (lo + hi + 1) >> 1;
-                if (pre[mid] <= i) lo = mid; else hi = mid - 1;
-            }
-            const int c = blockIdx.x * K3_CH + lo;
-            const uint32_t j = i - pre[lo];
-            const uint32_t slot = (cand_first[c] + j) % (uint32_t) K;
-            const uint32_t *rec = cand + ((size_t) c * K + slot) * CAND_WORDS;
-            const uint32_t hdr = rec[0];
-            if (hdr & CAND_VALID) {
-                const int n = (int) (hdr & 0xffffu);
-                const int rawlen = (int) ((hdr >> 17) & 0x3ffu);
-                const int nbytes = n >> 3, buflen = nbytes + 2;
-                {
-                    uint32_t raw[CAND_WORDS - CAND_HDR];
-#pragma unroll
-                    for (int q = 0; q < CAND_WORDS - CAND_HDR; ++q) raw[q] = rec[CAND_HDR + q];
-#pragma unroll
-                    for (int q = 0; q < CAND_WORDS - CAND_HDR; ++q) rawlds[tid][q] = raw[q];
-                    unsigned long long acc = 0;
-                    uint32_t prevw = 0;
-                    int fill = 0, ow = 0;
-                    const int nwords = (rawlen + 31) >> 5;
+        const uint32_t hdr = r.v[0].x;
+        const int n = (int) (hdr & 0xffffu);
+        const int nbytes = n >> 3, buflen = nbytes + 2;
+        if (r.c >= 0 && (hdr & CAND_VALID)) {
+            const int rawlen = (int) ((hdr >> 17) & 0x3ffu);
+            {
+                rawlds[0] = r.v[0].z;
+                rawlds[256] = r.v[0].w;
+#pragma unroll
+                for (int q = 1; q < CAND_WORDS / 4; ++q) {
+                    rawlds[(4 * q - 2) * 256] = r.v[q].x;
+                    rawlds[(4 * q - 1) * 256] = r.v[q].y;
+                    rawlds[(4 * q) * 256] = r.v[q].z;
+                    rawlds[(4 * q + 1) * 256] = r.v[q].w;
+                }
+                unsigned long long acc = 0;
+                uint32_t prevw = 0;
+                int fill = 0, ow = 0;
+                const int nwords = (rawlen + 31) >> 5;
 #pragma unroll 1
-                    for (int q = 0; q < nwords; ++q) {
-                        uint32_t rw = rawlds[tid][q];
-                        const int nvq = rawlen - 32 * q < 32 ? rawlen - 32 * q : 32;
-                        const unsigned long long cc = ((unsigned long long) rw << 32) | prevw;
-                        const uint32_t five = (uint32_t) (cc >> 31) & (uint32_t) (cc >> 30) & (uint32_t) (cc >> 29) &
-                                              (uint32_t) (cc >> 28) & (uint32_t) (cc >> 27);
-                        uint32_t stf = five & ~rw & (nvq >= 32 ? ~0u : (1u << nvq) - 1u);
-                        prevw = rw;
-                        int nout = nvq;
-                        while (stf) {
-                            const int pz = 31 - __clz((int) stf);
-                            stf &= ~(1u << pz);
-                            rw = (rw & ((1u << pz) - 1u)) | ((pz >= 31 ? 0u : rw >> (pz + 1)) << pz);
-                            --nout;
-                        }
-                        if (nout < 32) rw &= (1u << nout) - 1u;
-                        acc |= (unsigned long long) rw << fill;
-                        fill += nout;
-                        if (fill >= 32) {
-                            if (ow <= HDLC_BUF_WORDS) stage[tid][ow] = (uint32_t) acc;
-                            ++ow;
-                            acc >>= 32;
-                            fill -= 32;
-                        }
+                for (int q = 0; q < nwords && q < RAW_WORDS; ++q) {
+                    uint32_t rw = rawlds[q * 256];
+                    const int nvq = rawlen - 32 * q < 32 ? rawlen - 32 * q : 32;
+                    const unsigned long long cc = ((unsigned long long) rw << 32) | prevw;
+                    const uint32_t five = (uint32_t) (cc >> 31) & (uint32_t) (cc >> 30) & (uint32_t) (cc >> 29) &
+                                          (uint32_t) (cc >> 28) & (uint32_t) (cc >> 27);
+                    uint32_t stf = five & ~rw & (nvq >= 32 ? ~0u : (1u << nvq) - 1u);
+                    prevw = rw;
+                    int nout = nvq;
+                    while (stf) {
+                        const int pz = 31 - __clz((int) stf);
+                        stf &= ~(1u << pz);
+                        rw = (rw & ((1u << pz) - 1u)) | ((pz >= 31 ? 0u : rw >> (pz + 1)) << pz);
+                        --nout;
                     }
-                    if (ow <= HDLC_BUF_WORDS) stage[tid][ow] = (uint32_t) acc;
-                    for (int q = ow + 1; q <= HDLC_BUF_WORDS; ++q) stage[tid][q] = 0;
-                }
-                uint32_t w[HDLC_BUF_WORDS];
-#pragma unroll
-                for (int q = 0; q < HDLC_BUF_WORDS; ++q) w[q] = stage[tid][q];
-                uint32_t crc = 0xffffu;
-#pragma unroll
-                for (int q = 0; q < HDLC_BUF_WORDS; ++q) {
-#pragma unroll
-                    for (int bq = 0; bq < 4; ++bq) {
-                        if (q * 4 + bq < buflen) {
-                            const uint32_t byte = (w[q] >> (8 * bq)) & 0xffu;
-                            crc = (crc >> 8) ^ tab[(crc ^ byte) & 0xffu];
-                        }
+                    if (nout < 32) rw &= (1u << nout) - 1u;
+                    acc |= (unsigned long long) rw << fill;
+                    fill += nout;
+                    if (fill >= 32) {
+                        if (ow <= HDLC_BUF_WORDS) stage[ow * 256] = (uint32_t) acc;
+                        ++ow;
+                        acc >>= 32;
+                        fill -= 32;
                     }
                 }
-                if (crc == 0xf0b8u) {
-                    good = true;
-                    atomicAdd(&counters[c], 1);
-                    out[0] = (uint32_t) c;
-                    out[1] = rec[1];
-#pragma unroll
-                    for (int q = 0; q < 14; ++q) {
-                        uint32_t v = 0;
-                        if (q * 4 < nbytes) {
-                            v = w[q];
-                            const int keep = nbytes - q * 4;
-                            if (keep < 4) v &= (1u << (8 * keep)) - 1u;
-                        }
-                        if (q == 13) v = (v & 0xffu) | ((1u | ((hdr >> 27) << 1)) << 8) | ((uint32_t) n << 16);
-                        out[2 + q] = v;
-                    }
-                } else {
-                    atomicAdd(&counters[n_ + c], 1);
-                }
+                if (ow <= HDLC_BUF_WORDS) stage[ow * 256] = (uint32_t) acc;
+                for (int q = ow + 1; q <= HDLC_BUF_WORDS; ++q) stage[q * 256] = 0;
+            }
+            uint32_t w[HDLC_BUF_WORDS];
+#pragma unroll
+            for (int q = 0; q < HDLC_BUF_WORDS; ++q) w[q] = stage[q * 256];
+            uint32_t crc = 0xffffu;
+#pragma unroll
+            for (int q = 0; q < HDLC_BUF_WORDS; ++q)
+                if (4 * q + 4 <= buflen) crc = crc::step4(crc, w[q], tab);
+            {
+                const int qt = buflen >> 2;
+                const uint32_t tw = stage[(qt < HDLC_BUF_WORDS ? qt : HDLC_BUF_WORDS) * 256];
+#pragma unroll
+                for (int bq = 0; bq < 3; ++bq)
+                    if (bq < (buflen & 3)) crc = crc::step1(crc, (tw >> (8 * bq)) & 0xffu, tab);
+            }
+            if (crc == 0xf0b8u) {
+                good = true;
+                atomicAdd(&counters[r.c], 1);
+            } else {
+                atomicAdd(&counters[n_ + r.c], 1);
             }
         }
         const unsigned long long m = __ballot(good);
@@ -469,6 +485,20 @@
         if (good) {
             const uint32_t idx = pass_base + woff + below;
             if (idx < frame_cap) {
+                uint32_t out[16];
+                out[0] = (uint32_t) r.c;
+                out[1] = r.v[0].y;
+#pragma unroll
+                for (int q = 0; q < 14; ++q) {
+                    uint32_t v = 0;
+                    if (q * 4 < nbytes) {
+                        v = stage[q * 256];
+                        const int keep = nbytes - q * 4;
+                        if (keep < 4) v &= (1u << (8 * keep)) - 1u;
+                    }
+                    if (q == 13) v = (v & 0xffu) | ((1u | ((hdr >> 27) << 1)) << 8) | ((uint32_t) n << 16);
+                    out[2 + q] = v;
+                }
                 uint4 *dst = reinterpret_cast<uint4 *>(frames + (size_t) idx * 16);
                 dst[0] = make_uint4(out[0], out[1], out[2], out[3]);
                 dst[1] = make_uint4(out[4], out[5], out[6], out[7]);
@@ -491,13 +521,13 @@
     hipLaunchKernelGGL(hdlc_deframe_kernel, dim3((a.N + lpw - 1) / lpw), dim3(lpw),
                        (PACK_MAX + 1) * lpw * sizeof(uint32_t), stream,
                        a.segbits, a.segcnt, a.ctl, a.cand, a.cand_first, a.cand_count, a.counters,
-                       a.frame_count, a.N, a.n_seg, a.seg_words, a.K);
+                       a.frame_count, a.N, a.n_seg, a.seg_words, a.K, a.ovf_mark | (a.discard ? 1u : 0u));
     return hipGetLastError();
 }
 
 hipError_t launch_hdlc_crc(const HdlcLaunch &a, hipStream_t stream)
 {
-    constexpr size_t K3_DYN_LDS = 256 * ((HDLC_BUF_WORDS + 1) + (CAND_WORDS - CAND_HDR + 1)) * sizeof(uint32_t);
+    constexpr size_t K3_DYN_LDS = 256 * ((HDLC_BUF_WORDS + 1) + (CAND_WORDS - CAND_HDR)) * sizeof(uint32_t);
     hipLaunchKernelGGL(hdlc_crc_kernel, dim3((unsigned) ((a.N + K3_CH - 1) / K3_CH)), dim3(256), K3_DYN_LDS,
                        stream, a.cand, a.cand_first, a.cand_count, a.counters,
                        (uint32_t *) a.frames, a.frame_count, a.frame_cap, a.N, a.K, a.chunks, k3_passes(a.K_call > 0 ? a.K_call : a.K));
diff --git a/gnuais_amd/csrc/hdlc_events.hip b/gnuais_amd/csrc/hdlc_events.hip
--- a/gnuais_amd/csrc/hdlc_events.hip
+++ b/gnuais_amd/csrc/hdlc_events.hip
@@ -34,12 +34,13 @@
     const uint32_t *__restrict__ segbits, const uint32_t *__restrict__ segcnt,
     uint32_t *__restrict__ ctl, uint32_t *__restrict__ cand, uint32_t *__restrict__ cand_first,
     uint32_t *__restrict__ cand_count, int32_t *__restrict__ counters,
-    uint32_t *__restrict__ flags, int N, int n_seg, int seg_words, int K)
+    uint32_t *__restrict__ flags, int N, int n_seg, int seg_words, int K, uint32_t ovf_mark)
 {
     __builtin_amdgcn_s_setprio(3);
     extern __shared__ uint32_t lds[];
     const int tpb = TPB > 0 ? TPB : (int) blockDim.x, tx = (int) threadIdx.x;
     const int cg = blockIdx.x * blockDim.x + threadIdx.x;
+    if ((ovf_mark & 1u) && cg == 0) hdlc_discard_ring(flags, ovf_mark & ~1u);
     const bool live = cg < N;
     const size_t c = (size_t) (live ? cg : N - 1), n_ = (size_t) N;
     uint32_t *const Xa = lds + tx, *const NAa = Xa + (EW + 2) * tpb, *const CBa = NAa + EW * tpb,
@@ -71,7 +72,7 @@
          bufferpos = 0; cur = 0; rawpos = 0; bitstuff = 0; last = 0;                    \
          rec_ok = (nstart - first) < (uint32_t) K;                                      \
          rec = cand + ((size_t) c * K + nstart % (uint32_t) K) * CAND_WORDS;            \
-         if (rec_ok) rec[0] = 0; else flags[1] = 1;                                     \
+         if (rec_ok) rec[0] = 0; else flags[1] = ovf_mark & ~1u;                                    \
          ++nstart; } while (0)
 #define RAW_APPEND(v_, n_bits_)                                                         \
     do { const uint32_t sb_ = (v_); const int nb_ = (n_bits_), bsh_ = rawpos & 31;      \
@@ -459,7 +460,7 @@
     const size_t lds = EV_ROWS * lpw * sizeof(uint32_t);
 #define EV_LAUNCH(T)                                                                                                  \
     hipLaunchKernelGGL(hdlc_events_kernel<T>, grid, block, lds, stream, a.segbits, a.segcnt, a.ctl, a.cand, a.cand_first, \
-                       a.cand_count, a.counters, a.frame_count, a.N, a.n_seg, a.seg_words, a.K)
+                       a.cand_count, a.counters, a.frame_count, a.N, a.n_seg, a.seg_words, a.K, a.ovf_mark | (a.discard ? 1u : 0u))
     switch (lpw) {
     case 8: EV_LAUNCH(8); break;
     case 16: EV_LAUNCH(16); break;
diff --git a/gnuais_amd/csrc/kernels.h b/gnuais_amd/csrc/kernels.h
--- a/gnuais_amd/csrc/kernels.h
+++ b/gnuais_amd/csrc/kernels.h
@@ -87,7 +87,17 @@
     int K_call = 0;
     int lanes_per_wave;
     uint2 *chunks = nullptr;
-};
+    bool discard = false;
+    uint32_t ovf_mark = 2;
+};
+#if defined(__HIPCC__)
+__device__ __forceinline__ void hdlc_discard_ring(uint32_t *flags, uint32_t ovf_mark)
+{
+    flags[0] = 0;
+    atomicAnd(&flags[1], ovf_mark);
+    flags[2] = 0;
+}
+#endif
 constexpr int K3_CH = 32;
 inline int k3_blocks(int N) { return (N + K3_CH - 1) / K3_CH; }
 inline int k3_passes(int K) { return (K3_CH * K + 255) / 256; }
```

After: 1.746 million Msamples/s, median of 6. 3.0% higher.
